# antoyang/TubeDETR

Measured on AMD Instinct MI355X. Metric: training clips/sec (fwd+bwd) at T=100 k=4 res=352, 1/2/4/8 MI355X, higher is better.
Workload: dtype bf16

## Files before the change

### include/tubedetr_hip.h

```cpp
#ifndef TUBEDETR_HIP_H
#define TUBEDETR_HIP_H
#include <stddef.h>
#include <stdint.h>
#ifdef __cplusplus
extern "C" {
#endif

#define TD_F32 0
#define TD_BF16 1
#define TD_U8 2
#define TD_OK 0
#define TD_ERR_INVALID (-1)
#define TD_ERR_LAUNCH (-2)

typedef void* td_stream_t;

const char* td_last_error(void);
int td_abi_version(void);

int td_set_deterministic(int on);
int td_get_deterministic(void);


#define TD_PROF_GEMM_128x128 0
#define TD_PROF_GEMM_128x64 1
#define TD_PROF_WGRAD 2
#define TD_PROF_GEMM_64x128 3
#define TD_PROF_PW_RESIDENT 4
#define TD_PROF_GEMM_256 5
#define TD_PROF_GEMM_256_PW 6
#define TD_PROF_FUSED 7
#define TD_PROF_CROSS_Q1 8
#define TD_PROF_WGRAD_SINGLE 9
#define TD_PROF_CHAIN 10
#define TD_PROF_FAMILIES 11
int td_prof_enable(int on);
int td_prof_collect(int family, int dtype, long long* launches, double* ms, double* flops);
int td_prof_collect_bytes(int family, int dtype, double* bytes);
int td_prof_dump(const char* path);
int td_debug_set_stamp_buffer(unsigned long long* buf);

typedef struct td_conv_desc {
  int N, Hs, Ws, C;
  int Ho, Wo;
  int R, S, stride, pad;
  int mode;
  int Nc;
  int ldc;
  int out_sp;
  int out_H, out_W;
  int aniso;
  int stride_w, pad_w;
} td_conv_desc;

typedef struct td_epilogue {
  const float* bias;
  const void* residual;
  const void* mask_src;
  int relu;
  int sigmoid;
  float dropout_p;
  uint32_t dropout_seed;
  float alpha;
  const uint32_t* dropout_counter;
} td_epilogue;

int td_conv_gemm(const void* src, const void* wmat, void* out, const td_conv_desc* d, const td_epilogue* e,
                 int dtype, td_stream_t stream);

typedef struct td_linear_ex_desc {
  int M, N, K1, K2;
  int lda1, lda2, ldc, ldr;
  int w_shared;
  long long rows1, rows2;
  const int* a1_map;
  const int* a2_map;
  const int* out_map;
  const int* res_map;
} td_linear_ex_desc;
int td_linear_ex(const void* a1, const void* a2, const void* wmat, void* out, const td_linear_ex_desc* x, const td_epilogue* e,
                 int dtype, td_stream_t stream);

int td_conv_wgrad(const void* g, const void* src, float* dw, const td_conv_desc* d, int ldg, int dtype, int splits,
                  td_stream_t stream);
int td_conv_wgrad_bias(const void* g, const void* src, float* dw, float* dbias, const td_conv_desc* d, int ldg, int dtype,
                       int splits, td_stream_t stream);

typedef struct td_wgrad_job {
  const void* g;
  const void* src;
  float* dW;
  const float* scale;
  td_conv_desc d;
  int ldg;
  int ci_real;
  float* dbias;
  int accumulate;
  int prezeroed;
} td_wgrad_job;
size_t td_conv_wgrad_batch_table_bytes(int n_jobs);
int td_conv_wgrad_batch(const td_wgrad_job* jobs, int n_jobs, int dtype, void* table_host, void* table_dev, size_t table_bytes,
                        td_stream_t stream);

typedef struct td_frame_source {
  const void* data;
  int dtype;
  int n;
  const int* index;
  const int* valid_hw;
} td_frame_source;
int td_frames_to_nhwc(const td_frame_source* srcs, int n_srcs, int C, int H, int W, int Cpad, const float* mean,
                      const float* inv_std, void* y, int dtype, td_stream_t stream);

size_t td_resnet_fwd_ws_bytes(int N, int H, int W, const int* nblocks, int dtype, int save);
int td_resnet_num_convs(const int* nblocks);
int td_resnet_fwd(const td_frame_source* srcs, int n_srcs, const float* mean, const float* inv_std, int N, int H, int W,
                  const int* nblocks, const void* const* w_fwd, const float* const* bias, int save, void* ws, size_t ws_bytes,
                  void** feat, int* feat_hw, int stem_pairs, int first_train_stage, int dtype, td_stream_t stream);
int td_bottleneck_fused(const void* x, void* out, const void* w1, const float* b1, const void* w2, const float* b2, const void* w3,
                        const float* b3, const void* wd, const float* bd, int N, int H, int W, int Cin, int dtype, td_stream_t stream);
int td_pw_chain2(const void* y2, const void* w3, const float* b3, const void* residual, void* out, const void* w1, const float* b1,
                 void* h1, int M, int planes, int dtype, td_stream_t stream);
int td_stem_pair_weights(const void* w_fwd_8, void* w_pairs, int Co, int dtype, td_stream_t stream);
int td_stem_pool(const void* x_pairs, const void* w_pairs, const float* bias, void* pooled, int N, int H, int W, int dtype,
                 td_stream_t stream);
size_t td_resnet_bwd_ws_bytes(int N, int H, int W, const int* nblocks, int first_train_stage, int dtype);
size_t td_resnet_bwd_table_bytes(const int* nblocks, int first_train_stage);
int td_resnet_bwd(const void* dfeat, int N, int N_fwd, int H, int W, const int* nblocks, int first_train_stage,
                  const void* const* w_dgrad, const float* const* scale, float* const* dW, const void* fwd_ws, void* ws,
                  size_t ws_bytes, void* table_host, void* table_dev, size_t table_bytes, int dW_prezeroed, int dtype, int only_stage, td_stream_t stream);

int td_weight_prep(const float* W, const float* bn_w, const float* bn_b, const float* bn_rm, const float* bn_rv,
                   const float* bias, int Co, int Ci, int R, int S, int Cpad, void* w_fwd, void* w_dgrad,
                   float* bias_out, float* scale_out, int dtype, td_stream_t stream);

typedef struct td_prep_item {
  const float* W;
  const float *bn_w, *bn_b, *bn_rm, *bn_rv, *bias;
  void *w_fwd, *w_dgrad;
  float *bias_out, *scale_out;
  int Co, Ci, RS, Cpad, Co_alloc, blk0;
} td_prep_item;
int td_weight_prep_batch(const td_prep_item* items_dev, int n, int total_blocks, int dtype, td_stream_t stream);

int td_wgrad_finalize(const float* dw_k, const float* scale, float* dW, int Co, int Ci, int R, int S, int Cpad,
                      int accumulate, td_stream_t stream);

int td_nchw_to_nhwc(const float* x, void* y, int N, int C, int H, int W, int Cpad, int dtype, td_stream_t stream);
int td_nhwc_to_nchw(const void* x, float* y, int N, int C, int H, int W, int dtype, td_stream_t stream);
int td_cast(const void* x, void* y, size_t n, int src_dtype, int dst_dtype, td_stream_t stream);

int td_maxpool3x3s2(const void* x, void* y, int N, int H, int W, int C, int dtype, td_stream_t stream);

int td_add_layernorm_fwd(const void* x, const void* r, const float* gamma, const float* beta, void* y, void* s_out,
                         float* mean, float* rstd, int rows, int cols, float eps, int dtype, td_stream_t stream);
int td_add_layernorm_bwd(const void* dy, const void* s, const float* mean, const float* rstd, const float* gamma,
                         const void* extra, void* ds, float* dgamma, float* dbeta, int rows, int cols, int dtype,
                         td_stream_t stream);

int td_colsum(const void* g, float* out, int rows, int cols, int ld, int dtype, td_stream_t stream);
int td_add(const void* a, const void* b, void* y, size_t n, int dtype, td_stream_t stream);

int td_relu_bwd(const void* dy, const void* y, void* g, size_t n, float scale, int dtype, td_stream_t stream);

int td_gelu_fwd(const void* x, void* y, size_t n, int dtype, td_stream_t stream);
int td_gelu_bwd(const void* dy, const void* x, void* dx, size_t n, int dtype, td_stream_t stream);

int td_dropout(const void* x, void* y, size_t n, float p, uint32_t seed, const uint32_t* dropout_counter, int dtype,
               td_stream_t stream);

int td_pos_sine(const uint8_t* mask, void* pos, int N, int h, int w, int npf, float temperature, int rows_per_image, int dtype,
                td_stream_t stream);

int td_rows_copy(const void* src, const int* src_map, const void* add, void* dst, const int* dst_map, int n_rows, int cols, int ld_src,
                 int ld_add, int ld_dst, int dtype, td_stream_t stream);
int td_rows_segment_sum(const void* in, const int* idx, const int* ptr, void* out, const int* out_map, int n_out, int cols, int ld_in,
                        int ld_out, int dtype, td_stream_t stream);

int td_mha_fwd(const void* q, const void* k, const void* v, const uint8_t* key_pad, void* out, float* probs,
               float* wavg, int B, int H, int Lq, int Lk, int hd, int ldq, int ldk, int ldv, int ldo, float scale,
               float dropout_p, uint32_t dropout_seed, const uint32_t* dropout_counter, int dtype, td_stream_t stream);
int td_mha_bwd(const void* q, const void* k, const void* v, const void* dout, const float* probs, const float* dwavg,
               void* dq, void* dk, void* dv, float* ds_ws, int B, int H, int Lq, int Lk, int hd, int ldq, int ldk,
               int ldv, int ldo, float scale, float dropout_p, uint32_t dropout_seed, const uint32_t* dropout_counter,
               int dtype, td_stream_t stream);

int td_cross_q1_fwd(const void* u, const void* mem, const void* pos, const uint8_t* key_pad, float* probs, float* wavg, void* zext,
                    int F, int S, int H, int E, int ldz, float dropout_p, uint32_t dropout_seed, const uint32_t* dropout_counter,
                    int dtype, td_stream_t stream);
int td_cross_q1_bwd(const void* u, const void* mem, const void* pos, const float* probs, const void* d_zext, const float* dwavg,
                    void* d_u, float* d_mem, int accumulate, int F, int S, int H, int E, int ldz, float dropout_p, uint32_t dropout_seed,
                    const uint32_t* dropout_counter, int dtype, td_stream_t stream);
int td_cross_q1_bwd_coef(const void* u, const void* mem, const void* pos, const float* probs, const void* d_zext, const float* dwavg,
                         void* d_u, void* coef, int coef_ld, int coef_col, int F, int S, int H, int E, int ldz, float dropout_p,
                         uint32_t dropout_seed, const uint32_t* dropout_counter, int dtype, td_stream_t stream);
int td_cross_q1_dmem(const void* coef, int coef_ld, const void* const* u, const void* const* d_zext, int n_layers, void* d_mem, int F, int S,
                     int H, int E, int ldz, int dtype, td_stream_t stream);
int td_head_blocks_expand(const float* W, const float* bias, float alpha, void* w_n, void* w_t, int E, int H, int dtype, td_stream_t stream);
int td_head_blocks_extract(const float* G, float alpha, float* dW, float* db, int E, int H, td_stream_t stream);

size_t td_mha_lean_stats_bytes(int B, int H, int Lq);
int td_mha_lean_fwd(const void* q, const void* k, const void* v, const uint8_t* key_pad, void* out, float* stats, int B, int H,
                    int Lq, int Lk, int hd, int ldq, int ldk, int ldv, int ldo, float scale, float dropout_p,
                    uint32_t dropout_seed, const uint32_t* dropout_counter, int dtype, td_stream_t stream);
int td_mha_lean_bwd(const void* q, const void* k, const void* v, const uint8_t* key_pad, const void* out, const void* dout,
                    float* stats, void* dq, void* dk, void* dv, int B, int H, int Lq, int Lk, int hd, int ldq, int ldk, int ldv,
                    int ldo, float scale, float dropout_p, uint32_t dropout_seed, const uint32_t* dropout_counter, int dtype,
                    td_stream_t stream);


#define TD_OPTIM_MAX_SEGMENTS 32
#define TD_OPTIM_MAX_GROUPS 4
#define TD_OPTIM_NORM_BLOCKS 2048
typedef struct td_optim_segment {
  long long begin, end;
  int group;
  int active;
} td_optim_segment;
size_t td_grad_norm_ws_bytes(void);
int td_grad_norm_clip(const float* grad, size_t n, const td_optim_segment* segs, int n_segs, float max_norm, void* ws,
                      size_t ws_bytes, float* norm_clip, int* step, td_stream_t stream);
int td_adamw_ema_step(float* param, const float* grad, float* exp_avg, float* exp_avg_sq, float* ema, size_t n,
                      const td_optim_segment* segs, int n_segs, const float* lr_dev, const float* norm_clip,
                      const int* step_dev, float beta1, float beta2, float eps, float weight_decay, float ema_decay,
                      td_stream_t stream);

int td_criterion_fwd(const float* boxes, const float* tgt, const long long* keep, const float* sted, const float* weights,
                     const uint8_t* time_mask, const uint8_t* positive, const int* inter, const float* num_boxes_dev,
                     float num_boxes_host, float sigma, int nl, int b, int T, int n, float* losses, float* g_l1, float* g_giou,
                     float* g_sted, float* g_w, td_stream_t stream);
int td_criterion_bwd(const float* dlosses, const float* g_l1, const float* g_giou, const float* g_sted, const float* g_w,
                     float* d_boxes, float* d_sted, float* d_weights, int nl, int b, int T, td_stream_t stream);

int td_sted_decode(const float* steds, long long* start_end, int n_videos, int T, td_stream_t stream);

typedef struct td_resample_job {
  const void* src;
  long long src_frame_stride;
  int src_pitch;
  int T, sh, sw;
  int flip;
// ... 16 lines not shown
```

### tubedetr_amd/_hip.py

```python
from __future__ import annotations

import ctypes as C
import os

import torch

TD_F32, TD_BF16 = 0, 1
EXPECTED_ABI = 11
_LIB_PATH = os.environ.get("TD_HIP_LIB") or os.path.join(os.path.dirname(os.path.abspath(__file__)), "lib", "libtubedetr_hip.so")
_lib = None


class ConvDesc(C.Structure):
    _fields_ = [(n, C.c_int) for n in ("N", "Hs", "Ws", "C", "Ho", "Wo", "R", "S", "stride", "pad", "mode", "Nc", "ldc", "out_sp", "out_H", "out_W",
                                       "aniso", "stride_w", "pad_w")]


class PrepItem(C.Structure):
    _fields_ = [(n, C.c_void_p) for n in ("W", "bn_w", "bn_b", "bn_rm", "bn_rv", "bias", "w_fwd", "w_dgrad", "bias_out", "scale_out")] + \
               [(n, C.c_int) for n in ("Co", "Ci", "RS", "Cpad", "Co_alloc", "blk0")]


class WgradJob(C.Structure):
    _fields_ = [("g", C.c_void_p), ("src", C.c_void_p), ("dW", C.c_void_p), ("scale", C.c_void_p), ("d", ConvDesc), ("ldg", C.c_int), ("ci_real", C.c_int), ("dbias", C.c_void_p), ("accumulate", C.c_int), ("prezeroed", C.c_int)]


TD_U8 = 2


class FrameSource(C.Structure):
    _fields_ = [("data", C.c_void_p), ("dtype", C.c_int), ("n", C.c_int), ("index", C.c_void_p), ("valid_hw", C.c_void_p)]


class LinearExDesc(C.Structure):
    _fields_ = [(n, C.c_int) for n in ("M", "N", "K1", "K2", "lda1", "lda2", "ldc", "ldr", "w_shared")] + \
               [("rows1", C.c_longlong), ("rows2", C.c_longlong)] + [(n, C.c_void_p) for n in ("a1_map", "a2_map", "out_map", "res_map")]


class OptimSegment(C.Structure):
    _fields_ = [("begin", C.c_longlong), ("end", C.c_longlong), ("group", C.c_int), ("active", C.c_int)]


class ResampleJob(C.Structure):
    _fields_ = [("src", C.c_void_p), ("src_frame_stride", C.c_longlong)] + [(n, C.c_int) for n in ("src_pitch", "T", "sh", "sw", "flip", "rh", "rw", "wy", "wx", "wh", "ww")] + \
               [("dst", C.c_void_p)] + [(n, C.c_int) for n in ("planar", "frame_off", "H", "W")] + [("mask", C.c_void_p)]


class Epilogue(C.Structure):
    _fields_ = [
        ("bias", C.c_void_p),
        ("residual", C.c_void_p),
        ("mask_src", C.c_void_p),
        ("relu", C.c_int),
        ("sigmoid", C.c_int),
        ("dropout_p", C.c_float),
        ("dropout_seed", C.c_uint32),
        ("alpha", C.c_float),
        ("dropout_counter", C.c_void_p),
    ]


_P, _I, _F, _U32, _SZ = C.c_void_p, C.c_int, C.c_float, C.c_uint32, C.c_size_t
_SIGS = {
    "td_prof_enable": [_I],
    "td_prof_dump": [C.c_char_p],
    "td_debug_set_stamp_buffer": [_P],
    "td_prof_collect": [_I, _I, C.POINTER(C.c_longlong), C.POINTER(C.c_double), C.POINTER(C.c_double)],
    "td_prof_collect_bytes": [_I, _I, C.POINTER(C.c_double)],
    "td_conv_gemm": [_P, _P, _P, C.POINTER(ConvDesc), C.POINTER(Epilogue), _I, _P],
    "td_conv_wgrad": [_P, _P, _P, C.POINTER(ConvDesc), _I, _I, _I, _P],
    "td_conv_wgrad_bias": [_P, _P, _P, _P, C.POINTER(ConvDesc), _I, _I, _I, _P],
    "td_conv_wgrad_batch": [C.POINTER(WgradJob), _I, _I, _P, _P, _SZ, _P],
    "td_resnet_num_convs": [C.POINTER(C.c_int)],
    "td_resnet_fwd": [C.POINTER(FrameSource), _I, C.POINTER(C.c_float), C.POINTER(C.c_float), _I, _I, _I, C.POINTER(C.c_int), C.POINTER(_P), C.POINTER(_P), _I, _P, _SZ,
                      C.POINTER(_P), C.POINTER(C.c_int), _I, _I, _I, _P],
    "td_bottleneck_fused": [_P, _P, _P, _P, _P, _P, _P, _P, _P, _P, _I, _I, _I, _I, _I, _P],
    "td_stem_pair_weights": [_P, _P, _I, _I, _P],
    "td_stem_pool": [_P, _P, _P, _P, _I, _I, _I, _I, _P],
    "td_pw_chain2": [_P, _P, _P, _P, _P, _P, _P, _P, _I, _I, _I, _P],
    "td_set_deterministic": [_I],
    "td_get_deterministic": [],
    "td_frames_to_nhwc": [C.POINTER(FrameSource), _I, _I, _I, _I, _I, C.POINTER(C.c_float), C.POINTER(C.c_float), _P, _I, _P],
    "td_resnet_bwd": [_P, _I, _I, _I, _I, C.POINTER(C.c_int), _I, C.POINTER(_P), C.POINTER(_P), C.POINTER(_P), _P, _P, _SZ, _P, _P, _SZ, _I, _I, _I, _P],
    "td_weight_prep_batch": [_P, _I, _I, _I, _P],
    "td_weight_prep": [_P, _P, _P, _P, _P, _P, _I, _I, _I, _I, _I, _P, _P, _P, _P, _I, _P],
    "td_wgrad_finalize": [_P, _P, _P, _I, _I, _I, _I, _I, _I, _P],
    "td_nchw_to_nhwc": [_P, _P, _I, _I, _I, _I, _I, _I, _P],
    "td_nhwc_to_nchw": [_P, _P, _I, _I, _I, _I, _I, _P],
    "td_cast": [_P, _P, _SZ, _I, _I, _P],
    "td_maxpool3x3s2": [_P, _P, _I, _I, _I, _I, _I, _P],
    "td_add_layernorm_fwd": [_P, _P, _P, _P, _P, _P, _P, _P, _I, _I, _F, _I, _P],
    "td_add_layernorm_bwd": [_P, _P, _P, _P, _P, _P, _P, _P, _P, _I, _I, _I, _P],
    "td_colsum": [_P, _P, _I, _I, _I, _I, _P],
    "td_add": [_P, _P, _P, _SZ, _I, _P],
    "td_relu_bwd": [_P, _P, _P, _SZ, _F, _I, _P],
    "td_gelu_fwd": [_P, _P, _SZ, _I, _P],
    "td_gelu_bwd": [_P, _P, _P, _SZ, _I, _P],
    "td_dropout": [_P, _P, _SZ, _F, _U32, _P, _I, _P],
    "td_pos_sine": [_P, _P, _I, _I, _I, _I, _F, _I, _I, _P],
    "td_linear_ex": [_P, _P, _P, _P, C.POINTER(LinearExDesc), C.POINTER(Epilogue), _I, _P],
    "td_rows_copy": [_P, _P, _P, _P, _P, _I, _I, _I, _I, _I, _I, _P],
    "td_rows_segment_sum": [_P, _P, _P, _P, _P, _I, _I, _I, _I, _I, _P],
    "td_criterion_fwd": [_P, _P, _P, _P, _P, _P, _P, _P, _P, _F, _F, _I, _I, _I, _I, _P, _P, _P, _P, _P, _P],
    "td_criterion_bwd": [_P, _P, _P, _P, _P, _P, _P, _P, _I, _I, _I, _P],
    "td_sted_decode": [_P, _P, _I, _I, _P],
    "td_grad_norm_clip": [_P, _SZ, C.POINTER(OptimSegment), _I, _F, _P, _SZ, _P, _P, _P],
    "td_adamw_ema_step": [_P, _P, _P, _P, _P, _SZ, C.POINTER(OptimSegment), _I, _P, _P, _P, _F, _F, _F, _F, _F, _P],
    "td_mha_fwd": [_P, _P, _P, _P, _P, _P, _P, _I, _I, _I, _I, _I, _I, _I, _I, _I, _F, _F, _U32, _P, _I, _P],
    "td_mha_bwd": [_P, _P, _P, _P, _P, _P, _P, _P, _P, _P, _I, _I, _I, _I, _I, _I, _I, _I, _I, _F, _F, _U32, _P, _I, _P],
    "td_cross_q1_fwd": [_P, _P, _P, _P, _P, _P, _P, _I, _I, _I, _I, _I, _F, _U32, _P, _I, _P],
    "td_cross_q1_bwd": [_P, _P, _P, _P, _P, _P, _P, _P, _I, _I, _I, _I, _I, _I, _F, _U32, _P, _I, _P],
    "td_cross_q1_bwd_coef": [_P, _P, _P, _P, _P, _P, _P, _P, _I, _I, _I, _I, _I, _I, _I, _F, _U32, _P, _I, _P],
    "td_cross_q1_dmem": [_P, _I, _P, _P, _I, _P, _I, _I, _I, _I, _I, _I, _P],
    "td_head_blocks_expand": [_P, _P, _F, _P, _P, _I, _I, _I, _P],
    "td_head_blocks_extract": [_P, _F, _P, _P, _I, _I, _P],
    "td_mha_lean_fwd": [_P, _P, _P, _P, _P, _P, _I, _I, _I, _I, _I, _I, _I, _I, _I, _F, _F, _U32, _P, _I, _P],
    "td_mha_lean_bwd": [_P, _P, _P, _P, _P, _P, _P, _P, _P, _P, _I, _I, _I, _I, _I, _I, _I, _I, _I, _F, _F, _U32, _P, _I, _P],
    "td_clip_resample": [C.POINTER(ResampleJob), _I, _P, _P, _SZ, _P],
}
_SIZE_SIGS = {
    "td_grad_norm_ws_bytes": [],
    "td_mha_lean_stats_bytes": [_I, _I, _I],
    "td_conv_wgrad_batch_table_bytes": [_I],
    "td_clip_resample_table_bytes": [_I],
    "td_resnet_bwd_table_bytes": [C.POINTER(C.c_int), _I],
    "td_resnet_fwd_ws_bytes": [_I, _I, _I, C.POINTER(C.c_int), _I, _I],
    "td_resnet_bwd_ws_bytes": [_I, _I, _I, C.POINTER(C.c_int), _I, _I],
}
EXPORTS = ["td_last_error", "td_abi_version"] + list(_SIGS) + list(_SIZE_SIGS)


def lib_path() -> str:
    return _LIB_PATH


def lib() -> C.CDLL:
    global _lib
    if _lib is None:
        if not os.path.exists(_LIB_PATH):
            raise RuntimeError(
                f"{_LIB_PATH} is missing: build it with `python -m tubedetr_amd.build` (or __graft_entry__.build()); "
                "tubedetr_amd has no CPU / eager fallback"
            )
        L = C.CDLL(_LIB_PATH)
        L.td_last_error.restype = C.c_char_p
        L.td_last_error.argtypes = []
        L.td_abi_version.restype = C.c_int
        L.td_abi_version.argtypes = []
        got = L.td_abi_version()
        if got != EXPECTED_ABI:
            raise RuntimeError(f"{_LIB_PATH} has ABI version {got}, this binding needs {EXPECTED_ABI}: rebuild it with "
                               "`python -m tubedetr_amd.build --force`")
        for name, sig in _SIGS.items():
            fn = getattr(L, name)
            fn.restype = C.c_int
            fn.argtypes = sig
        for name, sig in _SIZE_SIGS.items():
            fn = getattr(L, name)
            fn.restype = C.c_size_t
            fn.argtypes = sig
        _lib = L
    return _lib


def check(rc: int, what: str = ""):
    if rc != 0:
        raise RuntimeError(f"libtubedetr_hip {what} failed ({rc}): {lib().td_last_error().decode()}")


def stream_ptr() -> int:
    return torch._C._cuda_getCurrentRawStream(torch._C._cuda_getDevice())


def dtype_code(dt: torch.dtype) -> int:
    if dt == torch.float32:
        return TD_F32
    if dt == torch.bfloat16:
        return TD_BF16
    raise TypeError(f"unsupported compute dtype {dt}")


def ptr(t) -> int:
    if t is None:
# ... 4 lines not shown
```

### tubedetr_amd/csrc/elementwise.hip

```cpp
#include "td_common.h"

namespace td {

template <typename T>
__global__ void maxpool3x3s2_kernel(const T* x, T* y, int N, int H, int W, int C, int Ho, int Wo) {
  constexpr int VEC = 16 / sizeof(T);
  const int cv = C / VEC;
  const size_t n = (size_t)N * Ho * Wo * cv;
  const size_t idx = (size_t)blockIdx.x * blockDim.x + threadIdx.x;
  if (idx >= n) return;
  int c = (idx % cv) * VEC;
  size_t t = idx / cv;
  int wo = t % Wo; t /= Wo;
  int ho = t % Ho;
  int img = t / Ho;
  float m[VEC];
#pragma unroll
  for (int i = 0; i < VEC; ++i) m[i] = -INFINITY;
  for (int r = 0; r < 3; ++r) {
    int h = ho * 2 - 1 + r;
    if ((unsigned)h >= (unsigned)H) continue;
    for (int s = 0; s < 3; ++s) {
      int w = wo * 2 - 1 + s;
      if ((unsigned)w >= (unsigned)W) continue;
// ... 43 lines not shown
      float dlt = v[j] - mu;
      var += dlt * dlt;
    }
  }
  var = wave_sum(var) / cols;
  const float rs = rsqrtf(var + eps);
  if (lane == 0) {
    if (mean) mean[row] = mu;
    if (rstd) rstd[row] = rs;
  }
#pragma unroll
  for (int j = 0; j < LN_MAXJ; ++j) {
    int c = lane + 64 * j;
    if (j < nj && c < cols) {
      if (s_out) Elem<T>::store(s_out, base + c, v[j]);
      Elem<T>::store(y, base + c, (v[j] - mu) * rs * gamma[c] + beta[c]);
    }
  }
}

__device__ __forceinline__ void unpack4v(const uint2& v, float (&o)[4]) {
  o[0] = __uint_as_float(v.x << 16); o[1] = __uint_as_float(v.x & 0xffff0000u);
  o[2] = __uint_as_float(v.y << 16); o[3] = __uint_as_float(v.y & 0xffff0000u);
}
__device__ __forceinline__ uint2 pack4_bf16(const float (&v)[4]) {
  return make_uint2((uint32_t)f32_to_bf16(v[0]) | ((uint32_t)f32_to_bf16(v[1]) << 16), (uint32_t)f32_to_bf16(v[2]) | ((uint32_t)f32_to_bf16(v[3]) << 16));
}
static bool aligned8(const void* a, const void* b, const void* c, const void* d) {
  return (((uintptr_t)a | (uintptr_t)b | (uintptr_t)c | (uintptr_t)d) & 7) == 0;
}

template <int NJ>
__global__ __launch_bounds__(256) void add_layernorm_fwd_v4_kernel(const u16* __restrict__ x, const u16* __restrict__ r, const float* __restrict__ gamma,
                                                                   const float* __restrict__ beta, u16* __restrict__ y, u16* __restrict__ s_out,
                                                                   float* __restrict__ mean, float* __restrict__ rstd, int rows, float eps) {
  constexpr int cols = NJ * 256;
  const int lane = threadIdx.x & 63;
  const int row = blockIdx.x * 4 + (threadIdx.x >> 6);
  if (row >= rows) return;
  const size_t base = (size_t)row * cols + lane * 4;
  float v[NJ][4];
  float sum = 0.f;
#pragma unroll
  for (int j = 0; j < NJ; ++j) {
    unpack4v(*(const uint2*)(x + base + 256 * j), v[j]);
    if (r) {
      float a[4];
      unpack4v(*(const uint2*)(r + base + 256 * j), a);
#pragma unroll
      for (int e = 0; e < 4; ++e) v[j][e] += a[e];
    }
#pragma unroll
    for (int e = 0; e < 4; ++e) sum += v[j][e];
  }
  const float mu = wave_sum(sum) * (1.f / cols);
  float var = 0.f;
#pragma unroll
  for (int j = 0; j < NJ; ++j)
#pragma unroll
    for (int e = 0; e < 4; ++e) {
      const float d = v[j][e] - mu;
      var += d * d;
    }
  var = wave_sum(var) * (1.f / cols);
  const float rs = rsqrtf(var + eps);
  if (lane == 0) {
    if (mean) mean[row] = mu;
    if (rstd) rstd[row] = rs;
  }
#pragma unroll
  for (int j = 0; j < NJ; ++j) {
    const float4 gm = *(const float4*)(gamma + lane * 4 + 256 * j), bt = *(const float4*)(beta + lane * 4 + 256 * j);
    if (s_out) *(uint2*)(s_out + base + 256 * j) = pack4_bf16(v[j]);
    float o[4] = {(v[j][0] - mu) * rs * gm.x + bt.x, (v[j][1] - mu) * rs * gm.y + bt.y, (v[j][2] - mu) * rs * gm.z + bt.z,
                  (v[j][3] - mu) * rs * gm.w + bt.w};
    *(uint2*)(y + base + 256 * j) = pack4_bf16(o);
  }
}

template <int NJ>
__global__ __launch_bounds__(256) void add_layernorm_bwd_v4_kernel(const u16* __restrict__ dy, const u16* __restrict__ s, const float* __restrict__ mean,
                                                                   const float* __restrict__ rstd, const float* __restrict__ gamma,
                                                                   const u16* __restrict__ extra, u16* __restrict__ ds, float* dgamma, float* dbeta,
                                                                   int rows) {
  constexpr int cols = NJ * 256;
  const int lane = threadIdx.x & 63;
  const int wid = blockIdx.x * 4 + (threadIdx.x >> 6);
  const int nw = gridDim.x * 4;
  float pg[NJ][4], pb[NJ][4], gm[NJ][4];
#pragma unroll
  for (int j = 0; j < NJ; ++j) {
    const float4 g4 = *(const float4*)(gamma + lane * 4 + 256 * j);
    gm[j][0] = g4.x; gm[j][1] = g4.y; gm[j][2] = g4.z; gm[j][3] = g4.w;
#pragma unroll
    for (int e = 0; e < 4; ++e) pg[j][e] = pb[j][e] = 0.f;
  }
  for (int row = wid; row < rows; row += nw) {
    const size_t base = (size_t)row * cols + lane * 4;
    const float mu = mean[row], rs = rstd[row];
    float xh[NJ][4], dg[NJ][4];
    float c1 = 0.f, c2 = 0.f;
#pragma unroll
    for (int j = 0; j < NJ; ++j) {
      float d[4], sv[4];
      unpack4v(*(const uint2*)(dy + base + 256 * j), d);
      unpack4v(*(const uint2*)(s + base + 256 * j), sv);
#pragma unroll
      for (int e = 0; e < 4; ++e) {
        xh[j][e] = (sv[e] - mu) * rs;
        dg[j][e] = d[e] * gm[j][e];
        c1 += dg[j][e];
        c2 += dg[j][e] * xh[j][e];
        pg[j][e] += d[e] * xh[j][e];
        pb[j][e] += d[e];
      }
    }
    c1 = wave_sum(c1) * (1.f / cols);
    c2 = wave_sum(c2) * (1.f / cols);
#pragma unroll
    for (int j = 0; j < NJ; ++j) {
      float o[4];
#pragma unroll
      for (int e = 0; e < 4; ++e) o[e] = rs * (dg[j][e] - c1 - xh[j][e] * c2);
      if (extra) {
        float ex[4];
        unpack4v(*(const uint2*)(extra + base + 256 * j), ex);
#pragma unroll
        for (int e = 0; e < 4; ++e) o[e] += ex[e];
      }
      *(uint2*)(ds + base + 256 * j) = pack4_bf16(o);
    }
  }
  __shared__ float redg[4][cols], redb[4][cols];
  const int wv = threadIdx.x >> 6;
#pragma unroll
  for (int j = 0; j < NJ; ++j)
#pragma unroll
    for (int e = 0; e < 4; ++e) {
      redg[wv][lane * 4 + 256 * j + e] = pg[j][e];
      redb[wv][lane * 4 + 256 * j + e] = pb[j][e];
    }
  __syncthreads();
  for (int c = threadIdx.x; c < cols; c += 256) {
    if (dgamma) atomicAdd(dgamma + c, redg[0][c] + redg[1][c] + redg[2][c] + redg[3][c]);
    if (dbeta) atomicAdd(dbeta + c, redb[0][c] + redb[1][c] + redb[2][c] + redb[3][c]);
  }
}

template <typename T>
__global__ __launch_bounds__(256) void add_layernorm_bwd_kernel(const T* dy, const T* s, const float* mean, const float* rstd,
                                                                const float* gamma, const T* extra, T* ds, float* dgamma,
                                                                float* dbeta, int rows, int cols) {
  const int lane = threadIdx.x & 63;
  const int wid = blockIdx.x * 4 + (threadIdx.x >> 6);
  const int nw = gridDim.x * 4;
  const int nj = (cols + 63) / 64;
  float pg[LN_MAXJ], pb[LN_MAXJ];
#pragma unroll
  for (int j = 0; j < LN_MAXJ; ++j) pg[j] = pb[j] = 0.f;
  for (int row = wid; row < rows; row += nw) {
    const size_t base = (size_t)row * cols;
    const float mu = mean[row], rs = rstd[row];
    float xh[LN_MAXJ], dg[LN_MAXJ];
    float c1 = 0.f, c2 = 0.f;
#pragma unroll
    for (int j = 0; j < LN_MAXJ; ++j) {
      xh[j] = dg[j] = 0.f;
      int c = lane + 64 * j;
      if (j < nj && c < cols) {
        float d = Elem<T>::load(dy, base + c);
        xh[j] = (Elem<T>::load(s, base + c) - mu) * rs;
        dg[j] = d * gamma[c];
        c1 += dg[j];
        c2 += dg[j] * xh[j];
        pg[j] += d * xh[j];
        pb[j] += d;
      }
    }
    c1 = wave_sum(c1) / cols;
    c2 = wave_sum(c2) / cols;
#pragma unroll
    for (int j = 0; j < LN_MAXJ; ++j) {
      int c = lane + 64 * j;
      if (j < nj && c < cols) {
        float o = rs * (dg[j] - c1 - xh[j] * c2);
        if (extra) o += Elem<T>::load(extra, base + c);
        Elem<T>::store(ds, base + c, o);
      }
    }
  }
  __shared__ float redg[4][64 * LN_MAXJ], redb[4][64 * LN_MAXJ];
  const int wv = threadIdx.x >> 6;
#pragma unroll
  for (int j = 0; j < LN_MAXJ; ++j) {
    if (j < nj) {
      redg[wv][lane + 64 * j] = pg[j];
      redb[wv][lane + 64 * j] = pb[j];
    }
  }
  __syncthreads();
  for (int c = threadIdx.x; c < cols; c += 256) {
    if (dgamma) atomicAdd(dgamma + c, redg[0][c] + redg[1][c] + redg[2][c] + redg[3][c]);
    if (dbeta) atomicAdd(dbeta + c, redb[0][c] + redb[1][c] + redb[2][c] + redb[3][c]);
  }
}

template <typename T>
__global__ void colsum_kernel(const T* g, float* out, int rows, int cols, int ld, int rows_per_block) {
  const int c = blockIdx.x * blockDim.x + threadIdx.x;
  if (c >= cols) return;
  const int r0 = blockIdx.y * rows_per_block;
  const int r1 = min(rows, r0 + rows_per_block);
  float acc = 0.f;
  for (int r = r0; r < r1; ++r) acc += Elem<T>::load(g, (size_t)r * ld + c);
  atomicAdd(out + c, acc);
}

template <typename T>
__global__ __launch_bounds__(256) void colsum_vec_kernel(const T* g, float* out, int rows, int cols, int ld, int rows_per_block) {
  constexpr int VEC = 16 / sizeof(T);
  __shared__ float red[8][32 * VEC + 1];
  const int cg = threadIdx.x & 31, rl = threadIdx.x >> 5;
  const int c0 = (blockIdx.x * 32 + cg) * VEC;
  const int r0 = blockIdx.y * rows_per_block;
  const int r1 = min(rows, r0 + rows_per_block);
  float acc[VEC];
#pragma unroll
  for (int i = 0; i < VEC; ++i) acc[i] = 0.f;
  if (c0 < cols) {
    for (int r = r0 + rl; r < r1; r += 8) {
      uint4 v = *(const uint4*)(g + (size_t)r * ld + c0);
      const T* e = (const T*)&v;
#pragma unroll
      for (int i = 0; i < VEC; ++i) acc[i] += Elem<T>::load(e, i);
    }
  }
#pragma unroll
  for (int i = 0; i < VEC; ++i) red[rl][cg * VEC + i] = acc[i];
  __syncthreads();
  for (int c = threadIdx.x; c < 32 * VEC; c += 256) {
    const int col = blockIdx.x * 32 * VEC + c;
    if (col < cols) {
      float sum = 0.f;
#pragma unroll
      for (int j = 0; j < 8; ++j) sum += red[j][c];
      atomicAdd(out + col, sum);
    }
  }
}

__device__ __forceinline__ float gelu_f(float x) { return 0.5f * x * (1.f + erff(x * 0.70710678118654752f)); }
__device__ __forceinline__ float gelu_grad_f(float x) {
  return 0.5f * (1.f + erff(x * 0.70710678118654752f)) + x * 0.3989422804014327f * __expf(-0.5f * x * x);
}

template <typename T, int OP>
__global__ __launch_bounds__(256) void ew_kernel(const T* a, const T* b, T* y, size_t n, float scale, uint32_t thresh, uint32_t seed_in, const uint32_t* seed_dev) {
  const uint32_t seed = (OP == 2) ? effective_seed(seed_in, seed_dev) : seed_in;
  constexpr int VEC = 16 / sizeof(T);
  const size_t nv = n / VEC;
  size_t i = (size_t)blockIdx.x * blockDim.x + threadIdx.x;
  const size_t stride = (size_t)gridDim.x * blockDim.x;
  for (size_t v = i; v < nv; v += stride) {
    uint4 va = ((const uint4*)a)[v], vb = make_uint4(0, 0, 0, 0), vo;
    if (b) vb = ((const uint4*)b)[v];
    const T* ea = (const T*)&va;
    const T* eb = (const T*)&vb;
    T* eo = (T*)&vo;
#pragma unroll
    for (int k = 0; k < VEC; ++k) {
// ... 107 lines not shown
  }
}

template <typename T>
__global__ __launch_bounds__(256) void rows_segment_sum_kernel(const char* __restrict__ in, const int* __restrict__ idx, const int* __restrict__ ptr,
                                                               char* __restrict__ out, const int* __restrict__ out_map, int n_out, int chunks, int ld_in,
                                                               int ld_out) {
  constexpr int EPL = 16 / sizeof(T);
  const size_t total = (size_t)n_out * chunks;
  for (size_t t = (size_t)blockIdx.x * blockDim.x + threadIdx.x; t < total; t += (size_t)gridDim.x * blockDim.x) {
    const int r = (int)(t / chunks), c = (int)(t - (size_t)r * chunks);
    float acc[EPL];
#pragma unroll
    for (int q = 0; q < EPL; ++q) acc[q] = 0.f;
    const int j0 = ptr[r], j1 = ptr[r + 1];
    for (int j = j0; j < j1; ++j) {
      const uint4 v = *(const uint4*)(in + ((size_t)idx[j] * ld_in + (size_t)c * EPL) * sizeof(T));
      if constexpr (sizeof(T) == 2) {
        const uint32_t* pv = (const uint32_t*)&v;
#pragma unroll
        for (int q = 0; q < 4; ++q) {
          acc[2 * q] += __uint_as_float(pv[q] << 16);
          acc[2 * q + 1] += __uint_as_float(pv[q] & 0xffff0000u);
        }
      } else {
        acc[0] += __uint_as_float(v.x); acc[1] += __uint_as_float(v.y); acc[2] += __uint_as_float(v.z); acc[3] += __uint_as_float(v.w);
      }
    }
    uint4 o;
    if constexpr (sizeof(T) == 2) {
      o.x = (uint32_t)f32_to_bf16(acc[0]) | ((uint32_t)f32_to_bf16(acc[1]) << 16);
      o.y = (uint32_t)f32_to_bf16(acc[2]) | ((uint32_t)f32_to_bf16(acc[3]) << 16);
      o.z = (uint32_t)f32_to_bf16(acc[4 % EPL]) | ((uint32_t)f32_to_bf16(acc[5 % EPL]) << 16);
      o.w = (uint32_t)f32_to_bf16(acc[6 % EPL]) | ((uint32_t)f32_to_bf16(acc[7 % EPL]) << 16);
    } else {
      o = make_uint4(__float_as_uint(acc[0]), __float_as_uint(acc[1]), __float_as_uint(acc[2]), __float_as_uint(acc[3]));
    }
    *(uint4*)(out + ((size_t)(out_map ? out_map[r] : r) * ld_out + (size_t)c * EPL) * sizeof(T)) = o;
  }
}

}
using namespace td;

static inline unsigned nblk(size_t n, int bs = 256) { return (unsigned)((n + bs - 1) / bs); }
#define TD_DISPATCH(dtype, CALL_BF16, CALL_F32, who)  \
  if (dtype == TD_BF16) { CALL_BF16; }                \
  else if (dtype == TD_F32) { CALL_F32; }             \
  else TD_REQUIRE(false, who ": bad dtype")

extern "C" int td_maxpool3x3s2(const void* x, void* y, int N, int H, int W, int C, int dtype, td_stream_t stream) {
  TD_REQUIRE(x && y, "td_maxpool3x3s2: null pointer");
  const int vec = dtype == TD_BF16 ? 8 : 4;
  TD_REQUIRE(C % vec == 0, "td_maxpool3x3s2: C must be a multiple of %d", vec);
  const int Ho = (H + 2 - 3) / 2 + 1, Wo = (W + 2 - 3) / 2 + 1;
  size_t n = (size_t)N * Ho * Wo * (C / vec);
  hipStream_t st = (hipStream_t)stream;
  TD_DISPATCH(dtype, (maxpool3x3s2_kernel<u16><<<nblk(n), 256, 0, st>>>((const u16*)x, (u16*)y, N, H, W, C, Ho, Wo)),
              (maxpool3x3s2_kernel<float><<<nblk(n), 256, 0, st>>>((const float*)x, (float*)y, N, H, W, C, Ho, Wo)),
              "td_maxpool3x3s2");
  return check_launch("td_maxpool3x3s2");
}

extern "C" int td_add_layernorm_fwd(const void* x, const void* r, const float* gamma, const float* beta, void* y,
                                    void* s_out, float* mean, float* rstd, int rows, int cols, float eps, int dtype,
                                    td_stream_t stream) {
  TD_REQUIRE(x && gamma && beta && y, "td_add_layernorm_fwd: null pointer");
  TD_REQUIRE(cols <= 64 * LN_MAXJ, "td_add_layernorm_fwd: cols > %d", 64 * LN_MAXJ);
  if (rows == 0) return TD_OK;
  hipStream_t st = (hipStream_t)stream;
  unsigned g = (rows + 3) / 4;
  if (dtype == TD_BF16 && (cols == 256 || cols == 768) && aligned8(x, r, y, s_out)) {
    if (cols == 256) add_layernorm_fwd_v4_kernel<1><<<g, 256, 0, st>>>((const u16*)x, (const u16*)r, gamma, beta, (u16*)y, (u16*)s_out, mean, rstd, rows, eps);
    else add_layernorm_fwd_v4_kernel<3><<<g, 256, 0, st>>>((const u16*)x, (const u16*)r, gamma, beta, (u16*)y, (u16*)s_out, mean, rstd, rows, eps);
    return check_launch("td_add_layernorm_fwd");
  }
  TD_DISPATCH(dtype,
              (add_layernorm_fwd_kernel<u16><<<g, 256, 0, st>>>((const u16*)x, (const u16*)r, gamma, beta, (u16*)y, (u16*)s_out, mean, rstd, rows, cols, eps)),
              (add_layernorm_fwd_kernel<float><<<g, 256, 0, st>>>((const float*)x, (const float*)r, gamma, beta, (float*)y, (float*)s_out, mean, rstd, rows, cols, eps)),
              "td_add_layernorm_fwd");
  return check_launch("td_add_layernorm_fwd");
}

extern "C" int td_add_layernorm_bwd(const void* dy, const void* s, const float* mean, const float* rstd,
                                    const float* gamma, const void* extra, void* ds, float* dgamma, float* dbeta,
                                    int rows, int cols, int dtype, td_stream_t stream) {
  TD_REQUIRE(dy && s && mean && rstd && gamma && ds, "td_add_layernorm_bwd: null pointer");
  TD_REQUIRE(cols <= 64 * LN_MAXJ, "td_add_layernorm_bwd: cols > %d", 64 * LN_MAXJ);
  if (rows == 0) return TD_OK;
  hipStream_t st = (hipStream_t)stream;
  unsigned g = (rows + 3) / 4;
  if (dtype == TD_BF16 && (cols == 256 || cols == 768) && aligned8(dy, s, ds, extra)) {
    unsigned gv = (rows + 31) / 32;
    if (gv > 1024) gv = 1024;
    if (deterministic()) gv = 1;
    if (cols == 256) add_layernorm_bwd_v4_kernel<1><<<gv, 256, 0, st>>>((const u16*)dy, (const u16*)s, mean, rstd, gamma, (const u16*)extra, (u16*)ds, dgamma, dbeta, rows);
    else add_layernorm_bwd_v4_kernel<3><<<gv, 256, 0, st>>>((const u16*)dy, (const u16*)s, mean, rstd, gamma, (const u16*)extra, (u16*)ds, dgamma, dbeta, rows);
    return check_launch("td_add_layernorm_bwd");
  }
  if (g > 256) g = 256;
  if (deterministic()) g = 1;
  TD_DISPATCH(dtype,
              (add_layernorm_bwd_kernel<u16><<<g, 256, 0, st>>>((const u16*)dy, (const u16*)s, mean, rstd, gamma, (const u16*)extra, (u16*)ds, dgamma, dbeta, rows, cols)),
              (add_layernorm_bwd_kernel<float><<<g, 256, 0, st>>>((const float*)dy, (const float*)s, mean, rstd, gamma, (const float*)extra, (float*)ds, dgamma, dbeta, rows, cols)),
              "td_add_layernorm_bwd");
  return check_launch("td_add_layernorm_bwd");
}

extern "C" int td_colsum(const void* g, float* out, int rows, int cols, int ld, int dtype, td_stream_t stream) {
  TD_REQUIRE(g && out, "td_colsum: null pointer");
  if (rows == 0 || cols == 0) return TD_OK;
  hipStream_t st = (hipStream_t)stream;
  const int vec = dtype == TD_BF16 ? 8 : 4;
  if (cols % vec == 0 && ld % vec == 0) {
    const int gx = (cols + 32 * vec - 1) / (32 * vec);
    int rpb = (int)(((long long)rows * gx + 511) / 512);
    if (rpb < 64) rpb = 64;
    if (deterministic()) rpb = rows;
    dim3 grid(gx, (rows + rpb - 1) / rpb);
    TD_DISPATCH(dtype, (colsum_vec_kernel<u16><<<grid, 256, 0, st>>>((const u16*)g, out, rows, cols, ld, rpb)),
                (colsum_vec_kernel<float><<<grid, 256, 0, st>>>((const float*)g, out, rows, cols, ld, rpb)), "td_colsum");
    return check_launch("td_colsum");
  }
  int rpb = (int)(((long long)rows * ((cols + 255) / 256) + 1023) / 1024);
  if (rpb < 8) rpb = 8;
  if (deterministic()) rpb = rows;
  dim3 grid((cols + 255) / 256, (rows + rpb - 1) / rpb);
  TD_DISPATCH(dtype, (colsum_kernel<u16><<<grid, 256, 0, st>>>((const u16*)g, out, rows, cols, ld, rpb)),
              (colsum_kernel<float><<<grid, 256, 0, st>>>((const float*)g, out, rows, cols, ld, rpb)), "td_colsum");
  return check_launch("td_colsum");
}

extern "C" int td_add(const void* a, const void* b, void* y, size_t n, int dtype, td_stream_t stream) {
  TD_REQUIRE(a && y, "td_add: null pointer");
  if (n == 0) return TD_OK;
  hipStream_t st = (hipStream_t)stream;
  unsigned g = nblk(n / 4 + 1);
  if (g > 4096) g = 4096;
  TD_REQUIRE(((uintptr_t)a | (uintptr_t)y | (uintptr_t)b) % 16 == 0, "td_add: pointers must be 16-byte aligned");
  TD_DISPATCH(dtype, (ew_kernel<u16, 0><<<g, 256, 0, st>>>((const u16*)a, (const u16*)b, (u16*)y, n, 1.f, 0, 0, nullptr)),
              (ew_kernel<float, 0><<<g, 256, 0, st>>>((const float*)a, (const float*)b, (float*)y, n, 1.f, 0, 0, nullptr)), "td_add");
  return check_launch("td_add");
}

extern "C" int td_relu_bwd(const void* dy, const void* y, void* g, size_t n, float scale, int dtype, td_stream_t stream) {
  TD_REQUIRE(dy && y && g, "td_relu_bwd: null pointer");
  if (n == 0) return TD_OK;
  hipStream_t st = (hipStream_t)stream;
  unsigned gr = nblk(n);
  if (gr > 4096) gr = 4096;
  TD_REQUIRE(((uintptr_t)dy | (uintptr_t)y | (uintptr_t)g) % 16 == 0, "td_relu_bwd: pointers must be 16-byte aligned");
  TD_DISPATCH(dtype, (ew_kernel<u16, 1><<<gr, 256, 0, st>>>((const u16*)dy, (const u16*)y, (u16*)g, n, scale, 0, 0, nullptr)),
              (ew_kernel<float, 1><<<gr, 256, 0, st>>>((const float*)dy, (const float*)y, (float*)g, n, scale, 0, 0, nullptr)), "td_relu_bwd");
  return check_launch("td_relu_bwd");
}

extern "C" int td_gelu_fwd(const void* x, void* y, size_t n, int dtype, td_stream_t stream) {
  TD_REQUIRE(x && y, "td_gelu_fwd: null pointer");
  if (n == 0) return TD_OK;
  hipStream_t st = (hipStream_t)stream;
  unsigned gr = nblk(n);
  if (gr > 4096) gr = 4096;
  TD_REQUIRE(((uintptr_t)x | (uintptr_t)y) % 16 == 0, "td_gelu_fwd: pointers must be 16-byte aligned");
  TD_DISPATCH(dtype, (ew_kernel<u16, 3><<<gr, 256, 0, st>>>((const u16*)x, nullptr, (u16*)y, n, 1.f, 0, 0, nullptr)),
              (ew_kernel<float, 3><<<gr, 256, 0, st>>>((const float*)x, nullptr, (float*)y, n, 1.f, 0, 0, nullptr)), "td_gelu_fwd");
  return check_launch("td_gelu_fwd");
}

extern "C" int td_gelu_bwd(const void* dy, const void* x, void* dx, size_t n, int dtype, td_stream_t stream) {
  TD_REQUIRE(dy && x && dx, "td_gelu_bwd: null pointer");
  if (n == 0) return TD_OK;
  hipStream_t st = (hipStream_t)stream;
  unsigned gr = nblk(n);
  if (gr > 4096) gr = 4096;
  TD_REQUIRE(((uintptr_t)dy | (uintptr_t)x | (uintptr_t)dx) % 16 == 0, "td_gelu_bwd: pointers must be 16-byte aligned");
  TD_DISPATCH(dtype, (ew_kernel<u16, 4><<<gr, 256, 0, st>>>((const u16*)dy, (const u16*)x, (u16*)dx, n, 1.f, 0, 0, nullptr)),
              (ew_kernel<float, 4><<<gr, 256, 0, st>>>((const float*)dy, (const float*)x, (float*)dx, n, 1.f, 0, 0, nullptr)), "td_gelu_bwd");
  return check_launch("td_gelu_bwd");
}

extern "C" int td_dropout(const void* x, void* y, size_t n, float p, uint32_t seed, const uint32_t* dropout_counter, int dtype,
                          td_stream_t stream) {
  TD_REQUIRE(x && y, "td_dropout: null pointer");
  TD_REQUIRE(p >= 0.f && p < 1.f, "td_dropout: p out of range");
  if (n == 0) return TD_OK;
  hipStream_t st = (hipStream_t)stream;
  unsigned gr = nblk(n);
// ... 61 lines not shown
```

### tubedetr_amd/csrc/gemm_conv.hip

```cpp
#include <stdlib.h>

#include <type_traits>

#include "td_common.h"
#include <algorithm>
#include <vector>

#ifndef TD_WGRAD_EARLY_ISSUE
#define TD_WGRAD_EARLY_ISSUE 1
#endif
#ifndef TD_BIG_XCD_CONTIG
#define TD_BIG_XCD_CONTIG 1
#endif
namespace td {

struct GemmParams {
  const char* src;
  const char* w;
  char* out;
  td_conv_desc d;
  int M, K;
  uint32_t src_bytes, w_bytes;
  unsigned long long* dbg;
  const float* bias;
  const char* residual;
  const char* mask_src;
  int relu, sigmoid;
  float alpha;
  uint32_t drop_thresh;
  float drop_scale;
  uint32_t seed;
  const uint32_t* seed_dev;
  const char* src2;
  uint32_t src2_bytes;
  int K1, lda1, lda2, ldr;
  int w_shared;
  const int* a1_map;
  const int* a2_map;
  const int* out_map;
  const int* res_map;
  int tap_inner;
  int w_ld;
  int wtap[4];
  int use_wtap;
};

template <typename T>
struct Mfma;
template <>
struct Mfma<u16> {
  static __device__ __forceinline__ void run(const uint4& wf, const uint4& af, f32x4& acc) {
    acc = __builtin_amdgcn_mfma_f32_16x16x32_bf16(*(const bf16x8*)&wf, *(const bf16x8*)&af, acc, 0, 0, 0);
  }
};
template <>
struct Mfma<float> {
  static __device__ __forceinline__ void run(const uint4& wf, const uint4& af, f32x4& acc) {
    const float* a = (const float*)&wf;
    const float* b = (const float*)&af;
#pragma unroll
    for (int s = 0; s < 4; ++s) acc = __builtin_amdgcn_mfma_f32_16x16x4f32(a[s], b[s], acc, 0, 0, 0);
  }
};

template <typename T>
__device__ __forceinline__ void load4(const char* base, size_t off, float (&o)[4]);
template <>
__device__ __forceinline__ void load4<float>(const char* base, size_t off, float (&o)[4]) {
  float4 v = *(const float4*)(base + off * 4);
  o[0] = v.x; o[1] = v.y; o[2] = v.z; o[3] = v.w;
}
template <>
__device__ __forceinline__ void load4<u16>(const char* base, size_t off, float (&o)[4]) {
  uint2 v = *(const uint2*)(base + off * 2);
  o[0] = __uint_as_float(v.x << 16); o[1] = __uint_as_float(v.x & 0xffff0000u);
  o[2] = __uint_as_float(v.y << 16); o[3] = __uint_as_float(v.y & 0xffff0000u);
}
template <typename T, typename V>
__device__ __forceinline__ void unpack4(const V& v, float (&o)[4]);
template <>
__device__ __forceinline__ void unpack4<float, float4>(const float4& v, float (&o)[4]) {
  o[0] = v.x; o[1] = v.y; o[2] = v.z; o[3] = v.w;
}
template <>
__device__ __forceinline__ void unpack4<u16, uint2>(const uint2& v, float (&o)[4]) {
  o[0] = __uint_as_float(v.x << 16); o[1] = __uint_as_float(v.x & 0xffff0000u);
  o[2] = __uint_as_float(v.y << 16); o[3] = __uint_as_float(v.y & 0xffff0000u);
}
typedef __bf16 bf16x2_t __attribute__((ext_vector_type(2)));
__device__ __forceinline__ uint32_t pack_bf16x2(float lo, float hi) {
  bf16x2_t v = {(__bf16)lo, (__bf16)hi};
  return *(uint32_t*)&v;
}
template <typename T>
__device__ __forceinline__ void unpack16(const uint4& v, float (&o)[16 / sizeof(T)]);
template <>
__device__ __forceinline__ void unpack16<float>(const uint4& v, float (&o)[4]) {
  o[0] = __uint_as_float(v.x); o[1] = __uint_as_float(v.y); o[2] = __uint_as_float(v.z); o[3] = __uint_as_float(v.w);
}
template <>
__device__ __forceinline__ void unpack16<u16>(const uint4& v, float (&o)[8]) {
  o[0] = __uint_as_float(v.x << 16); o[1] = __uint_as_float(v.x & 0xffff0000u);
  o[2] = __uint_as_float(v.y << 16); o[3] = __uint_as_float(v.y & 0xffff0000u);
  o[4] = __uint_as_float(v.z << 16); o[5] = __uint_as_float(v.z & 0xffff0000u);
  o[6] = __uint_as_float(v.w << 16); o[7] = __uint_as_float(v.w & 0xffff0000u);
}
template <typename T>
__device__ __forceinline__ uint4 pack16(const float (&v)[16 / sizeof(T)]);
template <>
__device__ __forceinline__ uint4 pack16<float>(const float (&v)[4]) {
  return make_uint4(__float_as_uint(v[0]), __float_as_uint(v[1]), __float_as_uint(v[2]), __float_as_uint(v[3]));
}
template <>
__device__ __forceinline__ uint4 pack16<u16>(const float (&v)[8]) {
  return make_uint4(pack_bf16x2(v[0], v[1]), pack_bf16x2(v[2], v[3]), pack_bf16x2(v[4], v[5]), pack_bf16x2(v[6], v[7]));
}
template <typename T>
__device__ __forceinline__ void store4(char* base, size_t off, const float (&v)[4]);
template <>
__device__ __forceinline__ void store4<float>(char* base, size_t off, const float (&v)[4]) {
  *(float4*)(base + off * 4) = make_float4(v[0], v[1], v[2], v[3]);
}
template <>
__device__ __forceinline__ void store4<u16>(char* base, size_t off, const float (&v)[4]) {
  uint2 o;
  o.x = (uint32_t)f32_to_bf16(v[0]) | ((uint32_t)f32_to_bf16(v[1]) << 16);
  o.y = (uint32_t)f32_to_bf16(v[2]) | ((uint32_t)f32_to_bf16(v[3]) << 16);
// ... 239 lines not shown
  const int n = n0 + wx * WN + cc * EPL;
  const bool vec_ok = ((d.ldc % EPL) == 0) && (!GX || (p.ldr % EPL) == 0) && (n + EPL - 1 < d.Nc);
  size_t offs[NIT];
  size_t roffs[GX ? NIT : 1];
  bool live[NIT];
  uint4 res[NIT], msk[NIT];
  auto fetch_epilogue_operands = [&]() {
#pragma unroll
    for (int it = 0; it < NIT; ++it) {
      const int m = m0 + wy * WM + it * RPI + rsub;
      live[it] = (m < p.M) && (n < d.Nc);
      size_t orow = live[it] ? m : 0;
      if (!PW && d.out_sp > 1) {
        int ni = (int)orow / HoWo;
        int rem = (int)orow - ni * HoWo;
        int ho = rem / d.Wo, wo = rem - ho * d.Wo;
        orow = ((size_t)ni * d.out_H + (size_t)ho * d.out_sp) * d.out_W + (size_t)wo * d.out_sp;
      }
      if constexpr (GX) {
        const size_t mm = orow;
        if (p.out_map) orow = (size_t)p.out_map[mm];
        roffs[it] = (p.res_map ? (size_t)p.res_map[mm] : orow) * (size_t)p.ldr + n;
      }
      offs[it] = orow * d.ldc + n;
      if (vec_ok && live[it]) {
        if (p.residual) res[it] = ld16(p.residual + (GX ? roffs[it] : offs[it]) * ES);
        if (p.mask_src) msk[it] = ld16(p.mask_src + offs[it] * ES);
      }
    }
  };

  const int nk = (p.K + BK - 1) / BK;
#define TD_STAMP(i) do { if (p.dbg && t == 0) p.dbg[(size_t)blockIdx.x * 8 + (i)] = __builtin_readcyclecounter(); } while (0)
  TD_STAMP(0);
  if constexpr (NST == 2) {
    issue_tile(smem0);
    for (int kt = 0; kt < nk; kt += 2) {
      __syncthreads();
      if (kt == 0) TD_STAMP(1);
      if (kt + 1 < nk) issue_tile(smem1);
      compute_tile(smem0);
      if (kt + 1 >= nk) break;
      __syncthreads();
      if (kt + 2 < nk) issue_tile(smem0);
      compute_tile(smem1);
    }
    TD_STAMP(2);
    fetch_epilogue_operands();
  } else {
#define TD_CG_STEP(cur, nxt, j)                                                     \
  asm volatile("s_waitcnt vmcnt(%0)" ::"n"(AI + BI) : "memory");                    \
  __builtin_amdgcn_s_barrier();                                                     \
  issue_tile(nxt);                                                                  \
  if ((j) >= 0) compute_tile(cur);
    for (int it = -2; it < nk; it += 3) {
      TD_CG_STEP(smem1, smem0, it)
      if (it + 1 >= nk) break;
      TD_CG_STEP(smem2, smem1, it + 1)
      if (it + 2 >= nk) break;
      TD_CG_STEP(smem0, smem2, it + 2)
    }
#undef TD_CG_STEP
    asm volatile("s_waitcnt vmcnt(0)" ::: "memory");
    TD_STAMP(2);
    fetch_epilogue_operands();
  }

  asm volatile("s_waitcnt lgkmcnt(0)" ::: "memory");
  __builtin_amdgcn_s_barrier();
  TD_STAMP(3);
  float* stg = (float*)((wave < 2 ? smem0 : smem1) + (wave & 1) * (WM * WN * 4));
  const float alpha = p.alpha;
#pragma unroll
  for (int j = 0; j < TM; ++j) {
    const int row = j * 16 + lr;
#pragma unroll
    for (int i = 0; i < TN; ++i) {
      const int c = (i * 4 + lg) ^ (row & (CPRW - 1));
      f32x4 a = acc[i][j];
      *(float4*)(stg + row * WN + c * 4) = make_float4(a[0] * alpha, a[1] * alpha, a[2] * alpha, a[3] * alpha);
    }
  }
  asm volatile("s_waitcnt lgkmcnt(0)" ::: "memory");
  float bias[EPL];
#pragma unroll
  for (int r = 0; r < EPL; ++r) bias[r] = (p.bias && n + r < d.Nc) ? p.bias[n + r] : 0.f;
  TD_STAMP(4);
  const uint32_t eff_seed = effective_seed(p.seed, p.drop_thresh ? p.seed_dev : nullptr);
#pragma unroll
  for (int it = 0; it < NIT; ++it) {
    if (!live[it]) continue;
    const int row = it * RPI + rsub;
    const int sw = row & (CPRW - 1);
    float v[EPL];
#pragma unroll
    for (int q = 0; q < EPL / 4; ++q) {
      float4 f = *(const float4*)(stg + row * WN + (((cc * (EPL / 4) + q) ^ sw) * 4));
      v[4 * q + 0] = f.x + bias[4 * q + 0]; v[4 * q + 1] = f.y + bias[4 * q + 1];
      v[4 * q + 2] = f.z + bias[4 * q + 2]; v[4 * q + 3] = f.w + bias[4 * q + 3];
    }
    const size_t off = offs[it];
    if (vec_ok) {
      if (p.residual) {
        float r8[EPL];
        unpack16<T>(res[it], r8);
#pragma unroll
        for (int r = 0; r < EPL; ++r) v[r] += r8[r];
      }
      if (p.relu) {
#pragma unroll
        for (int r = 0; r < EPL; ++r) v[r] = fmaxf(v[r], 0.f);
      }
      if (p.sigmoid) {
#pragma unroll
        for (int r = 0; r < EPL; ++r) v[r] = sigmoidf_(v[r]);
      }
      if (p.mask_src) {
        float m8[EPL];
        unpack16<T>(msk[it], m8);
#pragma unroll
        for (int r = 0; r < EPL; ++r) v[r] = m8[r] > 0.f ? v[r] : 0.f;
      }
      if (p.drop_thresh) {
#pragma unroll
        for (int r = 0; r < EPL; ++r) v[r] = dropout_keep(eff_seed, (uint32_t)(off + r), p.drop_thresh) ? v[r] * p.drop_scale : 0.f;
      }
      st16(p.out + off * ES, pack16<T>(v));
    } else {
      const int cnt = min(EPL, d.Nc - n);
      for (int r = 0; r < cnt; ++r) {
        float x = v[r];
        if (p.residual) x += Elem<T>::load(p.residual, (GX ? roffs[it] : off) + r);
        if (p.relu) x = fmaxf(x, 0.f);
        if (p.sigmoid) x = sigmoidf_(x);
        if (p.mask_src) x = Elem<T>::load(p.mask_src, off + r) > 0.f ? x : 0.f;
        if (p.drop_thresh) x = dropout_keep(eff_seed, (uint32_t)(off + r), p.drop_thresh) ? x * p.drop_scale : 0.f;
        Elem<T>::store(p.out, off + r, x);
      }
    }
  }
  TD_STAMP(5);
#undef TD_STAMP
}

#ifndef TD_ABL
#define TD_ABL 0
#endif
template <int OFF>
__device__ __forceinline__ u32x4_t lds_read16(uint32_t addr) {
  u32x4_t r;
#if TD_ABL & 4
  asm volatile("" : "=v"(r) : "v"(addr));
#else
  asm volatile("ds_read_b128 %0, %1 offset:%2" : "=v"(r) : "v"(addr), "n"(OFF));
#endif
  return r;
}
template <int N>
__device__ __forceinline__ void wait_vmcnt() {
  asm volatile("s_waitcnt vmcnt(%0)" ::"n"(N) : "memory");
}
template <int I>
using ic = std::integral_constant<int, I>;

#ifndef TD_BIG8_AUX_W
#define TD_BIG8_AUX_W 0
#endif
#ifndef TD_BIG8_AUX_X
#define TD_BIG8_AUX_X 0
#endif
template <bool TU, bool RES>
__global__ __launch_bounds__(512, 1) void conv_gemm_big8_kernel(GemmParams p) {
  using T = u16;
  constexpr int ES = 2, BM = 256, BN = 256, BK = 64, NW = 8, VEC = 8;
  constexpr int WM = 128, WN = 64, TM = 8, TN = 4;
  constexpr int STAGE = (BM + BN) * 128, WREG = BM * 128;
  constexpr uint32_t OOB = 0xFFFFFFF0u;
  constexpr int MAXT = 160;
  constexpr int STG = 16 * WN * ES;
  __shared__ __attribute__((aligned(16))) char smem[2 * STAGE];
  __shared__ __attribute__((aligned(16))) uint4 ktab[MAXT];
  __shared__ __attribute__((aligned(16))) char stg_all[NW * STG];

  const td_conv_desc& d = p.d;
  const int t = threadIdx.x;
  const int wave = __builtin_amdgcn_readfirstlane(t >> 6), lane = t & 63;
  const int NT = d.Nc / BN;
  const int lrow = lane >> 3;
  const int chunk = (lane & 7) ^ lrow;
  const int HoWo = d.Ho * d.Wo;
  const __amdgpu_buffer_rsrc_t rs_src = __builtin_amdgcn_make_buffer_rsrc((void*)p.src, 0, p.src_bytes, 0x00020000);
  const __amdgpu_buffer_rsrc_t rs_w = __builtin_amdgcn_make_buffer_rsrc((void*)p.w, 0, p.w_bytes, 0x00020000);
  const uint32_t out_bytes = (uint32_t)p.M * (uint32_t)d.ldc * ES;
  const __amdgpu_buffer_rsrc_t rs_out = __builtin_amdgcn_make_buffer_rsrc((void*)p.out, 0, out_bytes, 0x00020000);
  const int wy = wave >> 2, wx = wave & 3;
  const int RS = d.R * d.S;
  const int lane_c = chunk * VEC;
  const int nk = p.K / BK;
  const bool tap_inner = TU && p.tap_inner;
  if (t < nk + 4) {
    uint32_t xo, tap = 0, wo;
    if constexpr (TU) {
      const int cpt = d.C / BK;
      const int chunkc = tap_inner ? t / RS : t % cpt;
      tap = tap_inner ? t - chunkc * RS : t / cpt;
      const int r = (int)tap / d.S, sx = (int)tap - r * d.S;
      const int pix = d.mode == 0 ? r * d.Ws + sx : -(r * d.Ws + sx);
      xo = (uint32_t)(pix * d.C + chunkc * BK) * ES;
      wo = (uint32_t)((int)tap * d.C + chunkc * BK) * ES;
    } else {
      xo = wo = (uint32_t)t * BK * ES;
    }
    ktab[t] = make_uint4(xo, t < nk ? tap : 0u, wo, t < nk ? 0xFFFFFFFFu : 0u);
  }
#if TD_ABL & 16
  for (int i = t; i < 2 * STAGE / 4; i += 512) ((uint32_t*)smem)[i] = 0x3F803F80u ^ (mix32((uint32_t)i * 0x9E3779B1u + blockIdx.x) & 0x007F007Fu);
#endif
  const int nvb = 8 * ((cdiv(p.M, BM) + 7) / 8) * NT;
  const float rcp_howo = 1.f / (float)HoWo, rcp_wo = 1.f / (float)d.Wo;
  auto divmod = [](int a, int dv, float rcp, int& q, int& r) {
    q = (int)((float)a * rcp);
    r = a - q * dv;
    const int up = r >= dv, dn = r < 0;
    q += up - dn;
    r += (dn - up) * dv;
  };
#if TD_BIG_XCD_CONTIG
  const int mtx = (cdiv(p.M, BM) + 7) / 8;
  auto tile_m0 = [&](int vb) { const int seq = vb >> 3; return ((vb & 7) * mtx + seq / NT) * BM; };
  auto tile_n0 = [&](int vb) { const int seq = vb >> 3; return (seq - (seq / NT) * NT) * BN; };
  auto tile_ok = [&](int vb) { return vb < nvb && (vb >> 3) / NT < mtx && tile_m0(vb) < p.M; };
#else
  auto tile_m0 = [&](int vb) { const int seq = vb >> 3; return ((seq / NT) * 8 + (vb & 7)) * BM; };
  auto tile_n0 = [&](int vb) { const int seq = vb >> 3; return (seq - (seq / NT) * NT) * BN; };
  auto tile_ok = [&](int vb) { return vb < nvb && tile_m0(vb) < p.M; };
#endif

  uint32_t a_off[4];
  uint32_t a_mask[4];
  uint32_t b_off[4];
  const bool small_filter = d.R <= 3 && d.S <= 3;
  const int sgn = d.mode == 0 ? 1 : -1;
  auto tile_addr = [&](int m0, int n0) {
#pragma unroll
    for (int q = 0; q < 4; ++q) {
      const int m = m0 + (wave >> 2) * WM + q * 32 + (wave & 3) * 8 + lrow;
      const bool ok = m < p.M;
      if constexpr (!TU) {
        a_off[q] = (uint32_t)m * (uint32_t)p.K * ES + (uint32_t)lane_c * ES;
        a_mask[q] = ok ? 1u : 0u;
      } else {
        const int mm = ok ? m : 0;
        int n, rem, ho, wo;
        divmod(mm, HoWo, rcp_howo, n, rem);
// ... 82 lines not shown
#endif
#pragma unroll
    for (int ks = 0; ks < 2; ++ks)
#pragma unroll
      for (int j = 0; j < 2; ++j)
#pragma unroll
        for (int i = 0; i < TN; ++i)
          asm volatile("v_mfma_f32_16x16x32_bf16 %0, %1, %2, %0" : "+v"(acc[i][2 * P + j]) : "v"(wreg[ks][i]), "v"(xreg[j][ks]));
#if !(TD_ABL & 8)
    __builtin_amdgcn_s_setprio(0);
#endif
    __builtin_amdgcn_sched_barrier(0);
    __builtin_amdgcn_s_barrier();
  };
  auto prologue_issue = [&]() {
    u32x4_t e0 = lds_read16<0>(tab0);
    ea = lds_read16<16>(tab0);
    asm volatile("s_waitcnt lgkmcnt(0)" : "+v"(e0), "+v"(ea) : : "memory");
    __builtin_amdgcn_sched_barrier(0);
#pragma unroll
    for (int i = 0; i < 4; ++i) issue_w(smem, i, e0);
#pragma unroll
    for (int q = 0; q < 4; ++q) issue_x(smem, q, e0);
#pragma unroll
    for (int i = 0; i < 4; ++i) issue_w(smem + STAGE, i, ea);
  };

  const uint32_t stg0 = (uint32_t)(uintptr_t)(lds_ptr_t)stg_all + (uint32_t)wave * STG;
  uint32_t swa[TN];
#pragma unroll
  for (int i = 0; i < TN; ++i) swa[i] = stg0 + (uint32_t)(lr * 128 + (((2 * i + (lg >> 1)) ^ (lr & 7)) << 4) + (lg & 1) * 8);
  const int cc = lane & 7, rsub = lane >> 3;
  const uint32_t sra = stg0 + (uint32_t)(rsub * 128 + ((cc ^ rsub) << 4));
  const float alpha = p.alpha;

#define TD_STAMP(i) do { if (p.dbg && t == 0) p.dbg[(size_t)vb * 8 + (i)] = __builtin_readcyclecounter(); } while (0)
  int vb = blockIdx.x;
  if (!tile_ok(vb)) return;
  tile_addr(tile_m0(vb), tile_n0(vb));
  asm volatile("s_waitcnt lgkmcnt(0)" ::: "memory");
  __builtin_amdgcn_s_barrier();
  prologue_issue();
#pragma unroll 1
  for (;;) {
    const int m0 = tile_m0(vb), n0 = tile_n0(vb);
    TD_STAMP(0);
    if (p.dbg && t == 0) p.dbg[(size_t)vb * 8 + 6] = wall_clock64();
#pragma unroll
    for (int i = 0; i < TN; ++i)
#pragma unroll
      for (int j = 0; j < TM; ++j) acc[i][j] = f32x4{0.f, 0.f, 0.f, 0.f};
    taddr = tab0 + 2 * 16;
    f32x4 bs[TN];
#pragma unroll
    for (int i = 0; i < TN; ++i) bs[i] = p.bias ? *(const f32x4*)(p.bias + n0 + wx * WN + i * 16 + lg * 4) : f32x4{0.f, 0.f, 0.f, 0.f};
    wait_vmcnt<7>();
    __builtin_amdgcn_s_barrier();
    if (wy == 1) __builtin_amdgcn_s_barrier();
    TD_STAMP(1);
    const int npair = (nk + 1) / 2;
#pragma unroll 1
    for (int it = 0; it < npair; ++it) {
      phase(ic<0>{}, ic<0>{}); phase(ic<0>{}, ic<1>{}); phase(ic<0>{}, ic<2>{}); phase(ic<0>{}, ic<3>{});
      phase(ic<1>{}, ic<0>{}); phase(ic<1>{}, ic<1>{}); phase(ic<1>{}, ic<2>{}); phase(ic<1>{}, ic<3>{});
    }
    if (wy == 0) __builtin_amdgcn_s_barrier();
    TD_STAMP(2);
    asm volatile("s_waitcnt vmcnt(0) lgkmcnt(0)" ::: "memory");
    asm volatile("s_nop 15\n\ts_nop 15" ::: "memory");
#pragma unroll
    for (int i = 0; i < TN; ++i)
#pragma unroll
      for (int j = 0; j < TM; ++j) asm volatile("" : "+v"(acc[i][j]));
#pragma unroll
    for (int i = 0; i < TN; ++i) asm volatile("" : "+v"(bs[i]));
    const int vb_next = vb + (int)gridDim.x;
    const bool more = tile_ok(vb_next);
    if (more) {
      tile_addr(tile_m0(vb_next), tile_n0(vb_next));
      prologue_issue();
    }
    TD_STAMP(3);
    uint4 mk[2][2];
    auto seg_off = [&](int j, int h) -> uint32_t {
      const int m = m0 + wy * WM + j * 16 + h * 8 + rsub;
      return m < p.M ? ((uint32_t)m * (uint32_t)d.ldc + (uint32_t)(n0 + wx * WN + cc * 8)) * ES : OOB;
    };
    auto fetch_mask = [&](int j, int b) {
#pragma unroll
      for (int h = 0; h < 2; ++h) {
        const uint32_t off = seg_off(j, h);
        mk[b][h] = off != OOB ? ld16(p.mask_src + off) : make_uint4(0, 0, 0, 0);
      }
    };
    auto put = [&](int j) {
#pragma unroll
      for (int i = 0; i < TN; ++i) {
        const f32x4 a = acc[i][j];
        float v[4] = {a[0] * alpha + bs[i][0], a[1] * alpha + bs[i][1], a[2] * alpha + bs[i][2], a[3] * alpha + bs[i][3]};
        if constexpr (RES) {
          const int m = m0 + wy * WM + j * 16 + lr;
          if (m < p.M) {
            const uint2 rr = *(const uint2*)(p.residual + ((size_t)m * d.ldc + n0 + wx * WN + i * 16 + lg * 4) * ES);
            v[0] += __uint_as_float(rr.x << 16); v[1] += __uint_as_float(rr.x & 0xffff0000u);
            v[2] += __uint_as_float(rr.y << 16); v[3] += __uint_as_float(rr.y & 0xffff0000u);
          }
        }
        if (p.relu) {
#pragma unroll
          for (int r = 0; r < 4; ++r) v[r] = fmaxf(v[r], 0.f);
        }
        const uint32_t lo = pack_bf16x2(v[0], v[1]), hi = pack_bf16x2(v[2], v[3]);
        asm volatile("ds_write_b64 %0, %1" ::"v"(swa[i]), "v"(u32x2_t{lo, hi}) : "memory");
      }
    };
    if (p.mask_src) fetch_mask(0, 0);
    put(0);
    u32x4_t o0, o1;
    asm volatile("ds_read_b128 %0, %1" : "=v"(o0) : "v"(sra) : "memory");
    asm volatile("ds_read_b128 %0, %1 offset:1024" : "=v"(o1) : "v"(sra) : "memory");
#pragma unroll
    for (int j = 0; j < TM; ++j) {
      const int b = j & 1;
      if (j + 1 < TM) {
        if (p.mask_src) fetch_mask(j + 1, b ^ 1);
        put(j + 1);
        asm volatile("s_waitcnt lgkmcnt(4)" : "+v"(o0), "+v"(o1) : : "memory");
      } else {
        asm volatile("s_waitcnt lgkmcnt(0)" : "+v"(o0), "+v"(o1) : : "memory");
      }
      u32x4_t s0 = o0, s1 = o1;
      if (j + 1 < TM) {
        asm volatile("ds_read_b128 %0, %1" : "=v"(o0) : "v"(sra) : "memory");
        asm volatile("ds_read_b128 %0, %1 offset:1024" : "=v"(o1) : "v"(sra) : "memory");
      }
      if (p.mask_src) {
        float x8[8], m8[8];
        unpack16<T>(make_uint4(s0.x, s0.y, s0.z, s0.w), x8);
        unpack16<T>(mk[b][0], m8);
#pragma unroll
        for (int r = 0; r < 8; ++r) x8[r] = m8[r] > 0.f ? x8[r] : 0.f;
        const uint4 q0 = pack16<T>(x8);
        s0 = u32x4_t{q0.x, q0.y, q0.z, q0.w};
        unpack16<T>(make_uint4(s1.x, s1.y, s1.z, s1.w), x8);
        unpack16<T>(mk[b][1], m8);
#pragma unroll
        for (int r = 0; r < 8; ++r) x8[r] = m8[r] > 0.f ? x8[r] : 0.f;
        const uint4 q1 = pack16<T>(x8);
        s1 = u32x4_t{q1.x, q1.y, q1.z, q1.w};
      }
      __builtin_amdgcn_raw_buffer_store_b128(s0, rs_out, (int)seg_off(j, 0), 0, 0);
      __builtin_amdgcn_raw_buffer_store_b128(s1, rs_out, (int)seg_off(j, 1), 0, 0);
    }
    TD_STAMP(5);
    if (p.dbg && t == 0) p.dbg[(size_t)vb * 8 + 7] = wall_clock64();
    if (!more) break;
    vb = vb_next;
  }
#undef TD_STAMP
}

template <bool TU>
__global__ __launch_bounds__(512, 1) void conv_gemm_big8n_kernel(GemmParams p) {
  using T = u16;
  constexpr int ES = 2, BM = 256, BN = 128, BK = 64, NW = 8, VEC = 8;
  constexpr int WM = 64, WN = 64, TM = 4, TN = 4;
  constexpr int WREG = BM * 128, STAGE = (BM + BN) * 128;
  constexpr uint32_t OOB = 0xFFFFFFF0u;
  constexpr int MAXT = 160;
  __shared__ __attribute__((aligned(16))) char smem[3 * STAGE];
  __shared__ __attribute__((aligned(16))) uint4 ktab[MAXT];

  const td_conv_desc& d = p.d;
  const int t = threadIdx.x;
  const int wave = __builtin_amdgcn_readfirstlane(t >> 6), lane = t & 63;
  const int NT = d.Nc / BN;
  const int xcd = blockIdx.x & 7, seq = blockIdx.x >> 3;
#if TD_BIG_XCD_CONTIG
  const int mtx = (cdiv(p.M, BM) + 7) / 8;
  const int mt = xcd * mtx + seq / NT, nt = seq - (seq / NT) * NT;
#else
  const int mt = (seq / NT) * 8 + xcd, nt = seq - (seq / NT) * NT;
#endif
  const int m0 = mt * BM, n0 = nt * BN;
  if (m0 >= p.M) return;
  const int lrow = lane >> 3;
  const int chunk = (lane & 7) ^ lrow;
  const int lane_c = chunk * VEC;
  const int HoWo = d.Ho * d.Wo;
  const int RS = d.R * d.S;
  const __amdgpu_buffer_rsrc_t rs_src = __builtin_amdgcn_make_buffer_rsrc((void*)p.src, 0, p.src_bytes, 0x00020000);
  const __amdgpu_buffer_rsrc_t rs_w = __builtin_amdgcn_make_buffer_rsrc((void*)p.w, 0, p.w_bytes, 0x00020000);
  const int wy = wave >> 1, wx = wave & 1;
  const int grp = wave >> 2;

  uint32_t a_off[4], a_mask[4];
  const float rcp_howo = 1.f / (float)HoWo, rcp_wo = 1.f / (float)d.Wo;
  auto divmod = [](int a, int dv, float rcp, int& q, int& r) {
    q = (int)((float)a * rcp);
    r = a - q * dv;
    const int up = r >= dv, dn = r < 0;
    q += up - dn;
    r += (dn - up) * dv;
  };
#pragma unroll
  for (int q = 0; q < 4; ++q) {
    const int m = m0 + (wave >> 1) * WM + (q >> 1) * 32 + ((wave & 1) * 2 + (q & 1)) * 8 + lrow;
    const bool ok = m < p.M;
    if constexpr (!TU) {
      a_off[q] = ((uint32_t)m * (uint32_t)p.K + (uint32_t)lane_c) * ES;
      a_mask[q] = ok ? 1u : 0u;
    } else {
      const int mm = ok ? m : 0;
      int n, rem, ho, wo;
      divmod(mm, HoWo, rcp_howo, n, rem);
      divmod(rem, d.Wo, rcp_wo, ho, wo);
      const int hb = d.mode == 0 ? ho * d.stride - d.pad : ho + d.pad;
      const int wb = d.mode == 0 ? wo * d.stride - d.pad : wo + d.pad;
      a_off[q] = ((uint32_t)(n * d.Hs * d.Ws + hb * d.Ws + wb) * (uint32_t)d.C + (uint32_t)lane_c) * ES;
      uint32_t cols = 0, msk = 0;
      for (int sx = 0; sx < d.S; ++sx) cols |= ((unsigned)(d.mode == 0 ? wb + sx : wb - sx) < (unsigned)d.Ws ? 1u : 0u) << sx;
      for (int r = 0; r < d.R; ++r) msk |= ((unsigned)(d.mode == 0 ? hb + r : hb - r) < (unsigned)d.Hs ? cols : 0u) << (r * d.S);
      a_mask[q] = ok ? msk : 0u;
    }
  }
  uint32_t b_off[2];
#pragma unroll
  for (int i = 0; i < 2; ++i) b_off[i] = ((uint32_t)(n0 + (i * NW + wave) * 8 + lrow) * (uint32_t)p.K + (uint32_t)lane_c) * ES;
  const int nk = p.K / BK;
  const bool tap_inner = TU && p.tap_inner;
// ... 1080 lines not shown
  if (jok[Jx]) {                                                                                                                            \
    float v_[4];                                                                                                                            \
    asm volatile("v_accvgpr_read_b32 %0, a%c4\n\tv_accvgpr_read_b32 %1, a%c5\n\tv_accvgpr_read_b32 %2, a%c6\n\tv_accvgpr_read_b32 %3, a%c7"     \
                 : "=v"(v_[0]), "=v"(v_[1]), "=v"(v_[2]), "=v"(v_[3])                                                                        \
                 : "n"(4 * (8 * (I) + (Jx))), "n"(4 * (8 * (I) + (Jx)) + 1), "n"(4 * (8 * (I) + (Jx)) + 2), "n"(4 * (8 * (I) + (Jx)) + 3));      \
    float* dst = jdst[Jx] + (size_t)((I) * 16) * cstride;                                                                                   \
    _Pragma("unroll") for (int rr = 0; rr < 4; ++rr) {                                                                                      \
      const float v = v_[rr] * sc[I][rr];                                                                                                   \
      if (plain) dst[(size_t)rr * cstride] = v;                                                                                             \
      else atomicAdd(dst + (size_t)rr * cstride, v);                                                                                        \
    }                                                                                                                                       \
  }
  const size_t cstride = (size_t)p.ci_real * RS;
  bool jok[8];
  float* jdst[8];
#pragma unroll
  for (int j = 0; j < 8; ++j) {
    const int kko = kk0 + wxk * 128 + j * 16 + lr;
    int tap = 0, ci = kko;
    if (!PW && RS > 1) {
      tap = kko / d.C;
      ci = kko - tap * d.C;
    }
    jok[j] = kko < p.K && ci < p.ci_real;
    jdst[j] = p.dw + ((size_t)(co0 + wyc * 128 + 4 * lg) * p.ci_real + ci) * RS + tap;
  }
#define TD_W4_OUTROW(I) TD_W4_OUT(I, 0) TD_W4_OUT(I, 1) TD_W4_OUT(I, 2) TD_W4_OUT(I, 3) TD_W4_OUT(I, 4) TD_W4_OUT(I, 5) TD_W4_OUT(I, 6) TD_W4_OUT(I, 7)
  TD_W4_OUTROW(0) TD_W4_OUTROW(1) TD_W4_OUTROW(2) TD_W4_OUTROW(3) TD_W4_OUTROW(4) TD_W4_OUTROW(5) TD_W4_OUTROW(6) TD_W4_OUTROW(7)
#undef TD_W4_OUTROW
#undef TD_W4_OUT
}

__global__ __launch_bounds__(256, 1) void conv_wgrad_wide4_batch_kernel(const WgradParams* __restrict__ jobs, WgradXcdIndex xi) {
  __shared__ __attribute__((aligned(1024))) char w4s0[32768];
  __shared__ __attribute__((aligned(1024))) char w4s1[32768];
  __shared__ __attribute__((aligned(1024))) char w4s2[32768];
  __shared__ __attribute__((aligned(1024))) char w4s3[32768];
  const int xcd = blockIdx.x & 7, slot = blockIdx.x >> 3;
  if (slot >= xi.slots[xcd]) return;
  int lo = xi.start[xcd], hi = xi.start[xcd + 1] - 1;
  while (lo < hi) {
    const int mid = (lo + hi + 1) >> 1;
    if (jobs[mid].first <= slot) lo = mid;
    else hi = mid - 1;
  }
  const WgradParams p = jobs[lo];
  int local = slot - p.first;
  const int bx = local % p.tn;
  local /= p.tn;
  const int by = local % p.tk, bz = local / p.tk;
  if (p.cls & 4) wgrad_wide4_body<true>(p, bx, by, bz, w4s0, w4s1, w4s2, w4s3);
  else wgrad_wide4_body<false>(p, bx, by, bz, w4s0, w4s1, w4s2, w4s3);
}

static int validate(const td_conv_desc* d, int dtype, const char* who) {
  const int vec = dtype == TD_BF16 ? 8 : 4;
  TD_REQUIRE(dtype == TD_F32 || dtype == TD_BF16, "%s: bad dtype %d", who, dtype);
  TD_REQUIRE(d->C % vec == 0, "%s: source channels C=%d must be a multiple of %d (pad them)", who, d->C, vec);
  TD_REQUIRE(d->N > 0 && d->Hs > 0 && d->Ws > 0 && d->Ho > 0 && d->Wo > 0 && d->R > 0 && d->S > 0 && d->stride > 0,
             "%s: bad geometry", who);
  TD_REQUIRE((double)d->N * d->Hs * d->Ws * d->C < 2147483647.0, "%s: source tensor exceeds 2^31 elements", who);
  TD_REQUIRE(!d->aniso || (d->mode == 0 && d->stride_w >= 1 && d->pad_w >= 0 && d->out_sp <= 1), "%s: anisotropic stride / padding is a forward-only geometry", who);
  return TD_OK;
}

}

using namespace td;

static thread_local unsigned long long* g_dbg = nullptr;
static int persist_min_tiles() {
  static const int v = [] { const char* e = getenv("TD_PW_PERSIST_MIN"); return e ? atoi(e) : 4; }();
  return v;
}
extern "C" int td_debug_set_stamp_buffer(unsigned long long* buf) { g_dbg = buf; return TD_OK; }

struct WeightSubset {
  int w_ld;
  int ntap;
  int wtap[4];
  size_t w_bytes;
};
static int conv_gemm_launch(const void* src, const void* wmat, void* out, const td_conv_desc* d, const td_epilogue* e, int dtype,
                            td_stream_t stream, const WeightSubset* sub);

static int conv_dgrad_s2_by_parity(const void* g, const void* w_dgrad, void* dx, const td_conv_desc* d, const td_epilogue* e, int dtype,
                                   td_stream_t stream) {
  const int Hg = d->Hs, Wg = d->Ws, Co = d->C, H = d->Ho, W = d->Wo;
  const size_t es = 2, wbytes = (size_t)d->Nc * 9 * Co * es;
  for (int ph = 0; ph < 2; ++ph)
    for (int pw = 0; pw < 2; ++pw) {
      const int nr = ph ? 2 : 1, ns = pw ? 2 : 1;
      const int rmap[2] = {ph ? 2 : 1, 0}, smap[2] = {pw ? 2 : 1, 0};
      td_conv_desc c = {d->N, Hg, Wg, Co, Hg, Wg, nr, ns, 1, 0, 0, d->Nc, d->ldc, 2, H, W};
      WeightSubset sub;
      memset(&sub, 0, sizeof(sub));
      sub.w_ld = 9 * Co;
      sub.ntap = nr * ns;
      for (int r = 0; r < nr; ++r)
        for (int s_ = 0; s_ < ns; ++s_) sub.wtap[r * ns + s_] = rmap[r] * 3 + smap[s_];
      const size_t ooff = ((size_t)ph * W + pw) * d->ldc * es;
      td_epilogue ec;
      memset(&ec, 0, sizeof(ec));
      if (e) ec = *e;
      if (ec.residual) ec.residual = (const char*)ec.residual + ooff;
      if (ec.mask_src) ec.mask_src = (const char*)ec.mask_src + ooff;
      const char* wp = (const char*)w_dgrad;
      if (sub.ntap == 1) {
        wp += (size_t)sub.wtap[0] * Co * es;
        sub.wtap[0] = 0;
      }
      sub.w_bytes = wbytes - (size_t)(wp - (const char*)w_dgrad);
      const int rc = conv_gemm_launch(g, wp, (char*)dx + ooff, &c, &ec, dtype, stream, &sub);
      if (rc) return rc;
    }
  return TD_OK;
}

extern "C" int td_conv_gemm(const void* src, const void* wmat, void* out, const td_conv_desc* d, const td_epilogue* e,
                            int dtype, td_stream_t stream) {
  TD_REQUIRE(src && wmat && out && d, "td_conv_gemm: null pointer");
  static const int parity = [] { const char* e_ = getenv("TD_DGRAD_S2_PARITY"); return e_ ? atoi(e_) : 1; }();
  if (parity && dtype == TD_BF16 && d->mode == 1 && d->stride == 2 && d->R == 3 && d->S == 3 && d->pad == 1 && !d->aniso && d->out_sp <= 1 &&
      d->Ho == 2 * d->Hs && d->Wo == 2 * d->Ws && d->C % 64 == 0 && d->ldc >= d->Nc && !(e && (e->dropout_p > 0.f || e->sigmoid))) {
    int rc = validate(d, dtype, "td_conv_gemm");
    if (rc) return rc;
    return conv_dgrad_s2_by_parity(src, wmat, out, d, e, dtype, stream);
  }
  return conv_gemm_launch(src, wmat, out, d, e, dtype, stream, nullptr);
}

static int conv_gemm_launch(const void* src, const void* wmat, void* out, const td_conv_desc* d, const td_epilogue* e, int dtype,
                            td_stream_t stream, const WeightSubset* sub) {
  TD_REQUIRE(src && wmat && out && d, "td_conv_gemm: null pointer");
  int rc = validate(d, dtype, "td_conv_gemm");
  if (rc) return rc;
  GemmParams p;
  memset(&p, 0, sizeof(p));
  p.src = (const char*)src;
  p.w = (const char*)wmat;
  p.out = (char*)out;
  p.d = *d;
  if (p.d.out_sp < 1) p.d.out_sp = 1;
  p.M = d->N * d->Ho * d->Wo;
  p.K = d->R * d->S * d->C;
  {
    const double es = dtype == TD_BF16 ? 2.0 : 4.0;
    const double sb = (double)d->N * d->Hs * d->Ws * d->C * es, wb = (double)d->Nc * p.K * es;
    TD_REQUIRE(sb < 4294967000.0 && wb < 4294967000.0, "td_conv_gemm: operand exceeds the 4 GiB buffer-descriptor range");
    p.src_bytes = (uint32_t)sb;
    p.w_bytes = (uint32_t)wb;
  }
  if (sub) {
    p.w_ld = sub->w_ld;
    p.w_bytes = (uint32_t)sub->w_bytes;
    p.use_wtap = sub->ntap > 1;
    for (int i = 0; i < 4; ++i) p.wtap[i] = sub->wtap[i];
  }
  p.alpha = 1.f;
  p.dbg = g_dbg;
  if (e) {
    p.bias = e->bias;
    p.residual = (const char*)e->residual;
    p.mask_src = (const char*)e->mask_src;
    p.relu = e->relu;
    p.sigmoid = e->sigmoid;
    if (e->alpha != 0.f) p.alpha = e->alpha;
    if (e->dropout_p > 0.f) {
      TD_REQUIRE(e->dropout_p < 1.f, "td_conv_gemm: dropout_p must be < 1");
      p.drop_thresh = (uint32_t)((double)e->dropout_p * 4294967296.0);
      if (p.drop_thresh == 0) p.drop_thresh = 1;
      p.drop_scale = 1.f / (1.f - e->dropout_p);
      p.seed = e->dropout_seed;
      p.seed_dev = e->dropout_counter;
    }
  }
  TD_REQUIRE(d->ldc >= d->Nc, "td_conv_gemm: ldc < Nc");
  hipStream_t st = (hipStream_t)stream;
  static const int n_cu = [] {
    int dev = 0, cus = 256;
    if (hipGetDevice(&dev) == hipSuccess) (void)hipDeviceGetAttribute(&cus, hipDeviceAttributeMultiprocessorCount, dev);
    return cus;
  }();
  {
    static const int persist = [] { const char* e_ = getenv("TD_PW_PERSIST"); return e_ ? atoi(e_) : 1; }();
    static const int persist_dropout = [] { const char* e_ = getenv("TD_PW_PERSIST_DROPOUT"); return e_ ? atoi(e_) : 1; }();
    const bool pw0 = d->R == 1 && d->S == 1 && d->pad == 0 && p.d.out_sp == 1 && !d->aniso &&
                     ((d->stride == 1 && d->Hs == d->Ho && d->Ws == d->Wo) ||
                      (d->stride > 1 && d->mode == 0 && (d->Ho - 1) * d->stride < d->Hs && (d->Wo - 1) * d->stride < d->Ws));
    const int NTp = d->Nc / 128, Pp = 2 * n_cu / 8;
    const bool shape_ok = pw0 && !p.w_ld && dtype == TD_BF16 && p.K % 64 == 0 && p.K <= 256 && d->Nc % 128 == 0 &&
                          (NTp == 1 || NTp == 2 || NTp == 4 || NTp == 8 || NTp == 16) && Pp >= NTp && d->ldc % 8 == 0 && !p.sigmoid &&
                          p.alpha == 1.f && n_cu % 8 == 0 && (!p.drop_thresh || persist_dropout) && (double)p.M * d->ldc < 2147483000.0;
    const int MTp = cdiv(p.M, 64);
    const int groups = shape_ok ? 8 * (Pp / NTp) : 1;
    if (persist && shape_ok && MTp >= persist_min_tiles() * groups && !(persist == 2 && p.mask_src) && !(persist == 3 && d->mode != 0)) {
      const bool prof_ = prof_on();
      if (prof_) {
        prof_begin(TD_PROF_PW_RESIDENT, dtype, 2.0 * p.M * d->Nc * p.K, st, p.M, d->Nc, p.K, d->R, d->stride, d->mode);
        const double es_ = 2.0;
        double by = ((double)p.M * p.K + (double)d->Nc * p.K + (double)p.M * d->Nc) * es_;
        if (p.residual) by += (double)p.M * d->Nc * es_;
        if (p.mask_src) by += (double)p.M * d->Nc * es_;
        prof_set_bytes(by);
      }
      const int nkt = p.K / 64;
      const bool hr = p.residual != nullptr, hm = p.mask_src != nullptr;
      dim3 g2(2 * n_cu);
#define TD_PWR(NK)                                                                               \
  do {                                                                                           \
    if (hr && hm) pw_resident2_kernel<NK, true, true><<<g2, 256, 0, st>>>(p, MTp, Pp);          \
    else if (hr) pw_resident2_kernel<NK, true, false><<<g2, 256, 0, st>>>(p, MTp, Pp);          \
    else if (hm) pw_resident2_kernel<NK, false, true><<<g2, 256, 0, st>>>(p, MTp, Pp);          \
    else pw_resident2_kernel<NK, false, false><<<g2, 256, 0, st>>>(p, MTp, Pp);                 \
  } while (0)
      if (nkt == 1) TD_PWR(1);
      else if (nkt == 2) TD_PWR(2);
      else if (nkt == 3) TD_PWR(3);
      else TD_PWR(4);
#undef TD_PWR
      if (prof_) prof_end(st);
      return check_launch("td_conv_gemm(pw_resident)");
    }
  }
  const bool narrow = d->Nc <= 64;
  const int tiles128 = cdiv(p.M, 128) * cdiv(d->Nc, 128);
  const bool small_m = !narrow && (tiles128 < 512 || p.K <= 512);
  const int BMsel = small_m ? 64 : 128, BNsel = narrow ? 64 : 128;
  const int MT = cdiv(p.M, BMsel), NTl = cdiv(d->Nc, BNsel);
  dim3 grid(8 * cdiv(MT, 8) * NTl);
  const bool prof = prof_on();
  const bool pw = d->R == 1 && d->S == 1 && d->stride == 1 && d->pad == 0 && p.d.out_sp == 1 && d->Hs == d->Ho && d->Ws == d->Wo;
  static const int tu_on = [] { const char* e_ = getenv("TD_CONV_TAP_UNIFORM"); return e_ ? atoi(e_) : 1; }();
  const int bk = dtype == TD_BF16 ? 64 : 32;
  const bool tu = (tu_on || p.use_wtap) && !pw && !d->aniso && (d->R * d->S > 1 || (d->stride > 1 && d->mode == 0)) && d->R * d->S <= 32 && d->C % bk == 0 &&
                  (p.d.out_sp == 1 || d->mode == 0) && (d->mode == 0 || d->stride == 1);
  TD_REQUIRE(tu || !p.use_wtap, "td_conv_gemm: a weight-column subset needs the tap-uniform addressing (C %% %d == 0, at most 32 taps)", bk);
  {
    static const int big_on = [] { const char* e_ = getenv("TD_CONV_BIG"); return e_ ? atoi(e_) : 1; }();
    static const int big_min = [] { const char* e_ = getenv("TD_CONV_BIG_MIN_WG"); return e_ ? atoi(e_) : 160; }();
    const int bnb = d->Nc % 256 == 0 ? 256 : 128;
    const int wgs = cdiv(p.M, 256) * (d->Nc / bnb);
    if (big_on && dtype == TD_BF16 && (pw || tu) && p.d.out_sp == 1 && !p.use_wtap && !p.w_ld && d->Nc % 128 == 0 && p.K % 64 == 0 && p.K >= 512 && d->ldc % 8 == 0 && !p.sigmoid &&
        !p.drop_thresh && wgs >= big_min && (double)p.M * d->ldc < 2147483000.0 &&
        p.K <= 64 * 154 && p.M < (1 << 24)) {
      if (prof) {
        prof_begin(tu ? TD_PROF_GEMM_256 : TD_PROF_GEMM_256_PW, dtype, 2.0 * p.M * d->Nc * p.K, st, p.M, d->Nc, p.K, d->R, d->stride, d->mode);
        double by = ((double)d->N * d->Hs * d->Ws * d->C + (double)d->Nc * p.K + (double)p.M * d->Nc) * 2.0;
        if (p.residual) by += (double)p.M * d->Nc * 2.0;
        if (p.mask_src) by += (double)p.M * d->Nc * 2.0;
        prof_set_bytes(by);
      }
      static const int tap_inner = [] { const char* e_ = getenv("TD_CONV_TAP_INNER"); return e_ ? atoi(e_) : 1; }();
      p.tap_inner = tu && tap_inner && d->R * d->S > 1;
      dim3 gb(8 * cdiv(cdiv(p.M, 256), 8) * (d->Nc / bnb));
      static const int persist8 = [] { const char* e_ = getenv("TD_CONV_BIG_PERSIST"); return e_ ? atoi(e_) : 1; }();
      if (bnb == 256) {
        const dim3 gp(persist8 && n_cu % 8 == 0 ? std::min((unsigned)n_cu, gb.x) : gb.x);
        if (tu && p.residual) conv_gemm_big8_kernel<true, true><<<gp, 512, 0, st>>>(p);
        else if (tu) conv_gemm_big8_kernel<true, false><<<gp, 512, 0, st>>>(p);
        else if (p.residual) conv_gemm_big8_kernel<false, true><<<gp, 512, 0, st>>>(p);
        else conv_gemm_big8_kernel<false, false><<<gp, 512, 0, st>>>(p);
      } else {
        if (tu) conv_gemm_big8n_kernel<true><<<gb, 512, 0, st>>>(p);
        else conv_gemm_big8n_kernel<false><<<gb, 512, 0, st>>>(p);
      }
      if (prof) prof_end(st);
      return check_launch("td_conv_gemm(256-row tiles)");
    }
  }
  if (prof) prof_begin(narrow ? TD_PROF_GEMM_128x64 : (small_m ? TD_PROF_GEMM_64x128 : TD_PROF_GEMM_128x128), dtype, 2.0 * p.M * d->Nc * p.K, st, p.M, d->Nc, p.K, d->R, d->stride, d->mode);
  if (prof) {
    const double es = dtype == TD_BF16 ? 2.0 : 4.0;
    const double rows_out = d->out_sp > 1 ? (double)d->N * d->out_H * d->out_W : (double)p.M;
    double by = ((double)d->N * d->Hs * d->Ws * d->C + (double)d->Nc * p.K + (double)p.M * d->Nc) * es;
    if (e && e->residual) by += rows_out * d->Nc * es;
    if (e && e->mask_src) by += rows_out * d->Nc * es;
    prof_set_bytes(by);
  }
#define TD_LAUNCH(TT, BMv, BNv)                                                                   \
  do {                                                                                            \
    if (pw) conv_gemm_kernel<TT, BMv, BNv, 2, true><<<grid, 256, 0, st>>>(p);                    \
    else if (tu) conv_gemm_kernel<TT, BMv, BNv, 2, false, true><<<grid, 256, 0, st>>>(p);        \
    else conv_gemm_kernel<TT, BMv, BNv, 2, false><<<grid, 256, 0, st>>>(p);                      \
  } while (0)
  static const int deep = [] { const char* e_ = getenv("TD_CONV_DEEP"); return e_ ? atoi(e_) : 1; }();
  const bool deep_ok = deep && small_m && (int)grid.x <= 2 * 256 && p.K >= 1024;
  if (dtype == TD_BF16) {
    if (narrow) TD_LAUNCH(u16, 128, 64);
    else if (deep_ok && pw) conv_gemm_kernel<u16, 64, 128, 3, true><<<grid, 256, 0, st>>>(p);
    else if (deep_ok && tu) conv_gemm_kernel<u16, 64, 128, 3, false, true><<<grid, 256, 0, st>>>(p);
    else if (deep_ok) conv_gemm_kernel<u16, 64, 128, 3, false><<<grid, 256, 0, st>>>(p);
    else if (small_m) TD_LAUNCH(u16, 64, 128);
    else TD_LAUNCH(u16, 128, 128);
  } else {
    if (narrow) TD_LAUNCH(float, 128, 64);
    else if (small_m) TD_LAUNCH(float, 64, 128);
    else TD_LAUNCH(float, 128, 128);
  }
#undef TD_LAUNCH
  if (prof) prof_end(st);
  return check_launch("td_conv_gemm");
}

extern "C" int td_linear_ex(const void* a1, const void* a2, const void* wmat, void* out, const td_linear_ex_desc* x, const td_epilogue* e,
                            int dtype, td_stream_t stream) {
  TD_REQUIRE(a1 && wmat && out && x, "td_linear_ex: null pointer");
  TD_REQUIRE(dtype == TD_F32 || dtype == TD_BF16, "td_linear_ex: bad dtype %d", dtype);
  const int vec = dtype == TD_BF16 ? 8 : 4, bk = dtype == TD_BF16 ? 64 : 32;
  const int es = dtype == TD_BF16 ? 2 : 4;
  const int K2 = a2 ? x->K2 : 0;
  TD_REQUIRE(x->M >= 1 && x->N >= 1 && x->K1 >= vec && K2 >= 0, "td_linear_ex: bad sizes");
  TD_REQUIRE(x->K1 % vec == 0 && K2 % vec == 0 && x->lda1 % vec == 0 && (!a2 || x->lda2 % vec == 0), "td_linear_ex: K1 / K2 / lda must be multiples of %d", vec);
  TD_REQUIRE(!a2 || x->K1 % bk == 0, "td_linear_ex: with a second source K1=%d must be a multiple of the K tile (%d)", x->K1, bk);
  TD_REQUIRE(x->lda1 >= x->K1 && (!a2 || x->lda2 >= K2) && x->ldc >= x->N, "td_linear_ex: row stride smaller than the row");
  TD_REQUIRE(x->rows1 >= 1 && (!a2 || x->rows2 >= 1) && (x->a1_map || x->rows1 >= x->M) && (!a2 || x->a2_map || x->rows2 >= x->M),
             "td_linear_ex: source has fewer rows than M and no row map");
  GemmParams p;
  memset(&p, 0, sizeof(p));
  p.src = (const char*)a1;
  p.src2 = (const char*)a2;
  p.w = (const char*)wmat;
  p.out = (char*)out;
  p.M = x->M;
  p.K = x->K1 + K2;
  p.K1 = x->K1;
  p.lda1 = x->lda1;
  p.lda2 = a2 ? x->lda2 : 0;
  p.ldr = x->ldr > 0 ? x->ldr : x->ldc;
  p.w_shared = (a2 && x->w_shared) ? 1 : 0;
  TD_REQUIRE(!p.w_shared || K2 == x->K1, "td_linear_ex: a shared weight needs K2 == K1");
  p.a1_map = x->a1_map;
  p.a2_map = a2 ? x->a2_map : nullptr;
  p.out_map = x->out_map;
  p.res_map = x->res_map;
  td_conv_desc d;
  memset(&d, 0, sizeof(d));
  d.N = 1; d.Hs = x->M; d.Ws = 1; d.C = p.K; d.Ho = x->M; d.Wo = 1; d.R = d.S = 1; d.stride = 1; d.Nc = x->N; d.ldc = x->ldc; d.out_sp = 1;
  p.d = d;
  {
    const double b1 = (double)x->rows1 * x->lda1 * es, b2 = a2 ? (double)x->rows2 * x->lda2 * es : 16.0, wb = (double)x->N * (p.w_shared ? x->K1 : p.K) * es;
    TD_REQUIRE(b1 < 4294967000.0 && b2 < 4294967000.0 && wb < 4294967000.0, "td_linear_ex: operand exceeds the 4 GiB buffer-descriptor range");
    p.src_bytes = (uint32_t)b1;
    p.src2_bytes = (uint32_t)b2;
    p.w_bytes = (uint32_t)wb;
  }
  p.alpha = 1.f;
  if (e) {
    p.bias = e->bias;
    p.residual = (const char*)e->residual;
    p.mask_src = (const char*)e->mask_src;
    p.relu = e->relu;
    p.sigmoid = e->sigmoid;
    if (e->alpha != 0.f) p.alpha = e->alpha;
    if (e->dropout_p > 0.f) {
      TD_REQUIRE(e->dropout_p < 1.f, "td_linear_ex: dropout_p must be < 1");
      p.drop_thresh = (uint32_t)((double)e->dropout_p * 4294967296.0);
      if (p.drop_thresh == 0) p.drop_thresh = 1;
      p.drop_scale = 1.f / (1.f - e->dropout_p);
      p.seed = e->dropout_seed;
      p.seed_dev = e->dropout_counter;
    }
  }
  hipStream_t st = (hipStream_t)stream;
  const bool narrow = x->N <= 64;
  const int tiles128 = cdiv(p.M, 128) * cdiv(x->N, 128);
  const bool small_m = !narrow && (tiles128 < 512 || p.K <= 512);
  const int BMsel = small_m ? 64 : 128, BNsel = narrow ? 64 : 128;
  dim3 grid(8 * cdiv(cdiv(p.M, BMsel), 8) * cdiv(x->N, BNsel));
  const bool prof = prof_on();
  if (prof) {
    prof_begin(narrow ? TD_PROF_GEMM_128x64 : (small_m ? TD_PROF_GEMM_64x128 : TD_PROF_GEMM_128x128), dtype, 2.0 * p.M * x->N * p.K, st, p.M, x->N, p.K, 1, 1, 2);
    double by = ((double)p.M * p.K + (double)x->N * p.K + (double)p.M * x->N) * es;
    if (p.residual) by += (double)p.M * x->N * es;
    if (p.mask_src) by += (double)p.M * x->N * es;
    prof_set_bytes(by);
  }
#define TD_LX(TT)                                                                                     \
  do {                                                                                                \
    if (narrow) conv_gemm_kernel<TT, 128, 64, 2, true, false, true><<<grid, 256, 0, st>>>(p);         \
    else if (small_m) conv_gemm_kernel<TT, 64, 128, 2, true, false, true><<<grid, 256, 0, st>>>(p);   \
    else conv_gemm_kernel<TT, 128, 128, 2, true, false, true><<<grid, 256, 0, st>>>(p);               \
  } while (0)
  if (dtype == TD_BF16) TD_LX(u16);
  else TD_LX(float);
#undef TD_LX
  if (prof) prof_end(st);
  return check_launch("td_linear_ex");
}

static int wgrad_stages() {
  static const int nstg = [] { const char* e = getenv("TD_WGRAD_STAGES"); return (e && atoi(e) == 2) ? 2 : 4; }();
  return nstg;
}

static int wgrad_fill(WgradParams& p, const void* g, const void* src, const td_conv_desc* d, int ldg, int dtype, int* splits_io,
                      int auto_mode, const char* who) {
  int rc = validate(d, dtype, who);
  if (rc) return rc;
  const int vec = dtype == TD_BF16 ? 8 : 4;
  TD_REQUIRE(d->mode == 0 && !d->aniso, "%s: isotropic forward geometry expected", who);
  TD_REQUIRE(d->Nc % vec == 0 && ldg % vec == 0, "%s: Nc=%d / ldg=%d must be multiples of %d", who, d->Nc, ldg, vec);
  memset(&p, 0, sizeof(p));
  p.g = (const char*)g;
  p.src = (const char*)src;
  p.d = *d;
// ... 237 lines not shown
```

### tubedetr_amd/functional.py

```python
from __future__ import annotations

import math
from typing import Optional

import torch
from torch.autograd import Function

from . import ops

Tensor = torch.Tensor

_EPOCH = [0]


def invalidate_prepared():
    _EPOCH[0] += 1


class _PrepEntry:
    __slots__ = ("base_ref", "offset", "shape", "bn", "dtype", "need_dgrad", "cpad", "co_alloc", "res", "ver", "dims")


class _PrepRegistry:

# ... 184 lines not shown
def _arm():
    with _DEFER_LOCK:
        if _ARMED[0]:
            return
        _ARMED[0] = True
    torch.autograd.Variable._execution_engine.queue_callback(_flush_deferred_wgrads)


def _wgrad(g: Tensor, x: Tensor, defer: bool, *, want_bias: bool, out: Optional[Tensor] = None, dbias: Optional[Tensor] = None,
           x2: Optional[Tensor] = None):
    M, K = x.shape
    N = g.shape[1]
    dev = g.device
    if not defer:
        db = dbias if dbias is not None else (ops.zeros_f32(N, dev) if want_bias else None)
        dW = ops.linear_wgrad(g, x, out=out, dbias=db)
        if x2 is not None:
            ops.linear_wgrad(g, x2, out=dW)
        return dW, db
    dW = out if out is not None else torch.empty((N, K), dtype=torch.float32, device=dev)
    db = dbias if dbias is not None else (torch.empty(N, dtype=torch.float32, device=dev) if want_bias else None)
    with _DEFER_LOCK:
        _DEFER_JOBS.append((g, x, dW.data_ptr(), db.data_ptr() if db is not None else None))
        if x2 is not None:
            _DEFER_JOBS.append((g, x2, dW.data_ptr(), None, True))
    return dW, db


class LinearFn(Function):

    @staticmethod
    def forward(ctx, x, W, b, relu: bool, dropout_p: float, seed: int):
        _note_use(ctx.needs_input_grad[1], W, b)
        N = W.shape[0]
        vec = ops.vec_of(x.dtype)
        Np = ops.pad_to(N, vec)
        wf, wd, _, _ = prepared(W, x.dtype, pad_out=Np if Np != N else 0)
        bias = b.detach() if b is not None else None
        if bias is not None and Np != N:
            bias = torch.cat([bias, bias.new_zeros(Np - N)])
        y = ops.linear_fwd(x, wf, bias, relu=relu, dropout_p=dropout_p, seed=seed)
        ctx.save_for_backward(x, y if (relu or dropout_p > 0) else None, wd)
        ctx.cfg = (relu, dropout_p, seed, N, Np, b is not None)
        ctx.params = (W, b)
        return y[:, :N].contiguous() if Np != N else y

    @staticmethod
    def backward(ctx, dy):
        _arm()
        x, y, wd = ctx.saved_tensors
        relu, p, seed, N, Np, has_b = ctx.cfg
        dy = dy.contiguous()
        if Np != N:
            g = dy.new_zeros((dy.shape[0], Np))
            g[:, :N] = dy
            dy = g
        if relu:
            g = ops.relu_bwd(dy, y, 1.0 / (1.0 - p) if p > 0 else 1.0)
        elif p > 0:
            g = ops.dropout(dy, p, seed)
        else:
            g = dy
        dx = ops.linear_fwd(g, wd) if ctx.needs_input_grad[0] else None
        want_w, want_b = ctx.needs_input_grad[1], has_b and ctx.needs_input_grad[2]
        dW = db = None
        if want_w:
            dW_full, db_full = _wgrad(g, x, _can_defer(*ctx.params), want_bias=want_b)
            dW = dW_full[:N]
            db = db_full[:N] if want_b else None
        elif want_b:
            db = ops.colsum(g)[:N]
        return dx, dW, db, None, None, None


def linear(x, W, b=None, relu=False, dropout_p=0.0, training=False):
    p = dropout_p if training else 0.0
    return LinearFn.apply(x, W, b, relu, p, _seed() if p > 0 else 0)


class FFNFn(Function):

    @staticmethod
    def forward(ctx, x, W1, b1, W2, b2, p: float, seed1: int, seed2: int):
        _note_use(ctx.needs_input_grad[1], W1, b1, W2, b2)
        w1f, w1d, _, _ = prepared(W1, x.dtype)
        w2f, w2d, _, _ = prepared(W2, x.dtype)
        h = ops.linear_fwd(x, w1f, b1.detach(), relu=True, dropout_p=p, seed=seed1)
        y = ops.linear_fwd(h, w2f, b2.detach(), dropout_p=p, seed=seed2)
        ctx.save_for_backward(x, h, w1d, w2d)
        ctx.cfg = (p, seed1, seed2)
        ctx.params = (W1, b1, W2, b2)
        return y

    @staticmethod
    def backward(ctx, dy):
        _arm()
        x, h, w1d, w2d = ctx.saved_tensors
        p, seed1, seed2 = ctx.cfg
        defer = _can_defer(*ctx.params)
        g2 = ops.dropout(dy.contiguous(), p, seed2) if p > 0 else dy.contiguous()
        dW2, db2 = _wgrad(g2, h, defer, want_bias=True)
        dh = ops.linear_fwd(g2, w2d, mask_src=h, alpha=1.0 / (1.0 - p) if p > 0 else 1.0)
        dW1, db1 = _wgrad(dh, x, defer, want_bias=True)
        dx = ops.linear_fwd(dh, w1d) if ctx.needs_input_grad[0] else None
        return dx, dW1, db1, dW2, db2, None, None, None


def ffn(x, W1, b1, W2, b2, dropout_p=0.0, training=False):
    p = dropout_p if training else 0.0
    return FFNFn.apply(x, W1, b1, W2, b2, p, _seed() if p > 0 else 0, _seed() if p > 0 else 0)


class AddLayerNormFn(Function):

    @staticmethod
    def forward(ctx, x, r, gamma, beta, eps: float):
        y, s, mean, rstd = ops.add_layernorm_fwd(x, r, gamma.detach(), beta.detach(), eps)
        ctx.save_for_backward(s, mean, rstd, gamma.detach())
        ctx.has_r = r is not None
        return y

    @staticmethod
    def backward(ctx, dy):
        s, mean, rstd, gamma = ctx.saved_tensors
        ds, dg, db = ops.add_layernorm_bwd(dy.contiguous(), s, mean, rstd, gamma)
        return ds, (ds if ctx.has_r else None), dg, db, None


def add_layernorm(x, r, gamma, beta, eps=1e-5):
    return AddLayerNormFn.apply(x, r, gamma, beta, eps)


class AddFn(Function):

    @staticmethod
    def forward(ctx, a, b):
        return ops.add(a, b)

    @staticmethod
    def backward(ctx, g):
        return g, g


class MHAFn(Function):

    @staticmethod
    def forward(ctx, q_in, q_pos, k_in, v_in, W_in, b_in, W_out, b_out, key_pad, B, Lq, Lk, H, need_w, p_attn, seed_attn, p_out, seed_out):
        _note_use(ctx.needs_input_grad[4], W_in, b_in, W_out, b_out)
        E = q_in.shape[1]
        dt = q_in.dtype
        same_qk = k_in is None
        bi = b_in.detach()

        def proj(x_, w_, b_):
            return ops.linear_ex(x_, w_, b_, a2=q_pos, w_shared=True) if q_pos is not None else ops.linear_fwd(x_, w_, b_)

        if same_qk:
            wqk_f, wqk_d, _, _ = prepared(W_in[: 2 * E], dt)
            qk = proj(q_in, wqk_f, bi[: 2 * E]).view(B, Lq, 2 * E)
            q, k = qk[..., :E], qk[..., E:]
            wd_list = (wqk_d,)
        else:
            wq_f, wq_d, _, _ = prepared(W_in[:E], dt)
            wk_f, wk_d, _, _ = prepared(W_in[E : 2 * E], dt)
            q = proj(q_in, wq_f, bi[:E]).view(B, Lq, E)
            k = ops.linear_fwd(k_in, wk_f, bi[E : 2 * E]).view(B, Lk, E)
            wd_list = (wq_d, wk_d)
        wv_f, wv_d, _, _ = prepared(W_in[2 * E :], dt)
        v = ops.linear_fwd(v_in, wv_f, bi[2 * E :]).view(B, Lk, E)
        scale = 1.0 / math.sqrt(E // H)
        lean = not need_w and ops.mha_lean_ok(q, k, v, H)
        if lean:
            ctxv, probs, kp = ops.mha_lean_fwd(q, k, v, key_pad, H, scale, dropout_p=p_attn, seed=seed_attn)
            wavg = None
        else:
            ctxv, probs, wavg = ops.mha_fwd(q, k, v, key_pad, H, scale, need_wavg=need_w, dropout_p=p_attn, seed=seed_attn)
            kp = None
        wo_f, wo_d, _, _ = prepared(W_out, dt)
        out = ops.linear_fwd(ctxv.view(B * Lq, E), wo_f, b_out.detach(), dropout_p=p_out, seed=seed_out)
        ctx.save_for_backward(q_in, q_pos, k_in, v_in, q, k, v, probs, ctxv, wv_d, wo_d, *wd_list)
        ctx.lean, ctx.kp = lean, kp
        ctx.cfg = (B, Lq, Lk, H, E, same_qk, scale, p_attn, seed_attn, p_out, seed_out)
        ctx.params = (W_in, b_in, W_out, b_out)
        return out, (wavg if need_w else None)

    @staticmethod
    def backward(ctx, dout, dwavg):
        _arm()
        q_in, q_pos, k_in, v_in, q, k, v, probs, ctxv, wv_d, wo_d, *wd_list = ctx.saved_tensors
        B, Lq, Lk, H, E, same_qk, scale, p_attn, seed_attn, p_out, seed_out = ctx.cfg
        dt = q_in.dtype
        dev = q_in.device
        defer = _can_defer(*ctx.params)
        g = ops.dropout(dout.contiguous(), p_out, seed_out) if p_out > 0 else dout.contiguous()
        if defer:
            dW_in = torch.empty((3 * E, E), dtype=torch.float32, device=dev)
            db_in = torch.empty(3 * E, dtype=torch.float32, device=dev)
        else:
            dW_in = ops.zeros_f32((3 * E, E), dev)
            db_in = ops.zeros_f32(3 * E, dev)
        dW_out, db_out = _wgrad(g, ctxv.view(B * Lq, E), defer, want_bias=True)
        dctx = ops.linear_fwd(g, wo_d).view(B, Lq, E)
        if same_qk:
            dqk = torch.empty((B, Lq, 2 * E), dtype=dt, device=dev)
            dq, dk = dqk[..., :E], dqk[..., E:]
        else:
            dq = torch.empty((B, Lq, E), dtype=dt, device=dev)
            dk = torch.empty((B, Lk, E), dtype=dt, device=dev)
        dv = torch.empty((B, Lk, E), dtype=dt, device=dev)
        dwa = dwavg.contiguous().float() if dwavg is not None else None
        if ctx.lean:
            ops.mha_lean_bwd(q, k, v, ctx.kp, ctxv, dctx, probs, H, scale, dq, dk, dv, dropout_p=p_attn, seed=seed_attn)
        else:
            ops.mha_bwd(q, k, v, dctx, probs, dwa, H, scale, dq, dk, dv, dropout_p=p_attn, seed=seed_attn)
        dv2 = dv.view(B * Lk, E)
        _wgrad(dv2, v_in, defer, want_bias=True, out=dW_in[2 * E :], dbias=db_in[2 * E :])
        d_v_in = ops.linear_fwd(dv2, wv_d) if ctx.needs_input_grad[3] else None
        d_q_in = d_k_in = None
        need_q = ctx.needs_input_grad[0] or (q_pos is not None and ctx.needs_input_grad[1])
        if same_qk:
            dqk2 = dqk.view(B * Lq, 2 * E)
            _wgrad(dqk2, q_in, defer, want_bias=True, out=dW_in[: 2 * E], dbias=db_in[: 2 * E], x2=q_pos)
            if need_q:
                d_q_in = ops.linear_fwd(dqk2, wd_list[0])
        else:
            dq2, dk2 = dq.view(B * Lq, E), dk.view(B * Lk, E)
            _wgrad(dq2, q_in, defer, want_bias=True, out=dW_in[:E], dbias=db_in[:E], x2=q_pos)
            _wgrad(dk2, k_in, defer, want_bias=True, out=dW_in[E : 2 * E], dbias=db_in[E : 2 * E])
            if need_q:
                d_q_in = ops.linear_fwd(dq2, wd_list[0])
            if ctx.needs_input_grad[2]:
                d_k_in = ops.linear_fwd(dk2, wd_list[1])
        return (d_q_in if ctx.needs_input_grad[0] else None, d_q_in if (q_pos is not None and ctx.needs_input_grad[1]) else None, d_k_in, d_v_in,
                dW_in, db_in, dW_out, db_out) + (None,) * 10


class _CrossKVShared:

    def __init__(self, mem, pos, n_layers, E):
        self.mem, self.pos, self.n_layers, self.E = mem, pos, n_layers, E
        self.dK = self.dV = None
        self.written = set()
        self.wk_d = self.wv_d = None

    def grads(self, like):
        if self.dK is None:
            self.dK = torch.empty((self.mem.shape[0], self.n_layers * self.E), dtype=like.dtype, device=like.device)
            self.dV = torch.empty_like(self.dK)
        return self.dK, self.dV


class CrossKVFn(Function):

    @staticmethod
    def forward(ctx, mem, pos, shared, *w_and_b):
        E, dt = shared.E, mem.dtype
        Ws, bs = w_and_b[0::2], w_and_b[1::2]
        kf, vf, kd, vd = [], [], [], []
        for W in Ws:
            f, d_, _, _ = prepared(W[E : 2 * E], dt)
            kf.append(f); kd.append(d_)
            f, d_, _, _ = prepared(W[2 * E :], dt)
            vf.append(f); vd.append(d_)
        bk = torch.cat([b.detach()[E : 2 * E] for b in bs])
        bv = torch.cat([b.detach()[2 * E :] for b in bs])
        wk = torch.cat(kf, dim=0)
        K_all = ops.linear_ex(mem, wk, bk, a2=pos, w_shared=True) if pos is not None else ops.linear_fwd(mem, wk, bk)
        V_all = ops.linear_fwd(mem, torch.cat(vf, dim=0), bv)
        shared.wk_d, shared.wv_d = torch.cat(kd, dim=1), torch.cat(vd, dim=1)
        ctx.shared = shared
        ctx.set_materialize_grads(False)
        return K_all, V_all

    @staticmethod
    def backward(ctx, gK, gV):
        sh = ctx.shared
        assert gK is None and gV is None, "the consumers of CrossKVFn hand their gradients over through the shared buffers"
        if sh.dK is None:
            return (None,) * (3 + 2 * sh.n_layers)
        for l in range(sh.n_layers):
            if l not in sh.written:
                sh.dK[:, l * sh.E : (l + 1) * sh.E].zero_()
                sh.dV[:, l * sh.E : (l + 1) * sh.E].zero_()
        d_mem = d_pos = None
        need_pos = sh.pos is not None and ctx.needs_input_grad[1]
        if ctx.needs_input_grad[0] or need_pos:
            d_k = ops.linear_fwd(sh.dK, sh.wk_d)
            if need_pos:
                d_pos = d_k
            if ctx.needs_input_grad[0]:
                d_mem = ops.linear_fwd(sh.dV, sh.wv_d, residual=d_k, out=None if need_pos else d_k)
        return (d_mem, d_pos, None) + (None,) * (2 * sh.n_layers)


class MHAPreKVFn(Function):

    @staticmethod
    def forward(ctx, q_in, q_pos, K_all, V_all, W_in, b_in, W_out, b_out, key_pad, shared, layer, B, Lq, Lk, H, need_w, p_attn, seed_attn, p_out, seed_out):
        _note_use(ctx.needs_input_grad[4], W_in, b_in, W_out, b_out)
        E = q_in.shape[1]
        dt = q_in.dtype
        nl = shared.n_layers
        wq_f, wq_d, _, _ = prepared(W_in[:E], dt)
        if q_pos is not None:
            q = ops.linear_ex(q_in, wq_f, b_in.detach()[:E], a2=q_pos, w_shared=True).view(B, Lq, E)
        else:
            q = ops.linear_fwd(q_in, wq_f, b_in.detach()[:E]).view(B, Lq, E)
        k = K_all.view(B, Lk, nl * E)[..., layer * E : (layer + 1) * E]
        v = V_all.view(B, Lk, nl * E)[..., layer * E : (layer + 1) * E]
        scale = 1.0 / math.sqrt(E // H)
        ctxv, probs, wavg = ops.mha_fwd(q, k, v, key_pad, H, scale, need_wavg=need_w, dropout_p=p_attn, seed=seed_attn)
        wo_f, wo_d, _, _ = prepared(W_out, dt)
        out = ops.linear_fwd(ctxv.view(B * Lq, E), wo_f, b_out.detach(), dropout_p=p_out, seed=seed_out)
        ctx.save_for_backward(q_in, q_pos, q, K_all, V_all, probs, ctxv, wq_d, wo_d)
        ctx.cfg = (B, Lq, Lk, H, E, scale, p_attn, seed_attn, p_out, seed_out, layer)
        ctx.params = (W_in, b_in, W_out, b_out)
        ctx.shared = shared
# ... 371 lines not shown
```

### tubedetr_amd/models/transformer.py

```python
from __future__ import annotations

import copy
import math
import os
from typing import List, Optional

import torch
from torch import Tensor, nn

from .. import functional as Fk
from .. import ops as _ops
from ..util.misc import LRUCache
from .position_encoding import TimeEmbeddingLearned, TimeEmbeddingSine

FAST_MODES_IN_HIP = ("",)
FAST_MODES = ("", "gating", "transformer", "pool", "noslow")


class MultiheadAttention(nn.Module):

    def __init__(self, embed_dim: int, num_heads: int, dropout: float = 0.0):
        super().__init__()
        self.embed_dim, self.num_heads, self.dropout = embed_dim, num_heads, dropout
        self.in_proj_weight = nn.Parameter(torch.empty(3 * embed_dim, embed_dim))
        self.in_proj_bias = nn.Parameter(torch.zeros(3 * embed_dim))
        self.out_proj = nn.Linear(embed_dim, embed_dim)
        nn.init.xavier_uniform_(self.in_proj_weight)
        nn.init.constant_(self.out_proj.bias, 0.0)

    def run_prekv(self, q_in, kv, layer, key_pad, B, Lq, Lk, need_weights, out_dropout, training, q_pos=None):
        return Fk.multihead_attention_prekv(q_in, kv, layer, self.in_proj_weight, self.in_proj_bias, self.out_proj.weight, self.out_proj.bias, key_pad,
                                            B, Lq, Lk, self.num_heads, need_weights, attn_dropout=self.dropout, out_dropout=out_dropout, training=training,
                                            q_pos=q_pos)

    def run_q1(self, q_in, anchor, key_pad, F, S, need_weights, out_dropout, training, q_pos=None):
        return Fk.multihead_attention_q1(q_in, anchor, self.in_proj_weight, self.in_proj_bias, self.out_proj.weight, self.out_proj.bias, key_pad,
                                         F, S, self.num_heads, need_weights, attn_dropout=self.dropout, out_dropout=out_dropout, training=training,
                                         q_pos=q_pos)

    def run(self, q_in, k_in, v_in, key_pad, B, Lq, Lk, need_weights, out_dropout, training, q_pos=None):
        return Fk.multihead_attention(q_in, k_in, v_in, self.in_proj_weight, self.in_proj_bias, self.out_proj.weight,
                                      self.out_proj.bias, key_pad, B, Lq, Lk, self.num_heads, need_weights,
                                      attn_dropout=self.dropout, out_dropout=out_dropout, training=training, q_pos=q_pos)


class TransformerEncoderLayer(nn.Module):
    def __init__(self, d_model, nhead, dim_feedforward=2048, dropout=0.1, activation="relu"):
        super().__init__()
        if activation != "relu":
            raise NotImplementedError("only the reference default activation (relu) is fused in the HIP FFN")
        self.self_attn = MultiheadAttention(d_model, nhead, dropout=dropout)
        self.linear1 = nn.Linear(d_model, dim_feedforward)
        self.linear2 = nn.Linear(dim_feedforward, d_model)
        self.norm1 = nn.LayerNorm(d_model)
        self.norm2 = nn.LayerNorm(d_model)
        self.p = dropout

    def forward(self, src: Tensor, pos: Optional[Tensor], key_pad: Optional[Tensor], B: int, S: int) -> Tensor:
        a, _ = self.self_attn.run(src, None, src, key_pad, B, S, S, False, self.p, self.training, q_pos=pos)
        src = Fk.add_layernorm(a, src, self.norm1.weight, self.norm1.bias, self.norm1.eps)
        f = Fk.ffn(src, self.linear1.weight, self.linear1.bias, self.linear2.weight, self.linear2.bias, self.p, self.training)
        return Fk.add_layernorm(f, src, self.norm2.weight, self.norm2.bias, self.norm2.eps)


class TransformerEncoder(nn.Module):
    def __init__(self, encoder_layer, num_layers, norm=None, return_weights=False):
        super().__init__()
        self.layers = nn.ModuleList([copy.deepcopy(encoder_layer) for _ in range(num_layers)])
        self.num_layers = num_layers
        self.norm = norm
        self.return_weights = return_weights

    def forward(self, src, key_pad, pos, B, S):
        out = src
        for layer in self.layers:
            out = layer(out, pos, key_pad, B, S)
        if self.norm is not None:
            out = Fk.add_layernorm(out, None, self.norm.weight, self.norm.bias, self.norm.eps)
        return out


class TransformerDecoderLayer(nn.Module):
    def __init__(self, d_model, nhead, dim_feedforward=2048, dropout=0.1, activation="relu", no_tsa=False):
        super().__init__()
        if activation != "relu":
            raise NotImplementedError("only relu")
        self.self_attn = MultiheadAttention(d_model, nhead, dropout=dropout)
        self.cross_attn_image = MultiheadAttention(d_model, nhead, dropout=dropout)
        self.linear1 = nn.Linear(d_model, dim_feedforward)
        self.linear2 = nn.Linear(dim_feedforward, d_model)
        self.norm1 = nn.LayerNorm(d_model)
        self.norm3 = nn.LayerNorm(d_model)
        self.norm4 = nn.LayerNorm(d_model)
        self.p = dropout
        self.no_tsa = no_tsa

    def forward(self, tgt, query_pos, mem, pos, query_mask, memory_mask, b: int, t: int, S: int, kv=None, index: int = 0):
        if self.no_tsa:
            a, w = self.self_attn.run(tgt, None, tgt, None, b * t, 1, 1, True, self.p, self.training, q_pos=query_pos)
        else:
            a, w = self.self_attn.run(tgt, None, tgt, query_mask, b, t, t, True, self.p, self.training, q_pos=query_pos)
        tgt = Fk.add_layernorm(a, tgt, self.norm1.weight, self.norm1.bias, self.norm1.eps)
        if isinstance(kv, tuple) and len(kv) == 2:
            a, cw = self.cross_attn_image.run_q1(tgt, kv, memory_mask, b * t, S, True, self.p, self.training, q_pos=query_pos)
        elif kv is not None:
            a, cw = self.cross_attn_image.run_prekv(tgt, kv, index, memory_mask, b * t, 1, S, True, self.p, self.training, q_pos=query_pos)
        else:
            mem_k = Fk.AddFn.apply(mem, pos) if pos is not None else mem
            a, cw = self.cross_attn_image.run(tgt, mem_k, mem, memory_mask, b * t, 1, S, True, self.p, self.training, q_pos=query_pos)
        tgt = Fk.add_layernorm(a, tgt, self.norm3.weight, self.norm3.bias, self.norm3.eps)
        f = Fk.ffn(tgt, self.linear1.weight, self.linear1.bias, self.linear2.weight, self.linear2.bias, self.p, self.training)
        tgt = Fk.add_layernorm(f, tgt, self.norm4.weight, self.norm4.bias, self.norm4.eps)
        return tgt, w, cw


class TransformerDecoder(nn.Module):
    def __init__(self, decoder_layer, num_layers, norm=None, return_intermediate=False, return_weights=False):
        super().__init__()
        self.layers = nn.ModuleList([copy.deepcopy(decoder_layer) for _ in range(num_layers)])
        self.num_layers = num_layers
        self.norm = norm
        self.return_intermediate = return_intermediate
        self.return_weights = return_weights

    def forward(self, tgt, query_pos, mem, pos, query_mask, memory_mask, b, t, S):
        inter, ws, cws = [], [], []
        out = tgt
        att = self.layers[0].cross_attn_image
        if (os.environ.get("TD_CROSS_Q1", "1") != "0" and att.embed_dim == 256 and att.num_heads == 8 and S <= 320
                and not (pos is not None and pos.requires_grad)):
            kv = Fk.cross_q1_memory(mem, pos)
        else:
            kv = Fk.cross_kv(mem, pos, [l.cross_attn_image for l in self.layers]) if os.environ.get("TD_KV_HOIST", "1") != "0" else None
        for i, layer in enumerate(self.layers):
            out, w, cw = layer(out, query_pos, mem, pos, query_mask, memory_mask, b, t, S, kv=kv, index=i)
            if self.return_intermediate:
                inter.append(Fk.add_layernorm(out, None, self.norm.weight, self.norm.bias, self.norm.eps))
                ws.append(w)
                cws.append(cw)
        if not self.return_intermediate:
            out = Fk.add_layernorm(out, None, self.norm.weight, self.norm.bias, self.norm.eps) if self.norm is not None else out
            return (out, w, cw) if self.return_weights else out
        hs = torch.stack(inter)
        if not self.return_weights:
            return hs
        return hs, torch.stack(ws), torch.stack(cws)


class FeatureResizer(nn.Module):

    def __init__(self, input_feat_size, output_feat_size, dropout, do_ln=True):
        super().__init__()
        self.do_ln = do_ln
        self.fc = nn.Linear(input_feat_size, output_feat_size, bias=True)
        self.layer_norm = nn.LayerNorm(output_feat_size, eps=1e-12)
        self.p = dropout

    def forward(self, rows: Tensor) -> Tensor:
        x = Fk.linear(rows, self.fc.weight, self.fc.bias)
        if self.do_ln:
            x = Fk.add_layernorm(x, None, self.layer_norm.weight, self.layer_norm.bias, self.layer_norm.eps)
        return Fk.dropout(x, self.p, self.training)


class HashTokenizer:

    def batch_encode_plus(self, text: List[str], padding="longest", return_tensors="pt"):
        import zlib

        from transformers import BatchEncoding

        rows = [[0] + [3 + zlib.crc32(w.encode()) % 49990 for w in s.split()] + [2] for s in text]
        L = max(len(r) for r in rows)
        ids = torch.tensor([r + [1] * (L - len(r)) for r in rows], dtype=torch.long)
        att = torch.tensor([[1] * len(r) + [0] * (L - len(r)) for r in rows], dtype=torch.long)
        be = BatchEncoding({"input_ids": ids, "attention_mask": att})
        be._encodings = [None] * len(text)
        return be


def _load_text_encoder(name: str):
    import os
    import warnings

    from transformers import RobertaConfig, RobertaModel, RobertaTokenizerFast

    try:
        tok = RobertaTokenizerFast.from_pretrained(name, local_files_only=True)
        enc = RobertaModel.from_pretrained(name, local_files_only=True)
        return tok, enc
    except Exception as exc:
        if os.environ.get("TD_ALLOW_RANDOM_TEXT_ENCODER", "0") != "1":
            raise RuntimeError(
                f"text encoder {name!r} could not be loaded ({type(exc).__name__}: {exc}); the reference needs the pretrained "
                "files too.  For synthetic benchmarks / tests without them set TD_ALLOW_RANDOM_TEXT_ENCODER=1 (random-init "
# ... 292 lines not shown
```

### tubedetr_amd/ops.py

```python
from __future__ import annotations

import os

import ctypes as C
from typing import Optional, Tuple

import torch

from . import _hip
from ._hip import ConvDesc, Epilogue, check, dtype_code, ptr, stream_ptr

Tensor = torch.Tensor


class _ZeroArena:

    def __init__(self, chunk: int):
        self.chunk = chunk
        self.buf = None
        self.off = 0

    def take(self, shape, device) -> torch.Tensor:
        n = 1
        for d_ in shape:
            n *= int(d_)
        n_al = (n + 63) // 64 * 64
        if self.buf is None or self.buf.device != device or self.off + n_al > self.buf.numel():
            self.buf = torch.zeros(max(self.chunk, n_al), dtype=torch.float32, device=device)
            self.off = 0
        out = self.buf[self.off : self.off + n].view(shape)
        self.off += n_al
        return out


_ARENAS: dict = {}
_CAPTURE_ARENAS: dict = {}


def reset_capture_arena() -> None:
    _CAPTURE_ARENAS.clear()


_USE_ARENA = __import__("os").environ.get("TD_ZERO_ARENA", "1") != "0"


def zeros_f32(shape, device) -> torch.Tensor:
    if not _USE_ARENA:
        return torch.zeros(shape, dtype=torch.float32, device=device)
    shape = tuple(shape) if not isinstance(shape, int) else (shape,)
    if device.type == "cuda" and torch.cuda.is_current_stream_capturing():
        sp = stream_ptr()
        if sp not in _CAPTURE_ARENAS:
            _CAPTURE_ARENAS[sp] = _ZeroArena(256 * 1024)
        return _CAPTURE_ARENAS[sp].take(shape, device)
    if _CAPTURE_ARENAS:
        _CAPTURE_ARENAS.clear()
    key = (str(device), stream_ptr() if device.type == "cuda" else 0)
    arena = _ARENAS.get(key)
    if arena is None:
        arena = _ARENAS[key] = _ZeroArena(32 * 1024 * 1024)
    return arena.take(shape, device)


def vec_of(dt: torch.dtype) -> int:
    return 8 if dt == torch.bfloat16 else 4


def pad_to(n: int, m: int) -> int:
    return (n + m - 1) // m * m


def conv_out(h: int, k: int, stride: int, pad: int) -> int:
    return (h + 2 * pad - k) // stride + 1


def _desc(N, Hs, Ws, Cs, Ho, Wo, R, S, stride, pad, mode, Nc, ldc, out_sp=1, out_H=0, out_W=0, stride_w=None, pad_w=None) -> ConvDesc:
    if stride_w is None and pad_w is None:
        return ConvDesc(N, Hs, Ws, Cs, Ho, Wo, R, S, stride, pad, mode, Nc, ldc, out_sp, out_H, out_W)
    return ConvDesc(N, Hs, Ws, Cs, Ho, Wo, R, S, stride, pad, mode, Nc, ldc, out_sp, out_H, out_W, 1, stride if stride_w is None else stride_w,
                    pad if pad_w is None else pad_w)


_DROPOUT_COUNTER = [None]


def set_dropout_counter(counter: Optional[torch.Tensor]) -> None:
    if counter is not None:
        assert counter.is_cuda and counter.numel() == 1 and counter.element_size() == 4
    _DROPOUT_COUNTER[0] = counter


def _ctr():
    c = _DROPOUT_COUNTER[0]
    return c.data_ptr() if c is not None else None


def _epi(bias=None, residual=None, mask_src=None, relu=False, sigmoid=False, dropout_p=0.0, seed=0, alpha=1.0) -> Epilogue:
    return Epilogue(ptr(bias), ptr(residual), ptr(mask_src), int(relu), int(sigmoid), float(dropout_p), int(seed) & 0xFFFFFFFF, float(alpha),
                    _ctr() if dropout_p > 0 else None)


def conv_gemm_raw(src: Tensor, w: Tensor, out: Tensor, desc: ConvDesc, epi: Optional[Epilogue]):
    check(_hip.lib().td_conv_gemm(ptr(src), ptr(w), ptr(out), C.byref(desc), C.byref(epi) if epi is not None else None,
                                  dtype_code(src.dtype), stream_ptr()), "td_conv_gemm")


def conv_fwd(x: Tensor, w_fwd: Tensor, bias: Optional[Tensor], R: int, S: int, stride: int, pad: int, *,
             residual: Optional[Tensor] = None, relu: bool = False, out: Optional[Tensor] = None) -> Tensor:
    N, H, W, Cs = x.shape
    Co = w_fwd.shape[0]
    assert w_fwd.shape[1] == R * S * Cs and w_fwd.dtype == x.dtype and x.is_contiguous() and w_fwd.is_contiguous()
    Ho, Wo = conv_out(H, R, stride, pad), conv_out(W, S, stride, pad)
    y = out if out is not None else torch.empty((N, Ho, Wo, Co), dtype=x.dtype, device=x.device)
    conv_gemm_raw(x, w_fwd, y, _desc(N, H, W, Cs, Ho, Wo, R, S, stride, pad, 0, Co, Co), _epi(bias, residual, None, relu))
    return y


def conv_dgrad(g: Tensor, w_dgrad: Tensor, in_hw: Tuple[int, int], R: int, S: int, stride: int, pad: int, *,
               residual: Optional[Tensor] = None, mask_src: Optional[Tensor] = None, out: Optional[Tensor] = None) -> Tensor:
    N, Hg, Wg, Co = g.shape
    H, W = in_hw
    Ci = w_dgrad.shape[0]
    assert w_dgrad.shape[1] == R * S * Co and g.is_contiguous()
    dx = out if out is not None else torch.empty((N, H, W, Ci), dtype=g.dtype, device=g.device)
    conv_gemm_raw(g, w_dgrad, dx, _desc(N, Hg, Wg, Co, H, W, R, S, stride, pad, 1, Ci, Ci), _epi(None, residual, mask_src))
    return dx


def conv1x1s_dgrad_scatter(g: Tensor, w_dgrad: Tensor, dx: Tensor, stride: int, *, mask_src: Optional[Tensor] = None):
    N, Hg, Wg, Co = g.shape
    _, H, W, Ci = dx.shape
    d = _desc(N, Hg, Wg, Co, Hg, Wg, 1, 1, 1, 0, 0, Ci, Ci, stride, H, W)
    conv_gemm_raw(g, w_dgrad, dx, d, _epi(None, dx, mask_src))
    return dx


def conv_wgrad(g: Tensor, x: Tensor, R: int, S: int, stride: int, pad: int, *, out: Optional[Tensor] = None, splits: int = 0) -> Tensor:
    N, H, W, Cs = x.shape
    _, Ho, Wo, Co = g.shape
    dw = out if out is not None else zeros_f32((Co, R * S * Cs), x.device)
    d = _desc(N, H, W, Cs, Ho, Wo, R, S, stride, pad, 0, Co, Co)
    check(_hip.lib().td_conv_wgrad(ptr(g), ptr(x), ptr(dw), C.byref(d), Co, dtype_code(x.dtype), splits, stream_ptr()), "td_conv_wgrad")
    return dw


class _JobTables:

    RING = 12

    def __init__(self):
        self.slots, self.retired, self.cap, self.next = [], [], 0, 0

    def _grow(self, nbytes, device):
        self.cap = max(self.cap, (nbytes + 4095) // 4096 * 4096, 65536)
        self.slots = [s for s in self.slots if s[0].numel() >= self.cap]
        while len(self.slots) < self.RING:
            self.slots.append([torch.empty(self.cap, dtype=torch.uint8, pin_memory=True),
                               torch.empty(self.cap, dtype=torch.uint8, device=device), None])

    def take(self, nbytes: int, device):
        capturing = torch.cuda.is_current_stream_capturing()
        if capturing:
            ok = [s for s in self.slots if s[0].numel() >= nbytes and s[1].device == device]
            if not ok:
                raise RuntimeError("td job tables must exist before a stream capture: run one training step eagerly first")
            slot = ok[0]
            self.slots.remove(slot)
            self.retired.append(slot)
            return slot[0], slot[1], (lambda: None)
        if len(self.slots) < self.RING or self.cap < nbytes:
            self._grow(nbytes, device)
        slot = self.slots[self.next % len(self.slots)]
        self.next += 1
        if slot[2] is not None:
            slot[2].synchronize()

        def done():
            ev = torch.cuda.Event()
            ev.record()
            slot[2] = ev

        return slot[0], slot[1], done


job_tables = _JobTables()


def conv_wgrad_batch(jobs) -> list:
    jobs = list(jobs)
    arr = (_hip.WgradJob * len(jobs))()
    outs = []
    for a, (g, x, R, S, stride, pad, scale, ci_real) in zip(arr, jobs):
        N, H, W, Cs = x.shape
        _, Ho, Wo, Co = g.shape
        assert g.is_contiguous() and x.is_contiguous() and g.dtype == x.dtype
        dw = torch.empty((Co, ci_real, R, S), dtype=torch.float32, device=x.device)
        outs.append(dw)
        a.g, a.src, a.dW, a.scale = g.data_ptr(), x.data_ptr(), dw.data_ptr(), (scale.data_ptr() if scale is not None else None)
        a.d = _desc(N, H, W, Cs, Ho, Wo, R, S, stride, pad, 0, Co, Co)
        a.ldg, a.ci_real, a.dbias = Co, ci_real, None
    nbytes = _hip.lib().td_conv_wgrad_batch_table_bytes(len(jobs))
    th, td_, done = job_tables.take(nbytes, jobs[0][0].device)
    check(_hip.lib().td_conv_wgrad_batch(arr, len(jobs), dtype_code(jobs[0][0].dtype), th.data_ptr(), td_.data_ptr(), nbytes, stream_ptr()),
          "td_conv_wgrad_batch")
    done()
    return outs


def linear_wgrad_batch(jobs) -> None:
    if not jobs:
        return
    key0 = (jobs[0][0].dtype, jobs[0][0].device)
    if any((j[0].dtype, j[0].device) != key0 for j in jobs):
        groups: dict = {}
        for j in jobs:
            groups.setdefault((j[0].dtype, j[0].device), []).append(j)
        for sub in groups.values():
            linear_wgrad_batch(sub)
        return
    arr = (_hip.WgradJob * len(jobs))()
    for a, job in zip(arr, jobs):
        g, x, dw_ptr, db_ptr = job[:4]
        M, K = x.shape
        Nn = g.shape[1]
        assert g.shape[0] == M and g.stride(1) == 1 and x.is_contiguous() and g.dtype == x.dtype
        a.g, a.src, a.dW, a.scale, a.dbias = g.data_ptr(), x.data_ptr(), dw_ptr, None, db_ptr
        a.d = _desc(1, M, 1, K, M, 1, 1, 1, 1, 0, 0, Nn, Nn)
        a.ldg, a.ci_real = g.stride(0), K
        a.accumulate = int(len(job) > 4 and bool(job[4]))
    nbytes = _hip.lib().td_conv_wgrad_batch_table_bytes(len(jobs))
    dev = jobs[0][0].device
    th, td_, done = job_tables.take(nbytes, dev)
    check(_hip.lib().td_conv_wgrad_batch(arr, len(jobs), dtype_code(jobs[0][0].dtype), th.data_ptr(), td_.data_ptr(), nbytes, stream_ptr()),
          "td_conv_wgrad_batch(linears)")
    done()


def linear_fwd(x: Tensor, w: Tensor, bias: Optional[Tensor] = None, *, residual=None, relu=False, sigmoid=False,
               mask_src=None, dropout_p=0.0, seed=0, alpha=1.0, out: Optional[Tensor] = None) -> Tensor:
    M, K = x.shape
    Nn = w.shape[0]
    assert w.shape[1] == K and w.dtype == x.dtype and x.is_contiguous() and w.is_contiguous()
    y = out if out is not None else torch.empty((M, Nn), dtype=x.dtype, device=x.device)
    conv_gemm_raw(x, w, y, _desc(1, M, 1, K, M, 1, 1, 1, 1, 0, 0, Nn, Nn), _epi(bias, residual, mask_src, relu, sigmoid, dropout_p, seed, alpha))
    return y


def pw_chain2(y2: Tensor, w3: Tensor, b3: Tensor, residual: Tensor, w1: Tensor, b1: Tensor, *, out: Optional[Tensor] = None,
              h1: Optional[Tensor] = None) -> Tuple[Tensor, Tensor]:
    M, P = y2.shape
    assert y2.dtype == torch.bfloat16 and w3.shape == (4 * P, P) and w1.shape == (P, 4 * P) and residual.shape == (M, 4 * P)
    assert y2.is_contiguous() and w3.is_contiguous() and w1.is_contiguous() and residual.is_contiguous()
    assert b3.dtype == torch.float32 and b1.dtype == torch.float32 and b3.numel() == 4 * P and b1.numel() == P
    out = out if out is not None else torch.empty((M, 4 * P), dtype=y2.dtype, device=y2.device)
    h1 = h1 if h1 is not None else torch.empty((M, P), dtype=y2.dtype, device=y2.device)
    check(_hip.lib().td_pw_chain2(ptr(y2), ptr(w3), ptr(b3), ptr(residual), ptr(out), ptr(w1), ptr(b1), ptr(h1), M, P, dtype_code(y2.dtype),
                                  stream_ptr()), "td_pw_chain2")
    return out, h1


def _rows2d(t: Tensor):
    assert t.dim() == 2 and t.stride(1) == 1, "row-major 2-D operand expected (unit column stride)"
    return t


def linear_ex(a1: Tensor, w: Tensor, bias: Optional[Tensor] = None, *, a2: Optional[Tensor] = None, a1_map: Optional[Tensor] = None,
              a2_map: Optional[Tensor] = None, w_shared: bool = False, out: Optional[Tensor] = None, out_map: Optional[Tensor] = None,
              out_rows: Optional[int] = None, residual: Optional[Tensor] = None, res_map: Optional[Tensor] = None, relu=False, mask_src=None,
              dropout_p=0.0, seed=0, alpha=1.0) -> Tensor:
    _rows2d(a1)
    K1 = a1.shape[1]
    K2 = _rows2d(a2).shape[1] if a2 is not None else 0
    M = int(a1_map.numel()) if a1_map is not None else a1.shape[0]
    Nn = w.shape[0]
    assert w.is_contiguous() and w.dtype == a1.dtype and w.shape[1] == (K1 if (w_shared or a2 is None) else K1 + K2)
    for m_ in (a1_map, a2_map, out_map, res_map):
        assert m_ is None or (m_.dtype == torch.int32 and m_.is_contiguous() and m_.numel() == M)
    if out is None:
        out = torch.empty((out_rows if out_rows is not None else M, Nn), dtype=a1.dtype, device=a1.device)
    _rows2d(out)
    x = _hip.LinearExDesc()
    x.M, x.N, x.K1, x.K2 = M, Nn, K1, K2
    x.lda1, x.lda2, x.ldc = a1.stride(0), (a2.stride(0) if a2 is not None else 0), out.stride(0)
    x.ldr = _rows2d(residual).stride(0) if residual is not None else 0
    x.w_shared = int(bool(w_shared and a2 is not None))
    x.rows1, x.rows2 = a1.shape[0], (a2.shape[0] if a2 is not None else 0)
    x.a1_map, x.a2_map, x.out_map, x.res_map = ptr(a1_map), ptr(a2_map), ptr(out_map), ptr(res_map)
    epi = _epi(bias, residual, mask_src, relu, False, dropout_p, seed, alpha)
    check(_hip.lib().td_linear_ex(ptr(a1), ptr(a2), ptr(w), ptr(out), C.byref(x), C.byref(epi), dtype_code(a1.dtype), stream_ptr()), "td_linear_ex")
    return out


def rows_copy(src: Tensor, src_map: Optional[Tensor], dst: Tensor, dst_map: Optional[Tensor], n_rows: int, add: Optional[Tensor] = None) -> Tensor:
    _rows2d(src), _rows2d(dst)
    cols = src.shape[1]
    assert dst.shape[1] == cols and dst.dtype == src.dtype and (add is None or (_rows2d(add).shape[1] == cols and add.dtype == src.dtype and add.shape[0] >= n_rows))
    for m_ in (src_map, dst_map):
        assert m_ is None or (m_.dtype == torch.int32 and m_.is_contiguous() and m_.numel() == n_rows)
    check(_hip.lib().td_rows_copy(ptr(src), ptr(src_map), ptr(add), ptr(dst), ptr(dst_map), n_rows, cols, src.stride(0), add.stride(0) if add is not None else 0,
                                  dst.stride(0), dtype_code(src.dtype), stream_ptr()), "td_rows_copy")
    return dst


def rows_segment_sum(inp: Tensor, idx: Tensor, seg_ptr: Tensor, out: Tensor, out_map: Optional[Tensor] = None) -> Tensor:
    _rows2d(inp), _rows2d(out)
    n_out = seg_ptr.numel() - 1
    assert idx.dtype == torch.int32 and seg_ptr.dtype == torch.int32 and out.dtype == inp.dtype and out.shape[1] == inp.shape[1]
    assert out_map is None or (out_map.dtype == torch.int32 and out_map.numel() == n_out)
    check(_hip.lib().td_rows_segment_sum(ptr(inp), ptr(idx), ptr(seg_ptr), ptr(out), ptr(out_map), n_out, inp.shape[1], inp.stride(0), out.stride(0),
                                         dtype_code(inp.dtype), stream_ptr()), "td_rows_segment_sum")
    return out


def linear_wgrad(g: Tensor, x: Tensor, *, out: Optional[Tensor] = None, splits: int = 0, dbias: Optional[Tensor] = None) -> Tensor:
    M, K = x.shape
    Nn = g.shape[1]
    dw = out if out is not None else zeros_f32((Nn, K), x.device)
    d = _desc(1, M, 1, K, M, 1, 1, 1, 1, 0, 0, Nn, Nn)
    if dbias is not None:
        assert dbias.dtype == torch.float32 and dbias.numel() == Nn and dbias.is_contiguous()
    assert g.stride(1) == 1 and x.is_contiguous()
    check(_hip.lib().td_conv_wgrad_bias(ptr(g), ptr(x), ptr(dw), ptr(dbias), C.byref(d), g.stride(0), dtype_code(x.dtype), splits, stream_ptr()),
          "td_conv_wgrad")
    return dw


def weight_prep(W: Tensor, dtype: torch.dtype, *, bn=None, bias: Optional[Tensor] = None, need_dgrad: bool = True, cpad: Optional[int] = None):
    if W.dim() == 2:
        Co, Ci = W.shape
        R = S = 1
    else:
        Co, Ci, R, S = W.shape
    cp = cpad if cpad is not None else pad_to(Ci, vec_of(dtype))
    dev = W.device
    wf = torch.empty((Co, R * S * cp), dtype=dtype, device=dev)
    wd = torch.empty((Ci, R * S * Co), dtype=dtype, device=dev) if need_dgrad else None
    b_out = torch.empty(Co, dtype=torch.float32, device=dev) if (bn is not None or bias is not None) else None
    sc = torch.empty(Co, dtype=torch.float32, device=dev) if bn is not None else None
    bw, bb, brm, brv = bn if bn is not None else (None, None, None, None)
    check(_hip.lib().td_weight_prep(ptr(W), ptr(bw), ptr(bb), ptr(brm), ptr(brv), ptr(bias), Co, Ci, R, S, cp, ptr(wf), ptr(wd),
                                    ptr(b_out), ptr(sc), dtype_code(dtype), stream_ptr()), "td_weight_prep")
    return wf, wd, b_out, sc


def wgrad_finalize(dw_k: Tensor, scale: Optional[Tensor], shape, cpad: int, out: Optional[Tensor] = None, accumulate: bool = False) -> Tensor:
    Co, Ci, R, S = shape
    dW = out if out is not None else torch.empty(shape, dtype=torch.float32, device=dw_k.device)
    check(_hip.lib().td_wgrad_finalize(ptr(dw_k), ptr(scale), ptr(dW), Co, Ci, R, S, cpad, int(accumulate), stream_ptr()), "td_wgrad_finalize")
    return dW


def nchw_to_nhwc(x: Tensor, dtype: torch.dtype, cpad: int) -> Tensor:
    N, Cc, H, W = x.shape
    assert x.dtype == torch.float32 and x.is_contiguous()
    y = torch.empty((N, H, W, cpad), dtype=dtype, device=x.device)
    check(_hip.lib().td_nchw_to_nhwc(ptr(x), ptr(y), N, Cc, H, W, cpad, dtype_code(dtype), stream_ptr()), "td_nchw_to_nhwc")
    return y


def nhwc_to_nchw(x: Tensor) -> Tensor:
    N, H, W, Cc = x.shape
    y = torch.empty((N, Cc, H, W), dtype=torch.float32, device=x.device)
    check(_hip.lib().td_nhwc_to_nchw(ptr(x), ptr(y), N, Cc, H, W, dtype_code(x.dtype), stream_ptr()), "td_nhwc_to_nchw")
    return y


def cast(x: Tensor, dtype: torch.dtype) -> Tensor:
    if x.dtype == dtype:
        return x
    y = torch.empty(x.shape, dtype=dtype, device=x.device)
    check(_hip.lib().td_cast(ptr(x.contiguous()), ptr(y), x.numel(), dtype_code(x.dtype), dtype_code(dtype), stream_ptr()), "td_cast")
    return y


def maxpool3x3s2(x: Tensor) -> Tensor:
    N, H, W, Cc = x.shape
    y = torch.empty((N, conv_out(H, 3, 2, 1), conv_out(W, 3, 2, 1), Cc), dtype=x.dtype, device=x.device)
    check(_hip.lib().td_maxpool3x3s2(ptr(x), ptr(y), N, H, W, Cc, dtype_code(x.dtype), stream_ptr()), "td_maxpool3x3s2")
    return y


def add_layernorm_fwd(x: Tensor, r: Optional[Tensor], gamma: Tensor, beta: Tensor, eps: float, save: bool = True):
    rows, cols = x.shape
    y = torch.empty_like(x)
    s = torch.empty_like(x) if (save and r is not None) else None
    mean = torch.empty(rows, dtype=torch.float32, device=x.device) if save else None
    rstd = torch.empty(rows, dtype=torch.float32, device=x.device) if save else None
    check(_hip.lib().td_add_layernorm_fwd(ptr(x), ptr(r), ptr(gamma), ptr(beta), ptr(y), ptr(s), ptr(mean), ptr(rstd), rows, cols, eps,
                                          dtype_code(x.dtype), stream_ptr()), "td_add_layernorm_fwd")
    return y, (s if r is not None else x), mean, rstd


def add_layernorm_bwd(dy: Tensor, s: Tensor, mean: Tensor, rstd: Tensor, gamma: Tensor, extra: Optional[Tensor] = None):
    rows, cols = dy.shape
    ds = torch.empty_like(dy)
    dgamma = zeros_f32(cols, dy.device)
    dbeta = zeros_f32(cols, dy.device)
    check(_hip.lib().td_add_layernorm_bwd(ptr(dy), ptr(s), ptr(mean), ptr(rstd), ptr(gamma), ptr(extra), ptr(ds), ptr(dgamma), ptr(dbeta),
                                          rows, cols, dtype_code(dy.dtype), stream_ptr()), "td_add_layernorm_bwd")
    return ds, dgamma, dbeta


def colsum(g: Tensor, out: Optional[Tensor] = None) -> Tensor:
    rows, cols = g.shape
    o = out if out is not None else zeros_f32(cols, g.device)
    check(_hip.lib().td_colsum(ptr(g), ptr(o), rows, cols, cols, dtype_code(g.dtype), stream_ptr()), "td_colsum")
    return o


def add(a: Tensor, b: Optional[Tensor]) -> Tensor:
    y = torch.empty_like(a)
    check(_hip.lib().td_add(ptr(a), ptr(b), ptr(y), a.numel(), dtype_code(a.dtype), stream_ptr()), "td_add")
    return y


def relu_bwd(dy: Tensor, y: Tensor, scale: float = 1.0) -> Tensor:
    g = torch.empty_like(dy)
    check(_hip.lib().td_relu_bwd(ptr(dy), ptr(y), ptr(g), dy.numel(), scale, dtype_code(dy.dtype), stream_ptr()), "td_relu_bwd")
    return g


def pos_sine(mask: Tensor, npf: int, dtype: torch.dtype, temperature: float = 10000.0, rows: Optional[int] = None) -> Tensor:
    N, h, w = mask.shape
    m8 = mask.to(torch.uint8).contiguous()
    rows = h * w if rows is None else int(rows)
    pos = torch.empty((N, rows, 2 * npf), dtype=dtype, device=mask.device)
    check(_hip.lib().td_pos_sine(ptr(m8), ptr(pos), N, h, w, npf, temperature, rows, dtype_code(dtype), stream_ptr()), "td_pos_sine")
    return pos


def mha_fwd(q: Tensor, k: Tensor, v: Tensor, key_pad: Optional[Tensor], H: int, scale: float, *, need_wavg: bool = False,
            dropout_p: float = 0.0, seed: int = 0):
    B, Lq, E = q.shape
    Lk = k.shape[1]
    hd = E // H
    for t_ in (q, k, v):
        assert t_.stride(2) == 1 and t_.stride(0) == t_.shape[1] * t_.stride(1)
    out = torch.empty((B, Lq, E), dtype=q.dtype, device=q.device)
    probs = torch.empty((B, H, Lq, Lk), dtype=torch.float32, device=q.device)
    wavg = torch.empty((B, Lq, Lk), dtype=torch.float32, device=q.device) if need_wavg else None
    kp = key_pad.to(torch.uint8).contiguous() if key_pad is not None else None
    check(_hip.lib().td_mha_fwd(ptr(q), ptr(k), ptr(v), ptr(kp), ptr(out), ptr(probs), ptr(wavg), B, H, Lq, Lk, hd, q.stride(1), k.stride(1),
                                v.stride(1), E, scale, dropout_p, seed & 0xFFFFFFFF, _ctr() if dropout_p > 0 else None, dtype_code(q.dtype), stream_ptr()),
          "td_mha_fwd")
    return out, probs, wavg


def mha_lean_ok(q: Tensor, k: Tensor, v: Tensor, H: int) -> bool:
    if os.environ.get("TD_MHA_LEAN", "1") == "0":
        return False
    E = q.shape[2]
    return (q.dtype == torch.bfloat16 and E // H == 32
            and all(t_.stride(1) % 8 == 0 and t_.data_ptr() % 16 == 0 for t_ in (q, k, v)))


def mha_lean_fwd(q: Tensor, k: Tensor, v: Tensor, key_pad: Optional[Tensor], H: int, scale: float, *, dropout_p: float = 0.0, seed: int = 0):
    B, Lq, E = q.shape
    Lk = k.shape[1]
    for t_ in (q, k, v):
        assert t_.stride(2) == 1 and t_.stride(0) == t_.shape[1] * t_.stride(1)
    out = torch.empty((B, Lq, E), dtype=q.dtype, device=q.device)
    stats = torch.empty((B * H * Lq, 4), dtype=torch.float32, device=q.device)
    kp = key_pad.to(torch.uint8).contiguous() if key_pad is not None else None
    check(_hip.lib().td_mha_lean_fwd(ptr(q), ptr(k), ptr(v), ptr(kp), ptr(out), ptr(stats), B, H, Lq, Lk, E // H, q.stride(1), k.stride(1), v.stride(1), E,
                                     scale, dropout_p, seed & 0xFFFFFFFF, _ctr() if dropout_p > 0 else None, dtype_code(q.dtype), stream_ptr()),
          "td_mha_lean_fwd")
    return out, stats, kp


def mha_lean_bwd(q: Tensor, k: Tensor, v: Tensor, kp: Optional[Tensor], out: Tensor, dout: Tensor, stats: Tensor, H: int, scale: float,
                 dq: Tensor, dk: Tensor, dv: Tensor, *, dropout_p: float = 0.0, seed: int = 0):
    B, Lq, E = q.shape
    Lk = k.shape[1]
    assert dout.is_contiguous() and out.is_contiguous()
    for a, b in ((q, dq), (k, dk), (v, dv)):
        assert a.stride() == b.stride() and a.shape == b.shape
    check(_hip.lib().td_mha_lean_bwd(ptr(q), ptr(k), ptr(v), ptr(kp), ptr(out), ptr(dout), ptr(stats), ptr(dq), ptr(dk), ptr(dv), B, H, Lq, Lk, E // H,
                                     q.stride(1), k.stride(1), v.stride(1), E, scale, dropout_p, seed & 0xFFFFFFFF, _ctr() if dropout_p > 0 else None,
                                     dtype_code(q.dtype), stream_ptr()), "td_mha_lean_bwd")
    return dq, dk, dv
# ... 108 lines not shown
```

Baseline: 107.6.

## Fuse residual accumulation into GEMM epilogue and dropout into layernorm backward

Adds an accumulate operand to the conv/linear GEMM epilogues so a residual or gradient sum is added in the store path instead of in a separate add kernel. Adds a layernorm-backward variant that also writes the dropout-masked gradient. Introduces self-attention and FFN block functions that chain these fused ops. This cuts extra elementwise launches and memory passes in encoder and decoder layers, at the cost of more epilogue registers in the big GEMM kernel and an extra bf16 rounding point.

Measured after the change: 107.6. No clear change (-0.0%).

```diff
diff --git a/include/tubedetr_hip.h b/include/tubedetr_hip.h
--- a/include/tubedetr_hip.h
+++ b/include/tubedetr_hip.h
@@ -68,6 +68,9 @@
 int td_conv_gemm(const void* src, const void* wmat, void* out, const td_conv_desc* d, const td_epilogue* e,
                  int dtype, td_stream_t stream);
 
+int td_conv_gemm_accum(const void* src, const void* wmat, void* out, const td_conv_desc* d, const td_epilogue* e,
+                       const void* accum, int dtype, td_stream_t stream);
+
 typedef struct td_linear_ex_desc {
   int M, N, K1, K2;
   int lda1, lda2, ldc, ldr;
@@ -80,6 +83,8 @@
 } td_linear_ex_desc;
 int td_linear_ex(const void* a1, const void* a2, const void* wmat, void* out, const td_linear_ex_desc* x, const td_epilogue* e,
                  int dtype, td_stream_t stream);
+int td_linear_ex_accum(const void* a1, const void* a2, const void* wmat, void* out, const td_linear_ex_desc* x, const td_epilogue* e,
+                       const void* accum, int dtype, td_stream_t stream);
 
 int td_conv_wgrad(const void* g, const void* src, float* dw, const td_conv_desc* d, int ldg, int dtype, int splits,
                   td_stream_t stream);
@@ -157,6 +162,9 @@
 int td_add_layernorm_bwd(const void* dy, const void* s, const float* mean, const float* rstd, const float* gamma,
                          const void* extra, void* ds, float* dgamma, float* dbeta, int rows, int cols, int dtype,
                          td_stream_t stream);
+int td_add_layernorm_bwd_drop(const void* dy, const void* s, const float* mean, const float* rstd, const float* gamma,
+                              const void* extra, void* ds, void* ds_dropped, float* dgamma, float* dbeta, int rows, int cols,
+                              float p, uint32_t seed, const uint32_t* dropout_counter, int dtype, td_stream_t stream);
 
 int td_colsum(const void* g, float* out, int rows, int cols, int ld, int dtype, td_stream_t stream);
 int td_add(const void* a, const void* b, void* y, size_t n, int dtype, td_stream_t stream);
diff --git a/tubedetr_amd/_hip.py b/tubedetr_amd/_hip.py
--- a/tubedetr_amd/_hip.py
+++ b/tubedetr_amd/_hip.py
@@ -68,6 +68,7 @@
     "td_prof_collect": [_I, _I, C.POINTER(C.c_longlong), C.POINTER(C.c_double), C.POINTER(C.c_double)],
     "td_prof_collect_bytes": [_I, _I, C.POINTER(C.c_double)],
     "td_conv_gemm": [_P, _P, _P, C.POINTER(ConvDesc), C.POINTER(Epilogue), _I, _P],
+    "td_conv_gemm_accum": [_P, _P, _P, C.POINTER(ConvDesc), C.POINTER(Epilogue), _P, _I, _P],
     "td_conv_wgrad": [_P, _P, _P, C.POINTER(ConvDesc), _I, _I, _I, _P],
     "td_conv_wgrad_bias": [_P, _P, _P, _P, C.POINTER(ConvDesc), _I, _I, _I, _P],
     "td_conv_wgrad_batch": [C.POINTER(WgradJob), _I, _I, _P, _P, _SZ, _P],
@@ -91,6 +92,7 @@
     "td_maxpool3x3s2": [_P, _P, _I, _I, _I, _I, _I, _P],
     "td_add_layernorm_fwd": [_P, _P, _P, _P, _P, _P, _P, _P, _I, _I, _F, _I, _P],
     "td_add_layernorm_bwd": [_P, _P, _P, _P, _P, _P, _P, _P, _P, _I, _I, _I, _P],
+    "td_add_layernorm_bwd_drop": [_P, _P, _P, _P, _P, _P, _P, _P, _P, _P, _I, _I, _F, _U32, _P, _I, _P],
     "td_colsum": [_P, _P, _I, _I, _I, _I, _P],
     "td_add": [_P, _P, _P, _SZ, _I, _P],
     "td_relu_bwd": [_P, _P, _P, _SZ, _F, _I, _P],
@@ -99,6 +101,7 @@
     "td_dropout": [_P, _P, _SZ, _F, _U32, _P, _I, _P],
     "td_pos_sine": [_P, _P, _I, _I, _I, _I, _F, _I, _I, _P],
     "td_linear_ex": [_P, _P, _P, _P, C.POINTER(LinearExDesc), C.POINTER(Epilogue), _I, _P],
+    "td_linear_ex_accum": [_P, _P, _P, _P, C.POINTER(LinearExDesc), C.POINTER(Epilogue), _P, _I, _P],
     "td_rows_copy": [_P, _P, _P, _P, _P, _I, _I, _I, _I, _I, _I, _P],
     "td_rows_segment_sum": [_P, _P, _P, _P, _P, _I, _I, _I, _I, _I, _P],
     "td_criterion_fwd": [_P, _P, _P, _P, _P, _P, _P, _P, _P, _F, _F, _I, _I, _I, _I, _P, _P, _P, _P, _P, _P],
diff --git a/tubedetr_amd/csrc/elementwise.hip b/tubedetr_amd/csrc/elementwise.hip
--- a/tubedetr_amd/csrc/elementwise.hip
+++ b/tubedetr_amd/csrc/elementwise.hip
@@ -149,7 +149,9 @@
 __global__ __launch_bounds__(256) void add_layernorm_bwd_v4_kernel(const u16* __restrict__ dy, const u16* __restrict__ s, const float* __restrict__ mean,
                                                                    const float* __restrict__ rstd, const float* __restrict__ gamma,
                                                                    const u16* __restrict__ extra, u16* __restrict__ ds, float* dgamma, float* dbeta,
-                                                                   int rows) {
+                                                                   int rows, u16* __restrict__ dsd, uint32_t thresh, float drop_scale, uint32_t seed_in,
+                                                                   const uint32_t* __restrict__ seed_dev) {
+  const uint32_t seed = dsd ? effective_seed(seed_in, seed_dev) : 0u;
   constexpr int cols = NJ * 256;
   const int lane = threadIdx.x & 63;
   const int wid = blockIdx.x * 4 + (threadIdx.x >> 6);
@@ -195,7 +197,15 @@
 #pragma unroll
         for (int e = 0; e < 4; ++e) o[e] += ex[e];
       }
-      *(uint2*)(ds + base + 256 * j) = pack4_bf16(o);
+      const uint2 pk = pack4_bf16(o);
+      *(uint2*)(ds + base + 256 * j) = pk;
+      if (dsd) {
+        float rr[4];
+        unpack4v(pk, rr);
+#pragma unroll
+        for (int e = 0; e < 4; ++e) rr[e] = dropout_keep(seed, (uint32_t)(base + 256 * j + e), thresh) ? rr[e] * drop_scale : 0.f;
+        *(uint2*)(dsd + base + 256 * j) = pack4_bf16(rr);
+      }
     }
   }
   __shared__ float redg[4][cols], redb[4][cols];
@@ -217,7 +227,9 @@
 template <typename T>
 __global__ __launch_bounds__(256) void add_layernorm_bwd_kernel(const T* dy, const T* s, const float* mean, const float* rstd,
                                                                 const float* gamma, const T* extra, T* ds, float* dgamma,
-                                                                float* dbeta, int rows, int cols) {
+                                                                float* dbeta, int rows, int cols, T* dsd, uint32_t thresh, float drop_scale,
+                                                                uint32_t seed_in, const uint32_t* seed_dev) {
+  const uint32_t seed = dsd ? effective_seed(seed_in, seed_dev) : 0u;
   const int lane = threadIdx.x & 63;
   const int wid = blockIdx.x * 4 + (threadIdx.x >> 6);
   const int nw = gridDim.x * 4;
@@ -253,6 +265,12 @@
         float o = rs * (dg[j] - c1 - xh[j] * c2);
         if (extra) o += Elem<T>::load(extra, base + c);
         Elem<T>::store(ds, base + c, o);
+        if (dsd) {
+          T rounded;
+          Elem<T>::store(&rounded, 0, o);
+          const float r = Elem<T>::load(&rounded, 0);
+          Elem<T>::store(dsd, base + c, dropout_keep(seed, (uint32_t)(base + c), thresh) ? r * drop_scale : 0.f);
+        }
       }
     }
   }
@@ -526,27 +544,47 @@
   return check_launch("td_add_layernorm_fwd");
 }
 
+static int add_layernorm_bwd_launch(const void* dy, const void* s, const float* mean, const float* rstd, const float* gamma, const void* extra,
+                                    void* ds, float* dgamma, float* dbeta, int rows, int cols, void* dsd, float p, uint32_t seed_in,
+                                    const uint32_t* seed_dev, int dtype, td_stream_t stream);
 extern "C" int td_add_layernorm_bwd(const void* dy, const void* s, const float* mean, const float* rstd,
                                     const float* gamma, const void* extra, void* ds, float* dgamma, float* dbeta,
                                     int rows, int cols, int dtype, td_stream_t stream) {
+  return add_layernorm_bwd_launch(dy, s, mean, rstd, gamma, extra, ds, dgamma, dbeta, rows, cols, nullptr, 0.f, 0, nullptr, dtype, stream);
+}
+extern "C" int td_add_layernorm_bwd_drop(const void* dy, const void* s, const float* mean, const float* rstd, const float* gamma,
+                                         const void* extra, void* ds, void* ds_dropped, float* dgamma, float* dbeta, int rows, int cols,
+                                         float p, uint32_t seed, const uint32_t* dropout_counter, int dtype, td_stream_t stream) {
+  TD_REQUIRE(ds_dropped, "td_add_layernorm_bwd_drop: null pointer");
+  TD_REQUIRE(p >= 0.f && p < 1.f, "td_add_layernorm_bwd_drop: p out of range");
+  TD_REQUIRE((double)rows * cols < 4294967296.0, "td_add_layernorm_bwd_drop: more than 2^32 elements");
+  return add_layernorm_bwd_launch(dy, s, mean, rstd, gamma, extra, ds, dgamma, dbeta, rows, cols, ds_dropped, p, seed, dropout_counter, dtype, stream);
+}
+static int add_layernorm_bwd_launch(const void* dy, const void* s, const float* mean, const float* rstd, const float* gamma, const void* extra,
+                                    void* ds, float* dgamma, float* dbeta, int rows, int cols, void* dsd, float p, uint32_t seed_in,
+                                    const uint32_t* seed_dev, int dtype, td_stream_t stream) {
+  uint32_t thresh = p > 0.f ? (uint32_t)((double)p * 4294967296.0) : 0u;
+  if (p > 0.f && !thresh) thresh = 1;
+  const float dsc = 1.f / (1.f - p);
+  if (!thresh) seed_dev = nullptr;
   TD_REQUIRE(dy && s && mean && rstd && gamma && ds, "td_add_layernorm_bwd: null pointer");
   TD_REQUIRE(cols <= 64 * LN_MAXJ, "td_add_layernorm_bwd: cols > %d", 64 * LN_MAXJ);
   if (rows == 0) return TD_OK;
   hipStream_t st = (hipStream_t)stream;
   unsigned g = (rows + 3) / 4;
-  if (dtype == TD_BF16 && (cols == 256 || cols == 768) && aligned8(dy, s, ds, extra)) {
+  if (dtype == TD_BF16 && (cols == 256 || cols == 768) && aligned8(dy, s, ds, extra) && ((uintptr_t)dsd & 7) == 0) {
     unsigned gv = (rows + 31) / 32;
     if (gv > 1024) gv = 1024;
     if (deterministic()) gv = 1;
-    if (cols == 256) add_layernorm_bwd_v4_kernel<1><<<gv, 256, 0, st>>>((const u16*)dy, (const u16*)s, mean, rstd, gamma, (const u16*)extra, (u16*)ds, dgamma, dbeta, rows);
-    else add_layernorm_bwd_v4_kernel<3><<<gv, 256, 0, st>>>((const u16*)dy, (const u16*)s, mean, rstd, gamma, (const u16*)extra, (u16*)ds, dgamma, dbeta, rows);
+    if (cols == 256) add_layernorm_bwd_v4_kernel<1><<<gv, 256, 0, st>>>((const u16*)dy, (const u16*)s, mean, rstd, gamma, (const u16*)extra, (u16*)ds, dgamma, dbeta, rows, (u16*)dsd, thresh, dsc, seed_in, seed_dev);
+    else add_layernorm_bwd_v4_kernel<3><<<gv, 256, 0, st>>>((const u16*)dy, (const u16*)s, mean, rstd, gamma, (const u16*)extra, (u16*)ds, dgamma, dbeta, rows, (u16*)dsd, thresh, dsc, seed_in, seed_dev);
     return check_launch("td_add_layernorm_bwd");
   }
   if (g > 256) g = 256;
   if (deterministic()) g = 1;
   TD_DISPATCH(dtype,
-              (add_layernorm_bwd_kernel<u16><<<g, 256, 0, st>>>((const u16*)dy, (const u16*)s, mean, rstd, gamma, (const u16*)extra, (u16*)ds, dgamma, dbeta, rows, cols)),
-              (add_layernorm_bwd_kernel<float><<<g, 256, 0, st>>>((const float*)dy, (const float*)s, mean, rstd, gamma, (const float*)extra, (float*)ds, dgamma, dbeta, rows, cols)),
+              (add_layernorm_bwd_kernel<u16><<<g, 256, 0, st>>>((const u16*)dy, (const u16*)s, mean, rstd, gamma, (const u16*)extra, (u16*)ds, dgamma, dbeta, rows, cols, (u16*)dsd, thresh, dsc, seed_in, seed_dev)),
+              (add_layernorm_bwd_kernel<float><<<g, 256, 0, st>>>((const float*)dy, (const float*)s, mean, rstd, gamma, (const float*)extra, (float*)ds, dgamma, dbeta, rows, cols, (float*)dsd, thresh, dsc, seed_in, seed_dev)),
               "td_add_layernorm_bwd");
   return check_launch("td_add_layernorm_bwd");
 }
diff --git a/tubedetr_amd/csrc/gemm_conv.hip b/tubedetr_amd/csrc/gemm_conv.hip
--- a/tubedetr_amd/csrc/gemm_conv.hip
+++ b/tubedetr_amd/csrc/gemm_conv.hip
@@ -43,6 +43,7 @@
   int w_ld;
   int wtap[4];
   int use_wtap;
+  const char* accum;
 };
 
 template <typename T>
@@ -448,6 +449,12 @@
     }
   }
   asm volatile("s_waitcnt lgkmcnt(0)" ::: "memory");
+  uint4 acm[NIT];
+  if (p.accum && vec_ok) {
+#pragma unroll
+    for (int it = 0; it < NIT; ++it)
+      if (live[it]) acm[it] = ld16(p.accum + (GX ? roffs[it] : offs[it]) * ES);
+  }
   float bias[EPL];
 #pragma unroll
   for (int r = 0; r < EPL; ++r) bias[r] = (p.bias && n + r < d.Nc) ? p.bias[n + r] : 0.f;
@@ -491,7 +498,16 @@
 #pragma unroll
         for (int r = 0; r < EPL; ++r) v[r] = dropout_keep(eff_seed, (uint32_t)(off + r), p.drop_thresh) ? v[r] * p.drop_scale : 0.f;
       }
-      st16(p.out + off * ES, pack16<T>(v));
+      uint4 o = pack16<T>(v);
+      if (p.accum) {
+        float o8[EPL], a8[EPL];
+        unpack16<T>(o, o8);
+        unpack16<T>(acm[it], a8);
+#pragma unroll
+        for (int r = 0; r < EPL; ++r) o8[r] += a8[r];
+        o = pack16<T>(o8);
+      }
+      st16(p.out + off * ES, o);
     } else {
       const int cnt = min(EPL, d.Nc - n);
       for (int r = 0; r < cnt; ++r) {
@@ -501,6 +517,11 @@
         if (p.sigmoid) x = sigmoidf_(x);
         if (p.mask_src) x = Elem<T>::load(p.mask_src, off + r) > 0.f ? x : 0.f;
         if (p.drop_thresh) x = dropout_keep(eff_seed, (uint32_t)(off + r), p.drop_thresh) ? x * p.drop_scale : 0.f;
+        if (p.accum) {
+          T rounded;
+          Elem<T>::store(&rounded, 0, x);
+          x = Elem<T>::load(&rounded, 0) + Elem<T>::load(p.accum, (GX ? roffs[it] : off) + r);
+        }
         Elem<T>::store(p.out, off + r, x);
       }
     }
@@ -535,7 +556,7 @@
 #ifndef TD_BIG8_AUX_X
 #define TD_BIG8_AUX_X 0
 #endif
-template <bool TU, bool RES>
+template <bool TU, bool RES, bool ACC = false>
 __global__ __launch_bounds__(512, 1) void conv_gemm_big8_kernel(GemmParams p) {
   using T = u16;
   constexpr int ES = 2, BM = 256, BN = 256, BK = 64, NW = 8, VEC = 8;
@@ -784,6 +805,7 @@
     }
     TD_STAMP(3);
     uint4 mk[2][2];
+    uint4 ak[ACC ? 2 : 1][2];
     auto seg_off = [&](int j, int h) -> uint32_t {
       const int m = m0 + wy * WM + j * 16 + h * 8 + rsub;
       return m < p.M ? ((uint32_t)m * (uint32_t)d.ldc + (uint32_t)(n0 + wx * WN + cc * 8)) * ES : OOB;
@@ -793,6 +815,15 @@
       for (int h = 0; h < 2; ++h) {
         const uint32_t off = seg_off(j, h);
         mk[b][h] = off != OOB ? ld16(p.mask_src + off) : make_uint4(0, 0, 0, 0);
+      }
+    };
+    auto fetch_acc = [&](int j, int b) {
+      if constexpr (ACC) {
+#pragma unroll
+        for (int h = 0; h < 2; ++h) {
+          const uint32_t off = seg_off(j, h);
+          ak[b][h] = off != OOB ? ld16(p.accum + off) : make_uint4(0, 0, 0, 0);
+        }
       }
     };
     auto put = [&](int j) {
@@ -817,6 +848,7 @@
       }
     };
     if (p.mask_src) fetch_mask(0, 0);
+    fetch_acc(0, 0);
     put(0);
     u32x4_t o0, o1;
     asm volatile("ds_read_b128 %0, %1" : "=v"(o0) : "v"(sra) : "memory");
@@ -826,6 +858,7 @@
       const int b = j & 1;
       if (j + 1 < TM) {
         if (p.mask_src) fetch_mask(j + 1, b ^ 1);
+        fetch_acc(j + 1, b ^ 1);
         put(j + 1);
         asm volatile("s_waitcnt lgkmcnt(4)" : "+v"(o0), "+v"(o1) : : "memory");
       } else {
@@ -848,6 +881,21 @@
         unpack16<T>(mk[b][1], m8);
 #pragma unroll
         for (int r = 0; r < 8; ++r) x8[r] = m8[r] > 0.f ? x8[r] : 0.f;
+        const uint4 q1 = pack16<T>(x8);
+        s1 = u32x4_t{q1.x, q1.y, q1.z, q1.w};
+      }
+      if constexpr (ACC) {
+        float x8[8], a8[8];
+        unpack16<T>(make_uint4(s0.x, s0.y, s0.z, s0.w), x8);
+        unpack16<T>(ak[b][0], a8);
+#pragma unroll
+        for (int r = 0; r < 8; ++r) x8[r] += a8[r];
+        const uint4 q0 = pack16<T>(x8);
+        s0 = u32x4_t{q0.x, q0.y, q0.z, q0.w};
+        unpack16<T>(make_uint4(s1.x, s1.y, s1.z, s1.w), x8);
+        unpack16<T>(ak[b][1], a8);
+#pragma unroll
+        for (int r = 0; r < 8; ++r) x8[r] += a8[r];
         const uint4 q1 = pack16<T>(x8);
         s1 = u32x4_t{q1.x, q1.y, q1.z, q1.w};
       }
@@ -2094,7 +2142,7 @@
   size_t w_bytes;
 };
 static int conv_gemm_launch(const void* src, const void* wmat, void* out, const td_conv_desc* d, const td_epilogue* e, int dtype,
-                            td_stream_t stream, const WeightSubset* sub);
+                            td_stream_t stream, const WeightSubset* sub, const void* accum = nullptr);
 
 static int conv_dgrad_s2_by_parity(const void* g, const void* w_dgrad, void* dx, const td_conv_desc* d, const td_epilogue* e, int dtype,
                                    td_stream_t stream) {
@@ -2129,6 +2177,14 @@
   return TD_OK;
 }
 
+extern "C" int td_conv_gemm_accum(const void* src, const void* wmat, void* out, const td_conv_desc* d, const td_epilogue* e, const void* accum,
+                                  int dtype, td_stream_t stream) {
+  TD_REQUIRE(src && wmat && out && d, "td_conv_gemm_accum: null pointer");
+  if (!accum) return td_conv_gemm(src, wmat, out, d, e, dtype, stream);
+  TD_REQUIRE(d->out_sp <= 1, "td_conv_gemm_accum: dense output rows only");
+  return conv_gemm_launch(src, wmat, out, d, e, dtype, stream, nullptr, accum);
+}
+
 extern "C" int td_conv_gemm(const void* src, const void* wmat, void* out, const td_conv_desc* d, const td_epilogue* e,
                             int dtype, td_stream_t stream) {
   TD_REQUIRE(src && wmat && out && d, "td_conv_gemm: null pointer");
@@ -2143,12 +2199,19 @@
 }
 
 static int conv_gemm_launch(const void* src, const void* wmat, void* out, const td_conv_desc* d, const td_epilogue* e, int dtype,
-                            td_stream_t stream, const WeightSubset* sub) {
+                            td_stream_t stream, const WeightSubset* sub, const void* accum) {
   TD_REQUIRE(src && wmat && out && d, "td_conv_gemm: null pointer");
   int rc = validate(d, dtype, "td_conv_gemm");
   if (rc) return rc;
   GemmParams p;
   memset(&p, 0, sizeof(p));
+  p.accum = (const char*)accum;
+  const bool acc_split_ok = accum && d->ldc == d->Nc && accum != out;
+  auto split_add = [&](const char* what) -> int {
+    const int rc_ = check_launch(what);
+    if (rc_ || !accum) return rc_;
+    return td_add(out, accum, out, (size_t)d->N * d->Ho * d->Wo * d->Nc, dtype, stream);
+  };
   p.src = (const char*)src;
   p.w = (const char*)wmat;
   p.out = (char*)out;
@@ -2206,7 +2269,8 @@
                           p.alpha == 1.f && n_cu % 8 == 0 && (!p.drop_thresh || persist_dropout) && (double)p.M * d->ldc < 2147483000.0;
     const int MTp = cdiv(p.M, 64);
     const int groups = shape_ok ? 8 * (Pp / NTp) : 1;
-    if (persist && shape_ok && MTp >= persist_min_tiles() * groups && !(persist == 2 && p.mask_src) && !(persist == 3 && d->mode != 0)) {
+    if (persist && shape_ok && MTp >= persist_min_tiles() * groups && !(persist == 2 && p.mask_src) && !(persist == 3 && d->mode != 0) &&
+        (!accum || acc_split_ok)) {
       const bool prof_ = prof_on();
       if (prof_) {
         prof_begin(TD_PROF_PW_RESIDENT, dtype, 2.0 * p.M * d->Nc * p.K, st, p.M, d->Nc, p.K, d->R, d->stride, d->mode);
@@ -2232,7 +2296,7 @@
       else TD_PWR(4);
 #undef TD_PWR
       if (prof_) prof_end(st);
-      return check_launch("td_conv_gemm(pw_resident)");
+      return split_add("td_conv_gemm(pw_resident)");
     }
   }
   const bool narrow = d->Nc <= 64;
@@ -2255,7 +2319,8 @@
     const int wgs = cdiv(p.M, 256) * (d->Nc / bnb);
     if (big_on && dtype == TD_BF16 && (pw || tu) && p.d.out_sp == 1 && !p.use_wtap && !p.w_ld && d->Nc % 128 == 0 && p.K % 64 == 0 && p.K >= 512 && d->ldc % 8 == 0 && !p.sigmoid &&
         !p.drop_thresh && wgs >= big_min && (double)p.M * d->ldc < 2147483000.0 &&
-        p.K <= 64 * 154 && p.M < (1 << 24)) {
+        p.K <= 64 * 154 && p.M < (1 << 24) && (!accum || acc_split_ok || (bnb == 256 && !tu && !p.residual))) {
+      const bool acc_native = accum && bnb == 256 && !tu && !p.residual;
       if (prof) {
         prof_begin(tu ? TD_PROF_GEMM_256 : TD_PROF_GEMM_256_PW, dtype, 2.0 * p.M * d->Nc * p.K, st, p.M, d->Nc, p.K, d->R, d->stride, d->mode);
         double by = ((double)d->N * d->Hs * d->Ws * d->C + (double)d->Nc * p.K + (double)p.M * d->Nc) * 2.0;
@@ -2272,13 +2337,14 @@
         if (tu && p.residual) conv_gemm_big8_kernel<true, true><<<gp, 512, 0, st>>>(p);
         else if (tu) conv_gemm_big8_kernel<true, false><<<gp, 512, 0, st>>>(p);
         else if (p.residual) conv_gemm_big8_kernel<false, true><<<gp, 512, 0, st>>>(p);
+        else if (acc_native) conv_gemm_big8_kernel<false, false, true><<<gp, 512, 0, st>>>(p);
         else conv_gemm_big8_kernel<false, false><<<gp, 512, 0, st>>>(p);
       } else {
         if (tu) conv_gemm_big8n_kernel<true><<<gb, 512, 0, st>>>(p);
         else conv_gemm_big8n_kernel<false><<<gb, 512, 0, st>>>(p);
       }
       if (prof) prof_end(st);
-      return check_launch("td_conv_gemm(256-row tiles)");
+      return acc_native ? check_launch("td_conv_gemm(256-row tiles)") : split_add("td_conv_gemm(256-row tiles)");
     }
   }
   if (prof) prof_begin(narrow ? TD_PROF_GEMM_128x64 : (small_m ? TD_PROF_GEMM_64x128 : TD_PROF_GEMM_128x128), dtype, 2.0 * p.M * d->Nc * p.K, st, p.M, d->Nc, p.K, d->R, d->stride, d->mode);
@@ -2315,8 +2381,18 @@
   return check_launch("td_conv_gemm");
 }
 
+static int linear_ex_launch(const void* a1, const void* a2, const void* wmat, void* out, const td_linear_ex_desc* x, const td_epilogue* e,
+                            const void* accum, int dtype, td_stream_t stream);
 extern "C" int td_linear_ex(const void* a1, const void* a2, const void* wmat, void* out, const td_linear_ex_desc* x, const td_epilogue* e,
                             int dtype, td_stream_t stream) {
+  return linear_ex_launch(a1, a2, wmat, out, x, e, nullptr, dtype, stream);
+}
+extern "C" int td_linear_ex_accum(const void* a1, const void* a2, const void* wmat, void* out, const td_linear_ex_desc* x, const td_epilogue* e,
+                                  const void* accum, int dtype, td_stream_t stream) {
+  return linear_ex_launch(a1, a2, wmat, out, x, e, accum, dtype, stream);
+}
+static int linear_ex_launch(const void* a1, const void* a2, const void* wmat, void* out, const td_linear_ex_desc* x, const td_epilogue* e,
+                            const void* accum, int dtype, td_stream_t stream) {
   TD_REQUIRE(a1 && wmat && out && x, "td_linear_ex: null pointer");
   TD_REQUIRE(dtype == TD_F32 || dtype == TD_BF16, "td_linear_ex: bad dtype %d", dtype);
   const int vec = dtype == TD_BF16 ? 8 : 4, bk = dtype == TD_BF16 ? 64 : 32;
@@ -2334,6 +2410,7 @@
   p.src2 = (const char*)a2;
   p.w = (const char*)wmat;
   p.out = (char*)out;
+  p.accum = (const char*)accum;
   p.M = x->M;
   p.K = x->K1 + K2;
   p.K1 = x->K1;
diff --git a/tubedetr_amd/functional.py b/tubedetr_amd/functional.py
--- a/tubedetr_amd/functional.py
+++ b/tubedetr_amd/functional.py
@@ -290,28 +290,38 @@
 
     @staticmethod
     def forward(ctx, x, W1, b1, W2, b2, p: float, seed1: int, seed2: int):
-        _note_use(ctx.needs_input_grad[1], W1, b1, W2, b2)
-        w1f, w1d, _, _ = prepared(W1, x.dtype)
-        w2f, w2d, _, _ = prepared(W2, x.dtype)
-        h = ops.linear_fwd(x, w1f, b1.detach(), relu=True, dropout_p=p, seed=seed1)
-        y = ops.linear_fwd(h, w2f, b2.detach(), dropout_p=p, seed=seed2)
-        ctx.save_for_backward(x, h, w1d, w2d)
-        ctx.cfg = (p, seed1, seed2)
-        ctx.params = (W1, b1, W2, b2)
+        y, saved = _ffn_forward(ctx, ctx.needs_input_grad[1], x, W1, b1, W2, b2, p, seed1, seed2)
+        ctx.save_for_backward(*saved)
         return y
 
     @staticmethod
     def backward(ctx, dy):
-        _arm()
-        x, h, w1d, w2d = ctx.saved_tensors
-        p, seed1, seed2 = ctx.cfg
-        defer = _can_defer(*ctx.params)
+        return _ffn_backward(ctx, ctx.saved_tensors, dy, ctx.needs_input_grad[0]) + (None, None, None)
+
+
+def _ffn_forward(ctx, recording, x, W1, b1, W2, b2, p, seed1, seed2):
+    _note_use(recording, W1, b1, W2, b2)
+    w1f, w1d, _, _ = prepared(W1, x.dtype)
+    w2f, w2d, _, _ = prepared(W2, x.dtype)
+    h = ops.linear_fwd(x, w1f, b1.detach(), relu=True, dropout_p=p, seed=seed1)
+    y = ops.linear_fwd(h, w2f, b2.detach(), dropout_p=p, seed=seed2)
+    ctx.cfg = (p, seed1, seed2)
+    ctx.params = (W1, b1, W2, b2)
+    return y, (x, h, w1d, w2d)
+
+
+def _ffn_backward(ctx, saved, dy, need_dx, g2=None, accum=None):
+    _arm()
+    x, h, w1d, w2d = saved
+    p, seed1, seed2 = ctx.cfg
+    defer = _can_defer(*ctx.params)
+    if g2 is None:
         g2 = ops.dropout(dy.contiguous(), p, seed2) if p > 0 else dy.contiguous()
-        dW2, db2 = _wgrad(g2, h, defer, want_bias=True)
-        dh = ops.linear_fwd(g2, w2d, mask_src=h, alpha=1.0 / (1.0 - p) if p > 0 else 1.0)
-        dW1, db1 = _wgrad(dh, x, defer, want_bias=True)
-        dx = ops.linear_fwd(dh, w1d) if ctx.needs_input_grad[0] else None
-        return dx, dW1, db1, dW2, db2, None, None, None
+    dW2, db2 = _wgrad(g2, h, defer, want_bias=True)
+    dh = ops.linear_fwd(g2, w2d, mask_src=h, alpha=1.0 / (1.0 - p) if p > 0 else 1.0)
+    dW1, db1 = _wgrad(dh, x, defer, want_bias=True)
+    dx = ops.linear_fwd(dh, w1d, accum=accum) if need_dx else None
+    return dx, dW1, db1, dW2, db2
 
 
 def ffn(x, W1, b1, W2, b2, dropout_p=0.0, training=False):
@@ -354,7 +364,14 @@
 
     @staticmethod
     def forward(ctx, q_in, q_pos, k_in, v_in, W_in, b_in, W_out, b_out, key_pad, B, Lq, Lk, H, need_w, p_attn, seed_attn, p_out, seed_out):
-        _note_use(ctx.needs_input_grad[4], W_in, b_in, W_out, b_out)
+        out, wavg, saved = MHAFn.forward_body(ctx, ctx.needs_input_grad[4], q_in, q_pos, k_in, v_in, W_in, b_in, W_out, b_out, key_pad, B, Lq, Lk, H,
+                                              need_w, p_attn, seed_attn, p_out, seed_out)
+        ctx.save_for_backward(*saved)
+        return out, wavg
+
+    @staticmethod
+    def forward_body(ctx, recording, q_in, q_pos, k_in, v_in, W_in, b_in, W_out, b_out, key_pad, B, Lq, Lk, H, need_w, p_attn, seed_attn, p_out, seed_out):
+        _note_use(recording, W_in, b_in, W_out, b_out)
         E = q_in.shape[1]
         dt = q_in.dtype
         same_qk = k_in is None
@@ -386,21 +403,26 @@
             kp = None
         wo_f, wo_d, _, _ = prepared(W_out, dt)
         out = ops.linear_fwd(ctxv.view(B * Lq, E), wo_f, b_out.detach(), dropout_p=p_out, seed=seed_out)
-        ctx.save_for_backward(q_in, q_pos, k_in, v_in, q, k, v, probs, ctxv, wv_d, wo_d, *wd_list)
         ctx.lean, ctx.kp = lean, kp
         ctx.cfg = (B, Lq, Lk, H, E, same_qk, scale, p_attn, seed_attn, p_out, seed_out)
         ctx.params = (W_in, b_in, W_out, b_out)
-        return out, (wavg if need_w else None)
+        return out, (wavg if need_w else None), (q_in, q_pos, k_in, v_in, q, k, v, probs, ctxv, wv_d, wo_d, *wd_list)
 
     @staticmethod
     def backward(ctx, dout, dwavg):
+        nig = ctx.needs_input_grad
+        return MHAFn.backward_body(ctx, ctx.saved_tensors, dout, dwavg, (nig[0], nig[1], nig[2], nig[3])) + (None,) * 10
+
+    @staticmethod
+    def backward_body(ctx, saved, dout, dwavg, need, g=None, fold=None):
         _arm()
-        q_in, q_pos, k_in, v_in, q, k, v, probs, ctxv, wv_d, wo_d, *wd_list = ctx.saved_tensors
+        q_in, q_pos, k_in, v_in, q, k, v, probs, ctxv, wv_d, wo_d, *wd_list = saved
         B, Lq, Lk, H, E, same_qk, scale, p_attn, seed_attn, p_out, seed_out = ctx.cfg
         dt = q_in.dtype
         dev = q_in.device
         defer = _can_defer(*ctx.params)
-        g = ops.dropout(dout.contiguous(), p_out, seed_out) if p_out > 0 else dout.contiguous()
+        if g is None:
+            g = ops.dropout(dout.contiguous(), p_out, seed_out) if p_out > 0 else dout.contiguous()
         if defer:
             dW_in = torch.empty((3 * E, E), dtype=torch.float32, device=dev)
             db_in = torch.empty(3 * E, dtype=torch.float32, device=dev)
@@ -423,9 +445,23 @@
             ops.mha_bwd(q, k, v, dctx, probs, dwa, H, scale, dq, dk, dv, dropout_p=p_attn, seed=seed_attn)
         dv2 = dv.view(B * Lk, E)
         _wgrad(dv2, v_in, defer, want_bias=True, out=dW_in[2 * E :], dbias=db_in[2 * E :])
-        d_v_in = ops.linear_fwd(dv2, wv_d) if ctx.needs_input_grad[3] else None
+        need_x, need_p, need_k, need_v = need
+        need_p = need_p and q_pos is not None
+        if fold is not None:
+            assert same_qk and need_x
+            dqk2 = dqk.view(B * Lq, 2 * E)
+            _wgrad(dqk2, q_in, defer, want_bias=True, out=dW_in[: 2 * E], dbias=db_in[: 2 * E], x2=q_pos)
+            if need_p:
+                d_pos = ops.linear_fwd(dqk2, wd_list[0])
+                t = ops.add(fold, d_pos)
+            else:
+                d_pos = None
+                t = ops.linear_fwd(dqk2, wd_list[0], accum=fold)
+            d_x = ops.linear_fwd(dv2, wv_d, accum=t)
+            return d_x, d_pos, None, None, dW_in, db_in, dW_out, db_out
+        d_v_in = ops.linear_fwd(dv2, wv_d) if need_v else None
         d_q_in = d_k_in = None
-        need_q = ctx.needs_input_grad[0] or (q_pos is not None and ctx.needs_input_grad[1])
+        need_q = need_x or need_p
         if same_qk:
             dqk2 = dqk.view(B * Lq, 2 * E)
             _wgrad(dqk2, q_in, defer, want_bias=True, out=dW_in[: 2 * E], dbias=db_in[: 2 * E], x2=q_pos)
@@ -437,10 +473,92 @@
             _wgrad(dk2, k_in, defer, want_bias=True, out=dW_in[E : 2 * E], dbias=db_in[E : 2 * E])
             if need_q:
                 d_q_in = ops.linear_fwd(dq2, wd_list[0])
-            if ctx.needs_input_grad[2]:
+            if need_k:
                 d_k_in = ops.linear_fwd(dk2, wd_list[1])
-        return (d_q_in if ctx.needs_input_grad[0] else None, d_q_in if (q_pos is not None and ctx.needs_input_grad[1]) else None, d_k_in, d_v_in,
-                dW_in, db_in, dW_out, db_out) + (None,) * 10
+        return (d_q_in if need_x else None, d_q_in if need_p else None, d_k_in, d_v_in, dW_in, db_in, dW_out, db_out)
+
+
+_BLOCK_FUSE = [_os.environ.get("TD_BLOCK_FUSE", "1") != "0"]
+
+
+def set_block_fusion(on: bool) -> None:
+    _BLOCK_FUSE[0] = bool(on)
+
+
+def _ln_bwd_for_block(ctx, ln_saved, dy, p, seed):
+    s, mean, rstd, gamma = ln_saved
+    if p > 0:
+        ds, dg, db, g = ops.add_layernorm_bwd(dy.contiguous(), s, mean, rstd, gamma, drop=(p, seed))
+    else:
+        ds, dg, db = ops.add_layernorm_bwd(dy.contiguous(), s, mean, rstd, gamma)
+        g = ds
+    return ds, g, dg, db
+
+
+class FFNBlockFn(Function):
+
+    @staticmethod
+    def forward(ctx, x, W1, b1, W2, b2, gamma, beta, eps: float, p: float, seed1: int, seed2: int):
+        f, saved = _ffn_forward(ctx, ctx.needs_input_grad[1], x, W1, b1, W2, b2, p, seed1, seed2)
+        y, s, mean, rstd = ops.add_layernorm_fwd(f, x, gamma.detach(), beta.detach(), eps)
+        ctx.save_for_backward(*saved, s, mean, rstd, gamma.detach())
+        return y
+
+    @staticmethod
+    def backward(ctx, dy):
+        saved = ctx.saved_tensors
+        p = ctx.cfg[0]
+        ds, g2, dg, db = _ln_bwd_for_block(ctx, saved[4:], dy, p, ctx.cfg[2])
+        if ctx.needs_input_grad[0]:
+            dx, dW1, db1, dW2, db2 = _ffn_backward(ctx, saved[:4], None, True, g2=g2, accum=ds)
+        else:
+            _, dW1, db1, dW2, db2 = _ffn_backward(ctx, saved[:4], None, False, g2=g2)
+            dx = None
+        return dx, dW1, db1, dW2, db2, dg, db, None, None, None, None
+
+
+class AttnBlockFn(Function):
+
+    @staticmethod
+    def forward(ctx, x, q_pos, W_in, b_in, W_out, b_out, gamma, beta, eps: float, key_pad, B, L, H, need_w, p_attn, seed_attn, p_out, seed_out):
+        a, wavg, saved = MHAFn.forward_body(ctx, ctx.needs_input_grad[2], x, q_pos, None, x, W_in, b_in, W_out, b_out, key_pad, B, L, L, H, need_w,
+                                            p_attn, seed_attn, p_out, seed_out)
+        y, s, mean, rstd = ops.add_layernorm_fwd(a, x, gamma.detach(), beta.detach(), eps)
+        ctx.n_mha = len(saved)
+        ctx.save_for_backward(*saved, s, mean, rstd, gamma.detach())
+        return y, wavg
+
+    @staticmethod
+    def backward(ctx, dy, dwavg):
+        saved = ctx.saved_tensors
+        n = ctx.n_mha
+        p_out, seed_out = ctx.cfg[9], ctx.cfg[10]
+        ds, g, dg, db = _ln_bwd_for_block(ctx, saved[n:], dy, p_out, seed_out)
+        nig = ctx.needs_input_grad
+        if nig[0]:
+            d_x, d_pos, _, _, dW_in, db_in, dW_out, db_out = MHAFn.backward_body(ctx, saved[:n], None, dwavg, (True, nig[1], False, False), g=g, fold=ds)
+        else:
+            _, d_pos, _, _, dW_in, db_in, dW_out, db_out = MHAFn.backward_body(ctx, saved[:n], None, dwavg, (False, nig[1], False, False), g=g)
+            d_x = None
+        return (d_x, d_pos, dW_in, db_in, dW_out, db_out, dg, db) + (None,) * 10
+
+
+def ffn_block(x, W1, b1, W2, b2, gamma, beta, eps, dropout_p=0.0, training=False):
+    if not _BLOCK_FUSE[0]:
+        return add_layernorm(ffn(x, W1, b1, W2, b2, dropout_p, training), x, gamma, beta, eps)
+    p = dropout_p if training else 0.0
+    return FFNBlockFn.apply(x, W1, b1, W2, b2, gamma, beta, eps, p, _seed() if p > 0 else 0, _seed() if p > 0 else 0)
+
+
+def self_attention_block(x, W_in, b_in, W_out, b_out, gamma, beta, eps, key_pad, B, L, H, need_weights=False, attn_dropout=0.0, out_dropout=0.0,
+                         training=False, q_pos=None):
+    if not _BLOCK_FUSE[0]:
+        a, w = multihead_attention(x, None, x, W_in, b_in, W_out, b_out, key_pad, B, L, L, H, need_weights, attn_dropout, out_dropout, training, q_pos)
+        return add_layernorm(a, x, gamma, beta, eps), w
+    pa = attn_dropout if training else 0.0
+    po = out_dropout if training else 0.0
+    return AttnBlockFn.apply(x, q_pos, W_in, b_in, W_out, b_out, gamma, beta, eps, key_pad, B, L, H, need_weights,
+                             pa, _seed() if pa > 0 else 0, po, _seed() if po > 0 else 0)
 
 
 class _CrossKVShared:
diff --git a/tubedetr_amd/models/transformer.py b/tubedetr_amd/models/transformer.py
--- a/tubedetr_amd/models/transformer.py
+++ b/tubedetr_amd/models/transformer.py
@@ -37,6 +37,11 @@
         return Fk.multihead_attention_q1(q_in, anchor, self.in_proj_weight, self.in_proj_bias, self.out_proj.weight, self.out_proj.bias, key_pad,
                                          F, S, self.num_heads, need_weights, attn_dropout=self.dropout, out_dropout=out_dropout, training=training,
                                          q_pos=q_pos)
+
+    def run_self_block(self, x, norm, key_pad, B, L, need_weights, out_dropout, training, q_pos=None):
+        return Fk.self_attention_block(x, self.in_proj_weight, self.in_proj_bias, self.out_proj.weight, self.out_proj.bias, norm.weight, norm.bias,
+                                       norm.eps, key_pad, B, L, self.num_heads, need_weights, attn_dropout=self.dropout, out_dropout=out_dropout,
+                                       training=training, q_pos=q_pos)
 
     def run(self, q_in, k_in, v_in, key_pad, B, Lq, Lk, need_weights, out_dropout, training, q_pos=None):
         return Fk.multihead_attention(q_in, k_in, v_in, self.in_proj_weight, self.in_proj_bias, self.out_proj.weight,
@@ -57,10 +62,9 @@
         self.p = dropout
 
     def forward(self, src: Tensor, pos: Optional[Tensor], key_pad: Optional[Tensor], B: int, S: int) -> Tensor:
-        a, _ = self.self_attn.run(src, None, src, key_pad, B, S, S, False, self.p, self.training, q_pos=pos)
-        src = Fk.add_layernorm(a, src, self.norm1.weight, self.norm1.bias, self.norm1.eps)
-        f = Fk.ffn(src, self.linear1.weight, self.linear1.bias, self.linear2.weight, self.linear2.bias, self.p, self.training)
-        return Fk.add_layernorm(f, src, self.norm2.weight, self.norm2.bias, self.norm2.eps)
+        src, _ = self.self_attn.run_self_block(src, self.norm1, key_pad, B, S, False, self.p, self.training, q_pos=pos)
+        return Fk.ffn_block(src, self.linear1.weight, self.linear1.bias, self.linear2.weight, self.linear2.bias, self.norm2.weight, self.norm2.bias,
+                            self.norm2.eps, self.p, self.training)
 
 
 class TransformerEncoder(nn.Module):
@@ -97,10 +101,9 @@
 
     def forward(self, tgt, query_pos, mem, pos, query_mask, memory_mask, b: int, t: int, S: int, kv=None, index: int = 0):
         if self.no_tsa:
-            a, w = self.self_attn.run(tgt, None, tgt, None, b * t, 1, 1, True, self.p, self.training, q_pos=query_pos)
-        else:
-            a, w = self.self_attn.run(tgt, None, tgt, query_mask, b, t, t, True, self.p, self.training, q_pos=query_pos)
-        tgt = Fk.add_layernorm(a, tgt, self.norm1.weight, self.norm1.bias, self.norm1.eps)
+            tgt, w = self.self_attn.run_self_block(tgt, self.norm1, None, b * t, 1, True, self.p, self.training, q_pos=query_pos)
+        else:
+            tgt, w = self.self_attn.run_self_block(tgt, self.norm1, query_mask, b, t, True, self.p, self.training, q_pos=query_pos)
         if isinstance(kv, tuple) and len(kv) == 2:
             a, cw = self.cross_attn_image.run_q1(tgt, kv, memory_mask, b * t, S, True, self.p, self.training, q_pos=query_pos)
         elif kv is not None:
@@ -109,8 +112,8 @@
             mem_k = Fk.AddFn.apply(mem, pos) if pos is not None else mem
             a, cw = self.cross_attn_image.run(tgt, mem_k, mem, memory_mask, b * t, 1, S, True, self.p, self.training, q_pos=query_pos)
         tgt = Fk.add_layernorm(a, tgt, self.norm3.weight, self.norm3.bias, self.norm3.eps)
-        f = Fk.ffn(tgt, self.linear1.weight, self.linear1.bias, self.linear2.weight, self.linear2.bias, self.p, self.training)
-        tgt = Fk.add_layernorm(f, tgt, self.norm4.weight, self.norm4.bias, self.norm4.eps)
+        tgt = Fk.ffn_block(tgt, self.linear1.weight, self.linear1.bias, self.linear2.weight, self.linear2.bias, self.norm4.weight, self.norm4.bias,
+                           self.norm4.eps, self.p, self.training)
         return tgt, w, cw
 
 
diff --git a/tubedetr_amd/ops.py b/tubedetr_amd/ops.py
--- a/tubedetr_amd/ops.py
+++ b/tubedetr_amd/ops.py
@@ -100,7 +100,11 @@
                     _ctr() if dropout_p > 0 else None)
 
 
-def conv_gemm_raw(src: Tensor, w: Tensor, out: Tensor, desc: ConvDesc, epi: Optional[Epilogue]):
+def conv_gemm_raw(src: Tensor, w: Tensor, out: Tensor, desc: ConvDesc, epi: Optional[Epilogue], accum: Optional[Tensor] = None):
+    if accum is not None:
+        check(_hip.lib().td_conv_gemm_accum(ptr(src), ptr(w), ptr(out), C.byref(desc), C.byref(epi) if epi is not None else None, ptr(accum),
+                                            dtype_code(src.dtype), stream_ptr()), "td_conv_gemm_accum")
+        return
     check(_hip.lib().td_conv_gemm(ptr(src), ptr(w), ptr(out), C.byref(desc), C.byref(epi) if epi is not None else None,
                                   dtype_code(src.dtype), stream_ptr()), "td_conv_gemm")
 
@@ -237,12 +241,14 @@
 
 
 def linear_fwd(x: Tensor, w: Tensor, bias: Optional[Tensor] = None, *, residual=None, relu=False, sigmoid=False,
-               mask_src=None, dropout_p=0.0, seed=0, alpha=1.0, out: Optional[Tensor] = None) -> Tensor:
+               mask_src=None, dropout_p=0.0, seed=0, alpha=1.0, out: Optional[Tensor] = None, accum: Optional[Tensor] = None) -> Tensor:
     M, K = x.shape
     Nn = w.shape[0]
     assert w.shape[1] == K and w.dtype == x.dtype and x.is_contiguous() and w.is_contiguous()
     y = out if out is not None else torch.empty((M, Nn), dtype=x.dtype, device=x.device)
-    conv_gemm_raw(x, w, y, _desc(1, M, 1, K, M, 1, 1, 1, 1, 0, 0, Nn, Nn), _epi(bias, residual, mask_src, relu, sigmoid, dropout_p, seed, alpha))
+    if accum is not None:
+        assert accum.shape == (M, Nn) and accum.dtype == x.dtype and accum.is_contiguous() and accum.data_ptr() != y.data_ptr()
+    conv_gemm_raw(x, w, y, _desc(1, M, 1, K, M, 1, 1, 1, 1, 0, 0, Nn, Nn), _epi(bias, residual, mask_src, relu, sigmoid, dropout_p, seed, alpha), accum)
     return y
 
 
@@ -267,7 +273,7 @@
 def linear_ex(a1: Tensor, w: Tensor, bias: Optional[Tensor] = None, *, a2: Optional[Tensor] = None, a1_map: Optional[Tensor] = None,
               a2_map: Optional[Tensor] = None, w_shared: bool = False, out: Optional[Tensor] = None, out_map: Optional[Tensor] = None,
               out_rows: Optional[int] = None, residual: Optional[Tensor] = None, res_map: Optional[Tensor] = None, relu=False, mask_src=None,
-              dropout_p=0.0, seed=0, alpha=1.0) -> Tensor:
+              dropout_p=0.0, seed=0, alpha=1.0, accum: Optional[Tensor] = None) -> Tensor:
     _rows2d(a1)
     K1 = a1.shape[1]
     K2 = _rows2d(a2).shape[1] if a2 is not None else 0
@@ -283,10 +289,17 @@
     x.M, x.N, x.K1, x.K2 = M, Nn, K1, K2
     x.lda1, x.lda2, x.ldc = a1.stride(0), (a2.stride(0) if a2 is not None else 0), out.stride(0)
     x.ldr = _rows2d(residual).stride(0) if residual is not None else 0
+    if accum is not None:
+        assert accum.dtype == a1.dtype and (residual is None or _rows2d(accum).stride(0) == residual.stride(0))
+        x.ldr = _rows2d(accum).stride(0)
     x.w_shared = int(bool(w_shared and a2 is not None))
     x.rows1, x.rows2 = a1.shape[0], (a2.shape[0] if a2 is not None else 0)
     x.a1_map, x.a2_map, x.out_map, x.res_map = ptr(a1_map), ptr(a2_map), ptr(out_map), ptr(res_map)
     epi = _epi(bias, residual, mask_src, relu, False, dropout_p, seed, alpha)
+    if accum is not None:
+        check(_hip.lib().td_linear_ex_accum(ptr(a1), ptr(a2), ptr(w), ptr(out), C.byref(x), C.byref(epi), ptr(accum), dtype_code(a1.dtype), stream_ptr()),
+              "td_linear_ex_accum")
+        return out
     check(_hip.lib().td_linear_ex(ptr(a1), ptr(a2), ptr(w), ptr(out), C.byref(x), C.byref(epi), dtype_code(a1.dtype), stream_ptr()), "td_linear_ex")
     return out
 
@@ -391,11 +404,18 @@
     return y, (s if r is not None else x), mean, rstd
 
 
-def add_layernorm_bwd(dy: Tensor, s: Tensor, mean: Tensor, rstd: Tensor, gamma: Tensor, extra: Optional[Tensor] = None):
+def add_layernorm_bwd(dy: Tensor, s: Tensor, mean: Tensor, rstd: Tensor, gamma: Tensor, extra: Optional[Tensor] = None, *, drop=None):
     rows, cols = dy.shape
     ds = torch.empty_like(dy)
     dgamma = zeros_f32(cols, dy.device)
     dbeta = zeros_f32(cols, dy.device)
+    if drop is not None:
+        p, seed = drop
+        dsd = torch.empty_like(dy)
+        check(_hip.lib().td_add_layernorm_bwd_drop(ptr(dy), ptr(s), ptr(mean), ptr(rstd), ptr(gamma), ptr(extra), ptr(ds), ptr(dsd), ptr(dgamma),
+                                                   ptr(dbeta), rows, cols, p, seed & 0xFFFFFFFF, _ctr() if p > 0 else None, dtype_code(dy.dtype),
+                                                   stream_ptr()), "td_add_layernorm_bwd_drop")
+        return ds, dgamma, dbeta, dsd
     check(_hip.lib().td_add_layernorm_bwd(ptr(dy), ptr(s), ptr(mean), ptr(rstd), ptr(gamma), ptr(extra), ptr(ds), ptr(dgamma), ptr(dbeta),
                                           rows, cols, dtype_code(dy.dtype), stream_ptr()), "td_add_layernorm_bwd")
     return ds, dgamma, dbeta
```
